# sanweiliti/LEMO

Measured on AMD Instinct MI355X. Metric: fitting-iterations/sec (T=120 frames), higher is better.
Workload: dtype f32

## Files before the change

include/lemo_hip.h:

```cpp
#ifndef LEMO_HIP_H
#define LEMO_HIP_H

#ifdef __cplusplus
extern "C" {
#endif
#if defined(__GNUC__) || defined(__clang__)
#pragma GCC visibility push(default)
#endif

#define LEMO_ERR_SHAPE 10001
#define LEMO_ERR_ARG 10002
#define LEMO_ERR_STATE 10003

int lemo_abi_version(void);
int lemo_build_flags(void);

int lemo_conv3x3_mfma(const float* in, const float* wt, const float* bias, const float* aux, float* out,
                      int H, int W, int cin, int cout, int epi, int variant, void* stream);
int lemo_conv3x3_mfma_splitk(const float* in, const float* wt, const float* bias, const float* aux, float* out,
                             float* partial, int ks, int H, int W, int cin, int cout, int epi, void* stream);
int lemo_conv3x3_mfma_lds(const float* in, const float* wt, const float* wt2, const float* bias, const float* aux,
                          float* out, int H, int W, int cin, int cout, int epi, void* stream);
int lemo_conv3x3_mfma_lds_census(const float* in, const float* wt, const float* wt2, const float* bias, float* out,
                                 int H, int W, int cin, int cout, unsigned long long* dbg, void* stream);
int lemo_conv3x3_split_supported(int H, int W, int cin, int cout);
int lemo_conv3x3_mfma_split(const float* in, const void* w3, const float* wt, const float* bias, const float* aux,
                            float* out, int H, int W, int cin, int cout, int epi, void* stream);
int lemo_conv3x3_mfma_split_census(const float* in, const void* w3, const float* wt, const float* bias, float* out,
                                   int H, int W, int cin, int cout, unsigned long long* dbg, void* stream);
int lemo_conv3x3_mfma_split_f16(const float* in, const void* w2, float winv, const float* wt, const float* bias, const float* aux,
                                float* out, int H, int W, int cin, int cout, int epi, void* stream);
int lemo_conv3x3_mfma_split_census2(const float* in, const void* w, float winv, int pieces, const float* wt, const float* bias, float* out,
                                    int H, int W, int cin, int cout, unsigned long long* dbg, void* stream);
int lemo_conv3x3_pair_supported(int H, int W, int c0, int c1, int c2);
int lemo_conv3x3_pair_f16(const float* in, const void* wA, float winvA, const float* biasA, const float* auxA, float* mid,
                          const void* wB, float winvB, const float* biasB, const float* auxB, float* out, int H, int W, int epi,
                          unsigned long long* dbg, void* stream);
int lemo_conv3x3_wino_supported(int H, int W, int cin, int cout);
int lemo_conv3x3_wino_f16(const float* in, const void* wU, float winv, const float* wt, const float* bias, const float* aux, float* out,
                          int H, int W, int epi, unsigned long long* dbg, void* stream);
int lemo_conv3x3_c1(const float* x0, const float* w, const float* bias, float* out, int H, int W, int cout, void* stream);
int lemo_conv3x3_c1_bwd(const float* dpre, const float* w, float* dx0, int H, int W, int cout, void* stream);
int lemo_smooth_loss_blocks(int H, int W, int C);
int lemo_smooth_loss(const float* z, float* dpre, float* partial, int H, int W, int C, float coef2, void* stream);

typedef struct lemo_vposer_w {
  const float *w1, *w1t, *b1;
  const float *w2, *w2t, *b2;
  const float *w3, *w3t, *b3;
} lemo_vposer_w;
int lemo_vposer_decode_fwd(const lemo_vposer_w* w, const float* z, int z_stride, int B, float* h1, float* h2, float* o,
                           float* matrot, float* aa, void* stream);
int lemo_vposer_decode_bwd(const lemo_vposer_w* w, const float* h1, const float* h2, const float* o, const float* d_aa,
                           const float* d_matrot, int B, float* dz, int dz_stride, float* scratch, void* stream);
int lemo_vposer_mlp_bwd(const lemo_vposer_w* w, const float* h1, const float* h2, int B, float* dz, int dz_stride,
                        float* scratch, void* stream);
int lemo_gemm_nt16(const float* A, int lda, const float* B, int ldb, int M, int N, int K, float* C, int ldc,
                   const float* bias, const float* aux, int ldaux, int epi, void* stream);
int lemo_gemm_nt16_splitk_part_floats(int M, int S);
int lemo_gemm_nt16_splitk(const float* A, int lda, const float* B, int ldb, int M, int N, int K, float* C, int ldc, float* part, int S,
                          const float* A_grouped, void* stream);
int lemo_rot6d_to_aa_fwd(const float* x6, int stride, int N, float* aa, void* stream);
int lemo_rot6d_to_aa_bwd(const float* x6, int stride, const float* d_aa, int N, float* dx6, void* stream);

typedef struct lemo_body_const {
  int nj, nshape, ncomp, nlev;
  const int *parents, *level_start, *level_joints, *child_start, *child_list;
  const float *J_template, *J_dirs, *pose_mean, *lh_comp, *rh_comp;
} lemo_body_const;
typedef struct lemo_pose_in {
  const float *global_orient, *body_pose, *jaw, *leye, *reye, *lh, *rh;
  int hand_stride;
  const float* betas;
  int betas_stride;
  const float* expr;
  const float* rot6d;
  const float* vposer_o;
  float* go_out;
  double* zero_f64;
  int n_zero;
  const int* step_ctr;
  int* step_cur;
  int* nonfinite;
} lemo_pose_in;
typedef struct lemo_pose_ws {
  float *full_pose, *R, *J, *T, *A, *Jtr, *Xg;
  int Bp;
  unsigned short* XgS;
  int xgs_f16;
} lemo_pose_ws;
typedef struct lemo_pose_grad_in {
  const float *dA, *dJtr, *dX;
  const float* d_full_pose;
} lemo_pose_grad_in;
typedef struct lemo_pose_grad_out {
  float *d_global_orient, *d_body_pose, *d_jaw, *d_leye, *d_reye, *d_lh, *d_rh;
  int hand_stride;
  float *d_betas, *d_expr;
  const float* rot6d;
  float* d_rot6d;
  const float* vposer_o;
  float* d_vposer_o;
} lemo_pose_grad_out;
int lemo_smplx_pose_fwd(const lemo_body_const* c, const lemo_pose_in* in, const lemo_pose_ws* ws, int B, void* stream);
int lemo_smplx_pose_bwd(const lemo_body_const* c, const lemo_pose_ws* ws, const lemo_pose_grad_in* gi,
                        const lemo_pose_grad_out* go, int B, void* stream);

typedef struct lemo_skin_const {
  int V, NC, KW;
  int blend_fp32;
  const float* Dg;
  const float* v_template;
  const int* w_idx;
  const float* w_val;
  const unsigned short* DgH;
  float dgh_inv;
} lemo_skin_const;
typedef struct lemo_vertex_set_bwd {
  int n, NCs;
  const int *ids, *vp_row;
  const float* Dk;
  const float* DkT;
  const int *jcsr_start, *jcsr_u;
  const float* jcsr_w;
  const int* jcsr_chunk;
  const int* jc_u;
  const float* jc_w;
  float* part;
  int part_frames;
  int gemm_slabs;
  float* gemm_part;
  const float* DkG;
} lemo_vertex_set_bwd;
int lemo_lbs_verts_fwd(const lemo_skin_const* c, const float* Xg, int Bp, const float* A, int nj, const float* transl,
                       const int* ids, int n, int B, float* verts, float* v_posed, void* stream);
int lemo_lbs_verts_fwd_xs(const lemo_skin_const* c, const float* Xg, const unsigned short* XgS, int Bp, const float* A, int nj,
                          const float* transl, const int* ids, int n, int B, float* verts, float* v_posed, void* stream);
int lemo_lbs_verts_fwd_census(const lemo_skin_const* c, const float* Xg, int Bp, const float* A, int nj, const float* transl,
                              int n, int B, float* verts, float* v_posed, unsigned long long* dbg, void* stream,
                              const unsigned short* XgS );
int lemo_lbs_verts_fwd_active(const lemo_skin_const* c, const lemo_vertex_set_bwd* u, const float* Xg, int Bp, const float* A,
                              int nj, const float* transl, int B, float* blend, float* verts, float* v_posed, void* stream);
int lemo_lbs_verts_bwd(const lemo_skin_const* c, const lemo_vertex_set_bwd* u, const float* A, int nj, const float* v_posed,
                       int vp_rows, const float* dverts, int B, int Bp, float* dvp, float* dA, float* dtransl, float* dX,
                       void* stream);
int lemo_joints_assemble(const float* Jtr, int nj, const float* verts, int vrows, const int* extra_rows, int n_extra,
                         const int* lmk_rows, const float* lmk_bary, int n_lmk, const float* transl, int B, float* joints,
                         void* stream);

int lemo_reconstruct_global_body(const float* in, int T, int J, double rot_0_pivot, float* out, void* stream);
int lemo_reconstruct_global_body_dev(const float* in, int T, int J, const double* rot_0_pivot, float* out, void* stream);
int lemo_decode_clip(const float* rec, const float* traj, const double* stats, const double* rot_0_pivot, const float* post, int T,
                     int J, float* contact_lbl, float* markers, void* stream);
int lemo_local_markers_4chan(const float* body, const float* contact, int T, int M1, float* image, double* rot_0_pivot,
                             void* stream);

int lemo_maxpool3s2_fwd(const float* in, int H, int W, float* out, unsigned char* idx, int C, void* stream);
int lemo_maxpool3s2_bwd(const float* dout, const unsigned char* idx, const float* act, float* din, int H, int W, int C, void* stream);
int lemo_stuff2_fwd(const float* in, int h, int w, float* out, int H, int W, int C, void* stream);
int lemo_stuff2_bwd(const float* dout, int H, int W, const float* act, float* din, int h, int w, int C, void* stream);
int lemo_conv3x3_wgrad_nslab(int H, int W);
int lemo_conv3x3_wgrad(const float* dy, const float* x, int H, int W, int cin, int cout, int cin_real, int cout_real,
                       float* partial, float* dw, float* db, void* stream);
#define LEMO_WGRAD_MAX_JOBS 24
typedef struct lemo_wgrad_job {
  const float* partial;
  const float* dy;
  float* dw;
  float* db;
  int nslab, cin, cout, cin_real, cout_real, H, W;
} lemo_wgrad_job;
int lemo_conv3x3_wgrad_partial(const float* dy, const float* x, int H, int W, int cin, int cout, float* partial, void* stream);
int lemo_conv3x3_wgrad_reduce_multi(const lemo_wgrad_job* jobs, int n, void* stream);
int lemo_adam_flat(float* p, const float* g, float* m, float* v, int n, float lr, int step, void* stream);
int lemo_adam_flat_ctr(float* p, const float* g, float* m, float* v, int n, float lr, int* step_ctr, void* stream);

typedef struct lemo_ae_desc {
  int H, W;
  float lr;
  float* ws;
  long long ws_floats;
  int clips;
} lemo_ae_desc;
long long lemo_ae_ws_floats(int H, int W);
int lemo_ae_n_param(void);
void* lemo_ae_create(const lemo_ae_desc* d);
void lemo_ae_destroy(void* h);
int lemo_ae_load(void* h, const float* flat, const float* x, const float* moc, void* stream);
int lemo_ae_step(void* h, int n, int use_graph, void* stream);
int lemo_ae_forward(void* h, float* rec, float* z, void* stream);
int lemo_ae_params(void* h, float* flat_out, void* stream);
int lemo_ae_load_clip(void* h, int clip, const float* flat, const float* x, const float* moc, void* stream);
int lemo_ae_forward_clip(void* h, int clip, float* rec, float* z, void* stream);
int lemo_ae_params_clip(void* h, int clip, float* flat_out, void* stream);
int lemo_ae_wgrad_probe(void* h, int mode, void* stream);
int lemo_ae_conv(const float* in, const float* wt, const float* bias, const float* aux, float* out, int H, int W, int fineH, int fineW,
                 int in_s, int out_s, int cin, int cout, int epi, int mt, int pt, int ks, void* stream);
int lemo_ae_conv_f16(const float* in, const float* wt, const float* bias, const float* aux, float* out, int H, int W, int fineH, int fineW,
                     int in_s, int out_s, int cin, int cout, int epi, int mt, int pt, int ks, const float* amax_in, float in_fac,
                     const float* wmax, float* amax_out, void* stream);

typedef struct lemo_sptrain_desc {
  int H, W, bs;
  float lr;
  float weight_rec, weight_smooth;
  float* ws;
  long long ws_floats;
  int use_graph;
} lemo_sptrain_desc;
long long lemo_sptrain_ws_floats(int H, int W, int bs);
int lemo_sptrain_n_param(void);
void* lemo_sptrain_create(const lemo_sptrain_desc* d);
void lemo_sptrain_destroy(void* h);
int lemo_sptrain_load(void* h, const float* flat, void* stream);
int lemo_sptrain_step(void* h, const float* x, int n, float* losses, void* stream);
int lemo_sptrain_eval(void* h, const float* x, float* losses, float* rec, void* stream);
int lemo_sptrain_params(void* h, float* flat_out, void* stream);
int lemo_sptrain_grads(void* h, float* flat_out, void* stream);
long long lemo_wgrad3x3_batched_ws_floats(int H, int W, int bs, int ca, int cb);
int lemo_wgrad3x3_batched(const float* A, long long a_stride, const float* B, long long b_stride, int bs, int H, int W, int ca, int cb,
                          int bias_b, float* ws, float* gw, float* gb, void* stream);
int lemo_dec_end_fwd(const float* u, long long u_stride, const float* w8, const float* b8, const float* w9, const float* b9, float* r1,
                     float* rec, int bs, int H, int W, void* stream);

int lemo_capture_begin(void* stream);
int lemo_capture_end(void* stream, void** graph_exec);
int lemo_graph_launch(void* graph_exec, void* stream);
int lemo_graph_destroy(void* graph_exec);

int lemo_sdf_sample(const float* sdf, int D, int H, int W, const float* pts, int N, const float* gmin, const float* gmax,
                    float* val, float* dval, void* stream);

typedef struct lemo_fit_const {
  int n, n67, n81;
  const int *row67, *row81, *foot_start, *foot_row, *u_row, *u_m67, *u_m81, *u_foot_mask;
  const float *Xstd, *Xmean;
  const float* cam2world;
} lemo_fit_const;

int lemo_enc_head(const lemo_fit_const* fc, const float* verts, int nrows, const float* Jtr, int nj, const float* transl, int B, const float* w0,
                  const float* b0, const void* w1pack, float w1inv, const float* b1, float* x0, float* canon, float* act1, float* act2,
                  void* stream);
int lemo_enc_tail(const float* din, const void* w1bpack, float w1binv, const float* act1, const float* w0, float* dx0, int H, int W,
                  void* stream);
int lemo_enc_tail3(const float* din, const void* w2bpack, float w2binv, const float* act2, const void* w1bpack, float w1binv, const float* act1,
                   const float* w0, float* dx0, int H, int W, void* stream);

typedef struct lemo_fit_desc {
  int B, Bp, V, nrows;
  int full_vertices;
  int conv_variant;
  lemo_vposer_w vposer;
  lemo_body_const body;
  lemo_skin_const skin;
  lemo_vertex_set_bwd uset;
  lemo_fit_const fit;
  const int* fwd_ids;
  int enc_ch[11];
  const float* enc_w[10];
  const float* enc_b[10];
  const float* enc_wbwd[10];
  const float* enc_w2[10];
  const float* enc_wbwd2[10];
  const void* enc_w3[10];
  const void* enc_wbwd3[10];
  float enc_w3_inv[10];
  float enc_wbwd3_inv[10];
  const float* target;
  const float* contact;
  const float* weights;
  float weights_host[6];
  float *transl, *rot6d, *other;
  const float* shape;
  float *adam_m[3], *adam_v[3];
  int* step_ctr;
  float lr0, lr1;
  int lr_switch;
  float *go_aa, *body_aa, *h1, *h2, *vo, *vp_scratch;
  lemo_pose_ws pose;
  float *verts, *v_posed, *x0, *canon;
  float* act[11];
  float* dact[2];
  float *dx0, *spartial, *vpartial, *losses, *dverts, *dvp, *dA, *dX;
  double* loss_acc;
  int* step_cur;
  float *g_transl, *g_rot6d, *g_other, *g_go, *g_body;
  float* snap;
  int* nonfinite;
  int per_frame;
  float lr2;
  int lr_switch2;
  float* verts_side;
  float* transl_side;
} lemo_fit_desc;

void* lemo_fit_create(const lemo_fit_desc* d);
void lemo_fit_destroy(void* h);
int lemo_fit_forward(void* h, void* stream);
int lemo_fit_backward(void* h, void* stream);
int lemo_fit_step(void* h, int n, int use_graph, void* stream);
int lemo_fit_prepare(void* h, int n, void* stream);
#define LEMO_FIT_NSTAGE 7
int lemo_fit_census(void* h, int reps, float* ms_out , void* stream);
typedef struct lemo_fit_state {
  float *transl, *rot6d, *other;
  float *adam_m[3], *adam_v[3];
  int* step;
} lemo_fit_state;
int lemo_fit_load_state(void* h, const lemo_fit_state* st, void* stream);
int lemo_fit_save_state(void* h, const lemo_fit_state* st, void* stream);

typedef struct lemo_prox_const {
  int n_op, n_sj;
  const int* joint_map;
  const int *jm_start, *jm_list;
  int n_extra, n_lmk;
  const int* extra_rows;
  const int* lmk_rows;
  const float* lmk_bary;
  int n_s;
  const int *s_vid, *s_m67, *s_m81, *s_foot_mask, *s_fric;
  const int *s_jstart, *s_jidx;
  const float* s_jw;
  int n_fric;
  const int* fric_vid;
  int n67;
  const int* m67_vid;
  const int *foot_start, *foot_vid;
} lemo_prox_const;

#define LEMO_PROX_NW 13
typedef struct lemo_prox_desc {
  int B, Bp, V;
  int conv_variant;
  int first_batch_flag;
  int use_infill;
  int T;
  lemo_vposer_w vposer;
  lemo_body_const body;
  lemo_skin_const skin;
  lemo_vertex_set_bwd uset;
  lemo_fit_const fit;
  lemo_prox_const pc;
  int enc_ch[11];
  const float* enc_w[10]; const float* enc_b[10]; const float* enc_wbwd[10];
  const float* enc_w2[10]; const float* enc_wbwd2[10];
  const void* enc_w3[10]; const void* enc_wbwd3[10];
  float enc_w3_inv[10]; float enc_wbwd3_inv[10];
  const float* sdf; int sdf_dim[3];
  float grid_min[3], grid_max[3];
  float cam2world[12];
  float cam[4];
  const float* gt_joints;
  const float* w2;
  const float* marker_mask;
  const float* body_markers_rec;
  const float* contact_lbl_rec;
  const float* weights;
  float weights_host[LEMO_PROX_NW];
  float *global_orient, *transl, *left_hand_pose, *right_hand_pose, *jaw_pose, *leye_pose, *reye_pose, *expression, *pose_embedding;
  const float* betas;
  float *adam_m, *adam_v;
  int* step_ctr; int* step_cur; int* nonfinite;
  float lr;
  float *h1, *h2, *vo, *vp_scratch;
  lemo_pose_ws pose;
  float *verts, *v_posed, *dverts;
  float *x0, *canon, *dx0;
  float* act[11]; float* dact[2];
  float *dJtr, *dJv, *dtr_j, *gp, *dfp_add;
  float *dvp, *dA, *dtr_v, *dX;
  float *g_go, *g_lh, *g_rh, *g_jaw, *g_leye, *g_reye, *g_expr, *g_pe;
  double* loss_acc;
  float* losses;
} lemo_prox_desc;
void* lemo_prox_create(const lemo_prox_desc* d);
void lemo_prox_destroy(void* h);
int lemo_prox_closure(void* h, void* stream);
int lemo_prox_step(void* h, int n, int use_graph, void* stream);
typedef struct lemo_prox_state {
  float *global_orient, *transl, *left_hand_pose, *right_hand_pose, *jaw_pose, *leye_pose, *reye_pose, *expression, *pose_embedding;
  float *adam_m, *adam_v;
  int* step;
} lemo_prox_state;
int lemo_prox_load_state(void* h, const lemo_prox_state* st, void* stream);
int lemo_prox_save_state(void* h, const lemo_prox_state* st, void* stream);

#if defined(__GNUC__) || defined(__clang__)
#pragma GCC visibility pop
#endif
#ifdef __cplusplus
}
#endif
#endif
```

lemo_amd/_hip.py:

```python
from __future__ import annotations

import ctypes as C
import os
from typing import Optional

import torch

_CSRC = os.path.join(os.path.dirname(os.path.abspath(__file__)), 'csrc')
LIB_PATH = os.environ.get('LEMO_HIP_LIB') or os.path.join(_CSRC, 'liblemo_hip.so')
EMU_LIB_PATH = os.path.join(_CSRC, 'liblemo_emu.so')

fp = C.POINTER(C.c_float)
ip = C.POINTER(C.c_int)
vp = C.c_void_p


class VPoserW(C.Structure):
    _fields_ = [(n, vp) for n in ('w1', 'w1t', 'b1', 'w2', 'w2t', 'b2', 'w3', 'w3t', 'b3')]


class BodyConst(C.Structure):
    _fields_ = [('nj', C.c_int), ('nshape', C.c_int), ('ncomp', C.c_int), ('nlev', C.c_int)] + \
        [(n, vp) for n in ('parents', 'level_start', 'level_joints', 'child_start', 'child_list',
                           'J_template', 'J_dirs', 'pose_mean', 'lh_comp', 'rh_comp')]


class PoseIn(C.Structure):
    _fields_ = [(n, vp) for n in ('global_orient', 'body_pose', 'jaw', 'leye', 'reye', 'lh', 'rh')] + \
        [('hand_stride', C.c_int), ('betas', vp), ('betas_stride', C.c_int), ('expr', vp),
         ('rot6d', vp), ('vposer_o', vp), ('go_out', vp), ('zero_f64', vp), ('n_zero', C.c_int),
         ('step_ctr', vp), ('step_cur', vp), ('nonfinite', vp)]


class PoseWs(C.Structure):
    _fields_ = [(n, vp) for n in ('full_pose', 'R', 'J', 'T', 'A', 'Jtr', 'Xg')] + [('Bp', C.c_int), ('XgS', vp), ('xgs_f16', C.c_int)]


class PoseGradIn(C.Structure):
    _fields_ = [(n, vp) for n in ('dA', 'dJtr', 'dX', 'd_full_pose')]


class PoseGradOut(C.Structure):
    _fields_ = [(n, vp) for n in ('d_global_orient', 'd_body_pose', 'd_jaw', 'd_leye', 'd_reye', 'd_lh', 'd_rh')] + \
        [('hand_stride', C.c_int), ('d_betas', vp), ('d_expr', vp),
         ('rot6d', vp), ('d_rot6d', vp), ('vposer_o', vp), ('d_vposer_o', vp)]


WGRAD_MAX_JOBS = 24


class WgradJob(C.Structure):
    _fields_ = [('partial', vp), ('dy', vp), ('dw', vp), ('db', vp), ('nslab', C.c_int), ('cin', C.c_int), ('cout', C.c_int),
                ('cin_real', C.c_int), ('cout_real', C.c_int), ('H', C.c_int), ('W', C.c_int)]


class AeDesc(C.Structure):
    _fields_ = [('H', C.c_int), ('W', C.c_int), ('lr', C.c_float), ('ws', vp), ('ws_floats', C.c_longlong), ('clips', C.c_int)]


class SptrainDesc(C.Structure):
    _fields_ = [('H', C.c_int), ('W', C.c_int), ('bs', C.c_int), ('lr', C.c_float), ('weight_rec', C.c_float),
                ('weight_smooth', C.c_float), ('ws', vp), ('ws_floats', C.c_longlong), ('use_graph', C.c_int)]


class SkinConst(C.Structure):
    _fields_ = [('V', C.c_int), ('NC', C.c_int), ('KW', C.c_int), ('blend_fp32', C.c_int)] + \
        [(n, vp) for n in ('Dg', 'v_template', 'w_idx', 'w_val', 'DgH')] + [('dgh_inv', C.c_float)]


class VertexSetBwd(C.Structure):
    _fields_ = [('n', C.c_int), ('NCs', C.c_int)] + \
        [(n, vp) for n in ('ids', 'vp_row', 'Dk', 'DkT', 'jcsr_start', 'jcsr_u', 'jcsr_w', 'jcsr_chunk', 'jc_u', 'jc_w', 'part')] + \
        [('part_frames', C.c_int), ('gemm_slabs', C.c_int), ('gemm_part', vp), ('DkG', vp)]


class FitConst(C.Structure):
    _fields_ = [('n', C.c_int), ('n67', C.c_int), ('n81', C.c_int)] + \
        [(n, vp) for n in ('row67', 'row81', 'foot_start', 'foot_row', 'u_row', 'u_m67', 'u_m81',
                           'u_foot_mask', 'Xstd', 'Xmean', 'cam2world')]


CHAIN_MAX = 8


class FitDesc(C.Structure):
    _fields_ = [
        ('B', C.c_int), ('Bp', C.c_int), ('V', C.c_int), ('nrows', C.c_int), ('full_vertices', C.c_int),
        ('conv_variant', C.c_int),
        ('vposer', VPoserW), ('body', BodyConst), ('skin', SkinConst), ('uset', VertexSetBwd), ('fit', FitConst),
        ('fwd_ids', vp),
        ('enc_ch', C.c_int * 11), ('enc_w', vp * 10), ('enc_b', vp * 10), ('enc_wbwd', vp * 10),
        ('enc_w2', vp * 10), ('enc_wbwd2', vp * 10), ('enc_w3', vp * 10), ('enc_wbwd3', vp * 10), ('enc_w3_inv', C.c_float * 10), ('enc_wbwd3_inv', C.c_float * 10),
        ('target', vp), ('contact', vp), ('weights', vp), ('weights_host', C.c_float * 6),
        ('transl', vp), ('rot6d', vp), ('other', vp), ('shape', vp),
        ('adam_m', vp * 3), ('adam_v', vp * 3), ('step_ctr', vp),
        ('lr0', C.c_float), ('lr1', C.c_float), ('lr_switch', C.c_int),
        ('go_aa', vp), ('body_aa', vp), ('h1', vp), ('h2', vp), ('vo', vp), ('vp_scratch', vp),
        ('pose', PoseWs),
        ('verts', vp), ('v_posed', vp), ('x0', vp), ('canon', vp),
        ('act', vp * 11), ('dact', vp * 2),
        ('dx0', vp), ('spartial', vp), ('vpartial', vp), ('losses', vp), ('dverts', vp), ('dvp', vp),
        ('dA', vp), ('dX', vp), ('loss_acc', vp), ('step_cur', vp),
        ('g_transl', vp), ('g_rot6d', vp), ('g_other', vp), ('g_go', vp), ('g_body', vp),
        ('snap', vp), ('nonfinite', vp), ('per_frame', C.c_int), ('lr2', C.c_float), ('lr_switch2', C.c_int),
        ('verts_side', vp), ('transl_side', vp),
    ]


class ProxConst(C.Structure):
    _fields_ = [('n_op', C.c_int), ('n_sj', C.c_int), ('joint_map', vp), ('jm_start', vp), ('jm_list', vp),
                ('n_extra', C.c_int), ('n_lmk', C.c_int), ('extra_rows', vp), ('lmk_rows', vp), ('lmk_bary', vp),
                ('n_s', C.c_int), ('s_vid', vp), ('s_m67', vp), ('s_m81', vp), ('s_foot_mask', vp), ('s_fric', vp),
                ('s_jstart', vp), ('s_jidx', vp), ('s_jw', vp), ('n_fric', C.c_int), ('fric_vid', vp), ('n67', C.c_int),
                ('m67_vid', vp), ('foot_start', vp), ('foot_vid', vp)]


PROX_NW = 13


class ProxDesc(C.Structure):
    _fields_ = [
        ('B', C.c_int), ('Bp', C.c_int), ('V', C.c_int), ('conv_variant', C.c_int), ('first_batch_flag', C.c_int),
        ('use_infill', C.c_int), ('T', C.c_int),
        ('vposer', VPoserW), ('body', BodyConst), ('skin', SkinConst), ('uset', VertexSetBwd), ('fit', FitConst), ('pc', ProxConst),
        ('enc_ch', C.c_int * 11), ('enc_w', vp * 10), ('enc_b', vp * 10), ('enc_wbwd', vp * 10), ('enc_w2', vp * 10),
        ('enc_wbwd2', vp * 10), ('enc_w3', vp * 10), ('enc_wbwd3', vp * 10), ('enc_w3_inv', C.c_float * 10), ('enc_wbwd3_inv', C.c_float * 10),
        ('sdf', vp), ('sdf_dim', C.c_int * 3), ('grid_min', C.c_float * 3), ('grid_max', C.c_float * 3),
        ('cam2world', C.c_float * 12), ('cam', C.c_float * 4),
        ('gt_joints', vp), ('w2', vp), ('marker_mask', vp), ('body_markers_rec', vp), ('contact_lbl_rec', vp),
        ('weights', vp), ('weights_host', C.c_float * PROX_NW),
        ('global_orient', vp), ('transl', vp), ('left_hand_pose', vp), ('right_hand_pose', vp), ('jaw_pose', vp),
        ('leye_pose', vp), ('reye_pose', vp), ('expression', vp), ('pose_embedding', vp), ('betas', vp),
        ('adam_m', vp), ('adam_v', vp), ('step_ctr', vp), ('step_cur', vp), ('nonfinite', vp), ('lr', C.c_float),
        ('h1', vp), ('h2', vp), ('vo', vp), ('vp_scratch', vp), ('pose', PoseWs),
        ('verts', vp), ('v_posed', vp), ('dverts', vp), ('x0', vp), ('canon', vp), ('dx0', vp),
        ('act', vp * 11), ('dact', vp * 2),
        ('dJtr', vp), ('dJv', vp), ('dtr_j', vp), ('gp', vp), ('dfp_add', vp),
        ('dvp', vp), ('dA', vp), ('dtr_v', vp), ('dX', vp),
        ('g_go', vp), ('g_lh', vp), ('g_rh', vp), ('g_jaw', vp), ('g_leye', vp), ('g_reye', vp), ('g_expr', vp), ('g_pe', vp),
        ('loss_acc', vp), ('losses', vp),
    ]


class FitState(C.Structure):
    _fields_ = [('transl', vp), ('rot6d', vp), ('other', vp), ('adam_m', vp * 3), ('adam_v', vp * 3), ('step', vp)]


class ProxState(C.Structure):
    _fields_ = [(n, vp) for n in ('global_orient', 'transl', 'left_hand_pose', 'right_hand_pose', 'jaw_pose', 'leye_pose', 'reye_pose',
                                  'expression', 'pose_embedding', 'adam_m', 'adam_v', 'step')]


def ptr(t: Optional[torch.Tensor]):
    if t is None:
        return None
    assert t.is_contiguous(), 'C ABI takes contiguous buffers'
    return t.data_ptr()


class LemoHipError(RuntimeError):
    pass


_SIGS = {
    'lemo_abi_version': (C.c_int, []),
    'lemo_build_flags': (C.c_int, []),
    'lemo_conv3x3_mfma': (C.c_int, [vp, vp, vp, vp, vp, C.c_int, C.c_int, C.c_int, C.c_int, C.c_int, C.c_int, vp]),
    'lemo_conv3x3_mfma_splitk': (C.c_int, [vp, vp, vp, vp, vp, vp, C.c_int, C.c_int, C.c_int, C.c_int, C.c_int, C.c_int, vp]),
    'lemo_conv3x3_mfma_lds': (C.c_int, [vp, vp, vp, vp, vp, vp, C.c_int, C.c_int, C.c_int, C.c_int, C.c_int, vp]),
    'lemo_lbs_verts_fwd_active': (C.c_int, [C.POINTER(SkinConst), C.POINTER(VertexSetBwd), vp, C.c_int, vp, C.c_int, vp, C.c_int, vp, vp, vp, vp]),
    'lemo_capture_begin': (C.c_int, [vp]),
    'lemo_capture_end': (C.c_int, [vp, C.POINTER(C.c_void_p)]),
    'lemo_graph_launch': (C.c_int, [vp, vp]),
    'lemo_graph_destroy': (C.c_int, [vp]),
    'lemo_reconstruct_global_body': (C.c_int, [vp, C.c_int, C.c_int, C.c_double, vp, vp]),
    'lemo_reconstruct_global_body_dev': (C.c_int, [vp, C.c_int, C.c_int, vp, vp, vp]),
    'lemo_local_markers_4chan': (C.c_int, [vp, vp, C.c_int, C.c_int, vp, vp, vp]),
    'lemo_decode_clip': (C.c_int, [vp, vp, vp, vp, vp, C.c_int, C.c_int, vp, vp, vp]),
    'lemo_conv3x3_split_supported': (C.c_int, [C.c_int, C.c_int, C.c_int, C.c_int]),
    'lemo_conv3x3_mfma_split': (C.c_int, [vp, vp, vp, vp, vp, vp, C.c_int, C.c_int, C.c_int, C.c_int, C.c_int, vp]),
    'lemo_conv3x3_mfma_split_census': (C.c_int, [vp, vp, vp, vp, vp, C.c_int, C.c_int, C.c_int, C.c_int, vp, vp]),
    'lemo_conv3x3_mfma_split_f16': (C.c_int, [vp, vp, C.c_float, vp, vp, vp, vp, C.c_int, C.c_int, C.c_int, C.c_int, C.c_int, vp]),
    'lemo_conv3x3_pair_supported': (C.c_int, [C.c_int] * 5),
    'lemo_conv3x3_wino_supported': (C.c_int, [C.c_int] * 4),
    'lemo_conv3x3_wino_f16': (C.c_int, [vp, vp, C.c_float, vp, vp, vp, vp, C.c_int, C.c_int, C.c_int, vp, vp]),
    'lemo_conv3x3_pair_f16': (C.c_int, [vp, vp, C.c_float, vp, vp, vp, vp, C.c_float, vp, vp, vp, C.c_int, C.c_int, C.c_int, vp, vp]),
    'lemo_enc_head': (C.c_int, [vp, vp, C.c_int, vp, C.c_int, vp, C.c_int, vp, vp, vp, C.c_float, vp, vp, vp, vp, vp, vp]),
    'lemo_enc_tail': (C.c_int, [vp, vp, C.c_float, vp, vp, vp, C.c_int, C.c_int, vp]),
    'lemo_enc_tail3': (C.c_int, [vp, vp, C.c_float, vp, vp, C.c_float, vp, vp, vp, C.c_int, C.c_int, vp]),
    'lemo_conv3x3_mfma_split_census2': (C.c_int, [vp, vp, C.c_float, C.c_int, vp, vp, vp, C.c_int, C.c_int, C.c_int, C.c_int, vp, vp]),
    'lemo_conv3x3_mfma_lds_census': (C.c_int, [vp, vp, vp, vp, vp, C.c_int, C.c_int, C.c_int, C.c_int, vp, vp]),
    'lemo_conv3x3_c1': (C.c_int, [vp, vp, vp, vp, C.c_int, C.c_int, C.c_int, vp]),
    'lemo_conv3x3_c1_bwd': (C.c_int, [vp, vp, vp, C.c_int, C.c_int, C.c_int, vp]),
    'lemo_smooth_loss_blocks': (C.c_int, [C.c_int, C.c_int, C.c_int]),
    'lemo_smooth_loss': (C.c_int, [vp, vp, vp, C.c_int, C.c_int, C.c_int, C.c_float, vp]),
    'lemo_vposer_decode_fwd': (C.c_int, [C.POINTER(VPoserW), vp, C.c_int, C.c_int, vp, vp, vp, vp, vp, vp]),
    'lemo_vposer_decode_bwd': (C.c_int, [C.POINTER(VPoserW), vp, vp, vp, vp, vp, C.c_int, vp, C.c_int, vp, vp]),
    'lemo_vposer_mlp_bwd': (C.c_int, [C.POINTER(VPoserW), vp, vp, C.c_int, vp, C.c_int, vp, vp]),
    'lemo_gemm_nt16': (C.c_int, [vp, C.c_int, vp, C.c_int, C.c_int, C.c_int, C.c_int, vp, C.c_int, vp, vp, C.c_int, C.c_int, vp]),
    'lemo_gemm_nt16_splitk_part_floats': (C.c_int, [C.c_int, C.c_int]),
    'lemo_gemm_nt16_splitk': (C.c_int, [vp, C.c_int, vp, C.c_int, C.c_int, C.c_int, C.c_int, vp, C.c_int, vp, C.c_int, vp, vp]),
    'lemo_rot6d_to_aa_fwd': (C.c_int, [vp, C.c_int, C.c_int, vp, vp]),
    'lemo_rot6d_to_aa_bwd': (C.c_int, [vp, C.c_int, vp, C.c_int, vp, vp]),
    'lemo_smplx_pose_fwd': (C.c_int, [C.POINTER(BodyConst), C.POINTER(PoseIn), C.POINTER(PoseWs), C.c_int, vp]),
    'lemo_smplx_pose_bwd': (C.c_int, [C.POINTER(BodyConst), C.POINTER(PoseWs), C.POINTER(PoseGradIn),
                                      C.POINTER(PoseGradOut), C.c_int, vp]),
    'lemo_lbs_verts_fwd': (C.c_int, [C.POINTER(SkinConst), vp, C.c_int, vp, C.c_int, vp, vp, C.c_int, C.c_int, vp, vp, vp]),
    'lemo_lbs_verts_fwd_xs': (C.c_int, [C.POINTER(SkinConst), vp, vp, C.c_int, vp, C.c_int, vp, vp, C.c_int, C.c_int, vp, vp, vp]),
    'lemo_lbs_verts_fwd_census': (C.c_int, [C.POINTER(SkinConst), vp, C.c_int, vp, C.c_int, vp, C.c_int, C.c_int, vp, vp, vp, vp, vp]),
    'lemo_lbs_verts_bwd': (C.c_int, [C.POINTER(SkinConst), C.POINTER(VertexSetBwd), vp, C.c_int, vp, C.c_int, vp,
                                     C.c_int, C.c_int, vp, vp, vp, vp, vp]),
    'lemo_joints_assemble': (C.c_int, [vp, C.c_int, vp, C.c_int, vp, C.c_int, vp, vp, C.c_int, vp, C.c_int, vp, vp]),
    'lemo_maxpool3s2_fwd': (C.c_int, [vp, C.c_int, C.c_int, vp, vp, C.c_int, vp]),
    'lemo_maxpool3s2_bwd': (C.c_int, [vp, vp, vp, vp, C.c_int, C.c_int, C.c_int, vp]),
    'lemo_stuff2_fwd': (C.c_int, [vp, C.c_int, C.c_int, vp, C.c_int, C.c_int, C.c_int, vp]),
    'lemo_stuff2_bwd': (C.c_int, [vp, C.c_int, C.c_int, vp, vp, C.c_int, C.c_int, C.c_int, vp]),
    'lemo_conv3x3_wgrad_nslab': (C.c_int, [C.c_int, C.c_int]),
    'lemo_conv3x3_wgrad': (C.c_int, [vp, vp, C.c_int, C.c_int, C.c_int, C.c_int, C.c_int, C.c_int, vp, vp, vp, vp]),
    'lemo_conv3x3_wgrad_partial': (C.c_int, [vp, vp, C.c_int, C.c_int, C.c_int, C.c_int, vp, vp]),
    'lemo_conv3x3_wgrad_reduce_multi': (C.c_int, [C.POINTER(WgradJob), C.c_int, vp]),
    'lemo_adam_flat': (C.c_int, [vp, vp, vp, vp, C.c_int, C.c_float, C.c_int, vp]),
    'lemo_adam_flat_ctr': (C.c_int, [vp, vp, vp, vp, C.c_int, C.c_float, vp, vp]),
    'lemo_ae_ws_floats': (C.c_longlong, [C.c_int, C.c_int]),
    'lemo_ae_n_param': (C.c_int, []),
    'lemo_ae_create': (vp, [C.POINTER(AeDesc)]),
    'lemo_ae_destroy': (None, [vp]),
    'lemo_ae_load': (C.c_int, [vp, vp, vp, vp, vp]),
    'lemo_ae_step': (C.c_int, [vp, C.c_int, C.c_int, vp]),
    'lemo_ae_forward': (C.c_int, [vp, vp, vp, vp]),
    'lemo_ae_params': (C.c_int, [vp, vp, vp]),
    'lemo_ae_load_clip': (C.c_int, [vp, C.c_int, vp, vp, vp, vp]),
    'lemo_ae_forward_clip': (C.c_int, [vp, C.c_int, vp, vp, vp]),
    'lemo_ae_params_clip': (C.c_int, [vp, C.c_int, vp, vp]),
    'lemo_ae_wgrad_probe': (C.c_int, [vp, C.c_int, vp]),
    'lemo_ae_conv': (C.c_int, [vp, vp, vp, vp, vp] + [C.c_int] * 12 + [vp]),
    'lemo_ae_conv_f16': (C.c_int, [vp, vp, vp, vp, vp] + [C.c_int] * 12 + [vp, C.c_float, vp, vp, vp]),
    'lemo_sptrain_ws_floats': (C.c_longlong, [C.c_int, C.c_int, C.c_int]),
    'lemo_sptrain_n_param': (C.c_int, []),
    'lemo_sptrain_create': (vp, [C.POINTER(SptrainDesc)]),
    'lemo_sptrain_destroy': (None, [vp]),
    'lemo_sptrain_load': (C.c_int, [vp, vp, vp]),
    'lemo_sptrain_step': (C.c_int, [vp, vp, C.c_int, vp, vp]),
    'lemo_sptrain_eval': (C.c_int, [vp, vp, vp, vp, vp]),
    'lemo_sptrain_params': (C.c_int, [vp, vp, vp]),
    'lemo_sptrain_grads': (C.c_int, [vp, vp, vp]),
    'lemo_wgrad3x3_batched_ws_floats': (C.c_longlong, [C.c_int] * 5),
    'lemo_wgrad3x3_batched': (C.c_int, [vp, C.c_longlong, vp, C.c_longlong] + [C.c_int] * 6 + [vp, vp, vp, vp]),
    'lemo_dec_end_fwd': (C.c_int, [vp, C.c_longlong, vp, vp, vp, vp, vp, vp, C.c_int, C.c_int, C.c_int, vp]),
    'lemo_sdf_sample': (C.c_int, [vp, C.c_int, C.c_int, C.c_int, vp, C.c_int, C.POINTER(C.c_float), C.POINTER(C.c_float), vp, vp, vp]),
    'lemo_fit_create': (vp, [C.POINTER(FitDesc)]),
    'lemo_fit_destroy': (None, [vp]),
    'lemo_fit_forward': (C.c_int, [vp, vp]),
    'lemo_fit_backward': (C.c_int, [vp, vp]),
    'lemo_fit_step': (C.c_int, [vp, C.c_int, C.c_int, vp]),
    'lemo_fit_prepare': (C.c_int, [vp, C.c_int, vp]),
    'lemo_fit_census': (C.c_int, [vp, C.c_int, C.POINTER(C.c_float), vp]),
    'lemo_fit_load_state': (C.c_int, [vp, C.POINTER(FitState), vp]),
    'lemo_fit_save_state': (C.c_int, [vp, C.POINTER(FitState), vp]),
    'lemo_prox_load_state': (C.c_int, [vp, C.POINTER(ProxState), vp]),
    'lemo_prox_save_state': (C.c_int, [vp, C.POINTER(ProxState), vp]),
    'lemo_prox_create': (vp, [C.POINTER(ProxDesc)]),
    'lemo_prox_destroy': (None, [vp]),
    'lemo_prox_closure': (C.c_int, [vp, vp]),
    'lemo_prox_step': (C.c_int, [vp, C.c_int, C.c_int, vp]),
}
EXPORTED_SYMBOLS = tuple(_SIGS)


class HipLib:

    def __init__(self, path: str, is_emu: bool = False):
        if not os.path.exists(path):
            raise LemoHipError(
                f'{path} not found: the HIP extension is not built. Build it with '
                f'`make -C {_CSRC}` (hipcc --offload-arch=gfx950); there is no CPU fallback.')
        self.path, self.is_emu = path, is_emu
        self._dll = C.CDLL(path)
        for name, (res, args) in _SIGS.items():
            fn = getattr(self._dll, name)
            fn.restype, fn.argtypes = res, args
            setattr(self, name[len('lemo_'):], fn)
        if not self.build_flags() & 1:
            raise LemoHipError(f'{path} was built without -fno-slp-vectorize -fno-vectorize (-DLEMO_NO_PACKED_FP32): rebuild it with '
                               f'`make -C {_CSRC}`')

    def check(self, rc: int, what: str = ''):
        if rc != 0:
            raise LemoHipError(f'liblemo_hip: {what} failed with code {rc}')

    def stream(self, device) -> Optional[int]:
        if self.is_emu:
            return None
        return torch.cuda.current_stream(device).cuda_stream


_DEFERRED: list = []


def quiesce(device, lib=None) -> bool:
    try:
        dev = torch.device(device)
        if dev.type == 'cuda' and not (lib is not None and lib.is_emu) and torch.cuda.is_available():
            if torch.cuda.is_current_stream_capturing():
                return False
            torch.cuda.synchronize(dev)
    except Exception:
        pass
    return True


def flush_deferred() -> None:
    if not _DEFERRED:
        return
    try:
        if torch.cuda.is_available() and torch.cuda.is_current_stream_capturing():
            return
    except Exception:
        return
    pending, _DEFERRED[:] = list(_DEFERRED), []
    for fn in pending:
        try:
            fn()
        except Exception:
            pass


def release(device, lib, destroy, event=None) -> None:
    def wait():
        if event is None:
            return quiesce(device, lib)
        try:
            if torch.cuda.is_current_stream_capturing():
                return False
            event.synchronize()
        except Exception:
            pass
        return True

    def run():
        if event is not None:
            try:
                event.synchronize()
            except Exception:
                pass
        destroy()

    if wait():
        flush_deferred()
        try:
            destroy()
        except Exception:
            pass
    else:
        _DEFERRED.append(run)


_LIB: Optional[HipLib] = None


def get_lib() -> HipLib:
    global _LIB
    if _LIB is None:
        _LIB = HipLib(LIB_PATH, is_emu=False)
    return _LIB


def check_device(lib: HipLib, t: torch.Tensor):
    if lib.is_emu:
        if t.is_cuda:
            raise LemoHipError('the host-emulated test library only takes CPU tensors')
    elif not t.is_cuda:
        raise LemoHipError('lemo_amd compute entry points need tensors on a HIP device (no CPU fallback)')


class StreamOrdered:
    _gpu = False
    _setup_ev = _run_ev = None

    def _init_order(self, device, lib):
        self._gpu = torch.device(device).type == 'cuda' and not lib.is_emu and os.environ.get('LEMO_UNORDERED', '0') != '1'
        self._odev = torch.device(device)
        self._setup_ev = self._run_ev = None

    def _cur(self):
        return torch.cuda.current_stream(self._odev)

    def _before_write(self):
        if self._gpu and self._run_ev is not None:
            self._cur().wait_event(self._run_ev)

    def _after_write(self):
        if self._gpu:
            if self._setup_ev is None:
                self._setup_ev = torch.cuda.Event()
            self._setup_ev.record(self._cur())

    def _before_run(self):
        if self._gpu:
            flush_deferred()
            for ev in (self._setup_ev, self._run_ev):
                if ev is not None:
                    self._cur().wait_event(ev)

    def _after_run(self):
        if self._gpu:
            if self._run_ev is None:
                self._run_ev = torch.cuda.Event()
            self._run_ev.record(self._cur())

    _before_read = _before_write
```

lemo_amd/csrc/conv_head_kernels.hip:

```cpp
#include <type_traits>
#include "conv_f16.hpp"
#include "loss_device.hpp"

namespace lemo {

constexpr int HD_TH = 10, HD_TW = 14;
constexpr int HD_XW = HD_TW + 4, HD_XH = HD_TH + 4, HD_NX = HD_XW * HD_XH;
constexpr int HD_MIDW = HD_TW + 2, HD_MIDH = HD_TH + 2;
constexpr int HD_MIDP = HD_MIDW + 2, HD_NMIDP = HD_MIDP * HD_MIDH;
constexpr int HD_PL_MID = HD_NMIDP * 16, HD_GRP_MID = 2 * HD_PL_MID;
constexpr int HD_PL_IN = HD_NX * 16, HD_GRP_IN = 2 * HD_PL_IN;
static_assert(HD_MIDW == 16 && HD_XW == HD_MIDP, "N-tiles = 2 rows x 16 columns on grids of row pitch 18");

__device__ __forceinline__ int hd_lane_col(int j) { return j < 16 ? j : ((j - 18) & 15); }

template <int U, int END> struct HdSteps {
  template <class F> static __device__ __forceinline__ void run(F&& f) { f(std::integral_constant<int, U>{}); HdSteps<U + 1, END>::run(f); }
};
template <int END> struct HdSteps<END, END> { template <class F> static __device__ __forceinline__ void run(F&&) {} };

#define HD_RA 4
template <int GRP, int PL, int MT = 1, int NST = 18, int PITCH = HD_MIDP>
__device__ __forceinline__ void hd_kloop(f32x16 (&acc)[3], const uint4* __restrict__ w, const unsigned char* bbase, int li, int lane, int mt = 0) {
  const int h = lane >> 5;
  uint4 ra[HD_RA][2], rb[2][2];
#define HD_LOAD_A(SET, U) _Pragma("unroll") for (int s_ = 0; s_ < 2; ++s_) ra[SET][s_] = w[(unsigned)(((U) * MT + mt) * 2 + s_) * 64u + lane];
#define HD_LOAD_B(SET, U) _Pragma("unroll") for (int s_ = 0; s_ < 2; ++s_)                                                          \
    rb[SET][s_] = *reinterpret_cast<const uint4*>(bbase + (2 * ((U) / 9) + h) * GRP + s_ * PL + (li + (((U) % 9) / 3 - 1) * PITCH + (((U) % 9) % 3 - 1)) * 16);
#pragma unroll
  for (int u0 = 0; u0 < HD_RA - 1; ++u0) { HD_LOAD_A(u0, u0) }
  HD_LOAD_B(0, 0)
  HdSteps<0, NST>::run([&](auto uc) {
    constexpr int u = decltype(uc)::value;
    if (u + HD_RA - 1 < NST) { HD_LOAD_A((u + HD_RA - 1) % HD_RA, (u + HD_RA - 1 < NST ? u + HD_RA - 1 : NST - 1)) }
    if (u + 1 < NST) { HD_LOAD_B((u + 1) & 1, (u + 1 < NST ? u + 1 : NST - 1)) }
    __builtin_amdgcn_sched_barrier(0);
    acc[0] = __builtin_amdgcn_mfma_f32_32x32x16_f16(__builtin_bit_cast(f16x8, ra[u % HD_RA][0]), __builtin_bit_cast(f16x8, rb[u & 1][1]), acc[0], 0, 0, 0);
    acc[1] = __builtin_amdgcn_mfma_f32_32x32x16_f16(__builtin_bit_cast(f16x8, ra[u % HD_RA][1]), __builtin_bit_cast(f16x8, rb[u & 1][0]), acc[1], 0, 0, 0);
    acc[2] = __builtin_amdgcn_mfma_f32_32x32x16_f16(__builtin_bit_cast(f16x8, ra[u % HD_RA][0]), __builtin_bit_cast(f16x8, rb[u & 1][0]), acc[2], 0, 0, 0);
    __builtin_amdgcn_sched_barrier(0);
  });
#undef HD_LOAD_A
#undef HD_LOAD_B
}

template <int GRP, int PL, int MT>
__device__ __forceinline__ void hd_kloop2(f32x16 (&acc)[2][3], const uint4* __restrict__ w, const unsigned char* bbase, const int (&li)[2], int lane, int mt) {
  const int h = lane >> 5;
  uint4 ra[HD_RA][2], rb[2][2][2];
#define HD_LOAD_A(SET, U) _Pragma("unroll") for (int s_ = 0; s_ < 2; ++s_) ra[SET][s_] = w[(unsigned)(((U) * MT + mt) * 2 + s_) * 64u + lane];
#define HD_LOAD_B(SET, U) _Pragma("unroll") for (int t_ = 0; t_ < 2; ++t_) _Pragma("unroll") for (int s_ = 0; s_ < 2; ++s_)            \
    rb[SET][t_][s_] = *reinterpret_cast<const uint4*>(bbase + (2 * ((U) / 9) + h) * GRP + s_ * PL + (li[t_] + (((U) % 9) / 3 - 1) * HD_MIDP + (((U) % 9) % 3 - 1)) * 16);
#pragma unroll
  for (int u0 = 0; u0 < HD_RA - 1; ++u0) { HD_LOAD_A(u0, u0) }
  HD_LOAD_B(0, 0)
  HdSteps<0, 18>::run([&](auto uc) {
    constexpr int u = decltype(uc)::value;
    if (u + HD_RA - 1 < 18) { HD_LOAD_A((u + HD_RA - 1) % HD_RA, (u + HD_RA - 1 < 18 ? u + HD_RA - 1 : 17)) }
    if (u + 1 < 18) { HD_LOAD_B((u + 1) & 1, (u + 1 < 18 ? u + 1 : 17)) }
    __builtin_amdgcn_sched_barrier(0);
#pragma unroll
    for (int t_ = 0; t_ < 2; ++t_) {
      acc[t_][0] = __builtin_amdgcn_mfma_f32_32x32x16_f16(__builtin_bit_cast(f16x8, ra[u % HD_RA][0]), __builtin_bit_cast(f16x8, rb[u & 1][t_][1]), acc[t_][0], 0, 0, 0);
      acc[t_][1] = __builtin_amdgcn_mfma_f32_32x32x16_f16(__builtin_bit_cast(f16x8, ra[u % HD_RA][1]), __builtin_bit_cast(f16x8, rb[u & 1][t_][0]), acc[t_][1], 0, 0, 0);
      acc[t_][2] = __builtin_amdgcn_mfma_f32_32x32x16_f16(__builtin_bit_cast(f16x8, ra[u % HD_RA][0]), __builtin_bit_cast(f16x8, rb[u & 1][t_][0]), acc[t_][2], 0, 0, 0);
    }
    __builtin_amdgcn_sched_barrier(0);
  });
#undef HD_LOAD_A
#undef HD_LOAD_B
}

struct HeadArgs {
  FitConst fc;
  const float* verts; int nrows;
  const float* Jtr; int nj;
  const float* transl; int B;
  const float *w0, *b0;
  const uint4* w1; float w1inv;
  const float* b1;
  float *x0, *canon_out, *act1, *act2;
  int ntx, ntiles;
};

__global__ void __launch_bounds__(512)
enc_head_kernel(HeadArgs a) {
  __shared__ __attribute__((aligned(16))) unsigned char mid[4 * HD_GRP_MID];
  __shared__ float xs[HD_NX];
  __shared__ float cn[12];
  __shared__ float wmax[8];
  const FitConst& fc = a.fc;
  const int tid = (int)threadIdx.x, lane = tid & 63, wave = tid >> 6;
  const int D = 3 * fc.n81, H = D + 2, W = a.B - 1 + 16, Wp = W + 2, HWp = (H + 2) * Wp;
  int tile = (int)blockIdx.x;
  {
    const int q = a.ntiles >> 3, r = a.ntiles & 7, xcd = tile & 7, k = tile >> 3;
    tile = (xcd < r ? xcd * (q + 1) : r * (q + 1) + (xcd - r) * q) + k;
  }
  const int ty = tile / a.ntx, tx = tile - ty * a.ntx;
  const int y0 = ty * HD_TH, x0c = tx * HD_TW;
  float va[3] = {0.f, 0.f, 0.f}, vb[3] = {0.f, 0.f, 0.f}, xm = 0.f, xsd = 1.f;
  int cc = 0;
  bool inside = false;
  const int ip = tid < HD_NX ? tid : HD_NX - 1;
  const int ily = ip / HD_XW, ilx = ip - ily * HD_XW;
  {
    const int yy = y0 - 2 + ily, xx = x0c - 2 + ilx;
    inside = yy >= 0 && yy < H && xx >= 0 && xx < W;
    const int yc = min(max(yy, 0), H - 1), xc = min(max(xx, 0), W - 1);
    const int d = reflect_idx(yc - 1, D), tp = reflect_idx(xc - 8, a.B - 1);
    const int m = d / 3;
    cc = d - 3 * m;
    const float* v0 = a.verts + ((size_t)tp * a.nrows + fc.row81[m]) * 3;
    const float* v1 = v0 + (size_t)a.nrows * 3;
#pragma unroll
    for (int e = 0; e < 3; ++e) { va[e] = v0[e]; vb[e] = v1[e]; }
    xm = fc.Xmean[d]; xsd = fc.Xstd[d];
  }
  if (tid >= 512 - HD_MIDH * 2 * 8) {
    const int i = tid - (512 - HD_MIDH * 2 * 8), pl = i / (HD_MIDH * 2), rc = i - pl * (HD_MIDH * 2);
    *reinterpret_cast<uint4*>(mid + pl * HD_PL_MID + ((rc >> 1) * HD_MIDP + (rc & 1) * (HD_MIDP - 1)) * 16) = make_uint4(0u, 0u, 0u, 0u);
  }
  if (tid == 0) {
    canonical_frame(a.verts, a.nrows, fc.row81, a.Jtr, a.nj, a.transl, cn, fc.cam2world);
    if (blockIdx.x == 0) for (int i = 0; i < 12; ++i) a.canon_out[i] = cn[i];
  }
  __syncthreads();
  if (tid < HD_NX) {
    const float g0 = (va[0] - cn[9]) * cn[cc] + (va[1] - cn[10]) * cn[3 + cc] + (va[2] - cn[11]) * cn[6 + cc];
    const float g1 = (vb[0] - cn[9]) * cn[cc] + (vb[1] - cn[10]) * cn[3 + cc] + (vb[2] - cn[11]) * cn[6 + cc];
    const float n0 = (g0 - xm) / xsd, n1 = (g1 - xm) / xsd;
    const float v = inside ? n1 - n0 : 0.f;
    xs[tid] = v;
    if (inside && ily >= 2 && ily < 2 + HD_TH && ilx >= 2 && ilx < 2 + HD_TW)
      a.x0[(size_t)(y0 + ily - 2 + 1) * Wp + (x0c + ilx - 2 + 1)] = v;
  }
  __syncthreads();
  const int halfu = __builtin_amdgcn_readfirstlane(wave / 3);
  const bool worker = wave < 6;
  const int px = worker ? tid - 192 * halfu : 0;
  const int my = px >> 4, mx = px & 15;
  const int y = y0 - 1 + my, x = x0c - 1 + mx;
  const bool inimg = worker && (unsigned)y < (unsigned)H && (unsigned)x < (unsigned)W;
  const bool inner = inimg && my >= 1 && my <= HD_TH && mx >= 1 && mx <= HD_TW;
  float r[16];
  float mloc = 0.f;
  if (worker) {
    float xin[9];
#pragma unroll
    for (int tp = 0; tp < 9; ++tp) xin[tp] = xs[(my + tp / 3) * HD_XW + mx + tp % 3];
#pragma unroll
    for (int c = 0; c < 16; ++c) {
      const float* wc = a.w0 + (size_t)(halfu * 16 + c) * 9;
      float acc = 0.f;
#pragma unroll
      for (int tp = 0; tp < 9; ++tp) acc = fmaf(wc[tp], xin[tp], acc);
      const float v = lrelu(acc + a.b0[halfu * 16 + c]);
      r[c] = inimg ? v : 0.f;
      mloc = fmaxf(mloc, fabsf(r[c]));
    }
  } else {
#pragma unroll
    for (int c = 0; c < 16; ++c) r[c] = 0.f;
  }
  mloc = wave_max(mloc);
  if (lane == 0) wmax[wave] = mloc;
  __syncthreads();
  float sm, smi;
  {
    float mm = 0.f;
#pragma unroll
    for (int i = 0; i < 8; ++i) mm = fmaxf(mm, wmax[i]);
    f16_scale_for(mm, sm, smi);
  }
  if (worker) {
    const int yc = y < 0 ? 0 : (y >= H ? H - 1 : y), xc = x < 0 ? 0 : (x >= W ? W - 1 : x);
    const int poff = (yc + 1) * Wp + (xc + 1);
#pragma unroll
    for (int g = 0; g < 2; ++g) {
      const float4 lo4 = make_float4(r[8 * g], r[8 * g + 1], r[8 * g + 2], r[8 * g + 3]);
      const float4 hi4 = make_float4(r[8 * g + 4], r[8 * g + 5], r[8 * g + 6], r[8 * g + 7]);
      if (inner) {
        float* o = a.act1 + ((size_t)(2 * halfu + g) * HWp + poff) * 8;
        st4(o, lo4); st4(o + 4, hi4);
      }
      uint2 a0, a1, b0, b1;
      split2x4(lo4, sm, a0, a1);
      split2x4(hi4, sm, b0, b1);
      unsigned char* d = mid + (2 * halfu + g) * HD_GRP_MID + (my * HD_MIDP + mx + 1) * 16;
      *reinterpret_cast<uint4*>(d) = make_uint4(a0.x, a0.y, b0.x, b0.y);
      *reinterpret_cast<uint4*>(d + HD_PL_MID) = make_uint4(a1.x, a1.y, b1.x, b1.y);
    }
  }
  __syncthreads();
  if (wave >= 5) return;
  const int j = lane & 31, h = lane >> 5;
  const int oy = 2 * wave + (j >> 4), c = hd_lane_col(j), ox = c - 1;
  const int lo = (oy + 1) * HD_MIDP + c + 1;
  f32x16 acc[3];
#pragma unroll
  for (int p = 0; p < 3; ++p)
#pragma unroll
    for (int e = 0; e < 16; ++e) acc[p][e] = 0.f;
  hd_kloop<HD_GRP_MID, HD_PL_MID>(acc, a.w1, mid, lo, lane);
  const int yo = y0 + oy, xo = x0c + ox;
  const bool ok = ox >= 0 && ox < HD_TW && yo < H && xo < W;
  const int yoc = yo < H ? yo : H - 1, xoc = xo < 0 ? 0 : (xo < W ? xo : W - 1);
  const int po = (yoc + 1) * Wp + (xoc + 1);
  const float f = smi * a.w1inv;
#pragma unroll
  for (int q = 0; q < 4; ++q) {
    const int c0 = q * 8 + 4 * h;
    const float4 bb = ld4(a.b1 + c0);
    float4 v;
    v.x = lrelu(((acc[0][4 * q] + acc[1][4 * q]) + acc[2][4 * q]) * f + bb.x);
    v.y = lrelu(((acc[0][4 * q + 1] + acc[1][4 * q + 1]) + acc[2][4 * q + 1]) * f + bb.y);
    v.z = lrelu(((acc[0][4 * q + 2] + acc[1][4 * q + 2]) + acc[2][4 * q + 2]) * f + bb.z);
    v.w = lrelu(((acc[0][4 * q + 3] + acc[1][4 * q + 3]) + acc[2][4 * q + 3]) * f + bb.w);
    if (ok) st4(a.act2 + ((size_t)(c0 >> 3) * HWp + po) * 8 + (c0 & 7), v);
  }
}

int enc_head(const FitConst& fc, const float* verts, int nrows, const float* Jtr, int nj, const float* transl, int B, const float* w0,
             const float* b0, const void* w1pack, float w1inv, const float* b1, float* x0, float* canon, float* act1, float* act2,
             hipStream_t s) {
  if (B < 10 || !w1pack || !(w1inv > 0.f) || !verts || !x0 || !canon || !act1 || !act2) return LEMO_ERR_ARG;
  const int H = 3 * fc.n81 + 2, W = B - 1 + 16;
  HeadArgs a{};
  a.fc = fc; a.verts = verts; a.nrows = nrows; a.Jtr = Jtr; a.nj = nj; a.transl = transl; a.B = B;
  a.w0 = w0; a.b0 = b0; a.w1 = reinterpret_cast<const uint4*>(w1pack); a.w1inv = w1inv; a.b1 = b1;
  a.x0 = x0; a.canon_out = canon; a.act1 = act1; a.act2 = act2;
  a.ntx = (W + HD_TW - 1) / HD_TW;
  a.ntiles = a.ntx * ((H + HD_TH - 1) / HD_TH);
  hipLaunchKernelGGL(enc_head_kernel, dim3(a.ntiles), dim3(512), 0, s, a);
  return (int)hipGetLastError();
}

constexpr int H3_IW = HD_TW + 6, H3_IH = HD_TH + 6, H3_NI = H3_IW * H3_IH;
constexpr int H3_PL1 = HD_NX * 16, H3_GRP1 = 2 * H3_PL1;

struct Head3Args {
  HeadArgs h;
  const uint4* w2; float w2inv; const float* b2;
  float* act3;
};

__global__ void __launch_bounds__(512)
enc_head3_kernel(Head3Args A3) {
  __shared__ __attribute__((aligned(16))) unsigned char p1[4 * H3_GRP1];
  __shared__ __attribute__((aligned(16))) unsigned char p2[4 * HD_GRP_MID];
  __shared__ float xs[H3_NI];
  __shared__ float cn[12];
  __shared__ float wmax[24];
  const HeadArgs& a = A3.h;
  const FitConst& fc = a.fc;
  const int tid = (int)threadIdx.x, lane = tid & 63, wave = tid >> 6;
  const int j = lane & 31, h = lane >> 5;
  const int D = 3 * fc.n81, H = D + 2, W = a.B - 1 + 16, Wp = W + 2, HWp = (H + 2) * Wp;
  int tile = (int)blockIdx.x;
  {
    const int q = a.ntiles >> 3, r = a.ntiles & 7, xcd = tile & 7, k = tile >> 3;
    tile = (xcd < r ? xcd * (q + 1) : r * (q + 1) + (xcd - r) * q) + k;
  }
  const int ty = tile / a.ntx, tx = tile - ty * a.ntx;
  const int y0 = ty * HD_TH, x0c = tx * HD_TW;
  float va[3] = {0.f, 0.f, 0.f}, vb[3] = {0.f, 0.f, 0.f}, xm = 0.f, xsd = 1.f;
  int cc = 0;
  bool inside = false;
  const int ip = tid < H3_NI ? tid : H3_NI - 1;
  const int ily = ip / H3_IW, ilx = ip - ily * H3_IW;
  {
    const int yy = y0 - 3 + ily, xx = x0c - 3 + ilx;
    inside = yy >= 0 && yy < H && xx >= 0 && xx < W;
    const int yc = min(max(yy, 0), H - 1), xc = min(max(xx, 0), W - 1);
    const int d = reflect_idx(yc - 1, D), tp = reflect_idx(xc - 8, a.B - 1);
    const int m = d / 3;
    cc = d - 3 * m;
    const float* v0 = a.verts + ((size_t)tp * a.nrows + fc.row81[m]) * 3;
    const float* v1 = v0 + (size_t)a.nrows * 3;
#pragma unroll
    for (int e = 0; e < 3; ++e) { va[e] = v0[e]; vb[e] = v1[e]; }
    xm = fc.Xmean[d]; xsd = fc.Xstd[d];
  }
  if (tid >= 512 - HD_MIDH * 2 * 8) {
    const int i = tid - (512 - HD_MIDH * 2 * 8), pl = i / (HD_MIDH * 2), rc = i - pl * (HD_MIDH * 2);
    *reinterpret_cast<uint4*>(p2 + pl * HD_PL_MID + ((rc >> 1) * HD_MIDP + (rc & 1) * (HD_MIDP - 1)) * 16) = make_uint4(0u, 0u, 0u, 0u);
  }
  if (tid == 0) {
    canonical_frame(a.verts, a.nrows, fc.row81, a.Jtr, a.nj, a.transl, cn, fc.cam2world);
    if (blockIdx.x == 0) for (int i = 0; i < 12; ++i) a.canon_out[i] = cn[i];
  }
  __syncthreads();
  if (tid < H3_NI) {
    const float g0 = (va[0] - cn[9]) * cn[cc] + (va[1] - cn[10]) * cn[3 + cc] + (va[2] - cn[11]) * cn[6 + cc];
    const float g1 = (vb[0] - cn[9]) * cn[cc] + (vb[1] - cn[10]) * cn[3 + cc] + (vb[2] - cn[11]) * cn[6 + cc];
    const float n0 = (g0 - xm) / xsd, n1 = (g1 - xm) / xsd;
    const float v = inside ? n1 - n0 : 0.f;
    xs[tid] = v;
    if (inside && ily >= 3 && ily < 3 + HD_TH && ilx >= 3 && ilx < 3 + HD_TW)
      a.x0[(size_t)(y0 + ily - 3 + 1) * Wp + (x0c + ilx - 3 + 1)] = v;
  }
  __syncthreads();
  {
    const int halfu = __builtin_amdgcn_readfirstlane(wave >> 2);
    const int px = tid & 255;
    const bool worker = px < HD_NX;
    const int pc = worker ? px : 0;
    const int r1 = pc / HD_XW, c1 = pc - r1 * HD_XW;
    const int y = y0 - 2 + r1, x = x0c - 2 + c1;
    const bool inimg = worker && (unsigned)y < (unsigned)H && (unsigned)x < (unsigned)W;
    const bool inner = inimg && r1 >= 2 && r1 < 2 + HD_TH && c1 >= 2 && c1 < 2 + HD_TW;
    float r[16];
    float mloc = 0.f;
    float xin[9];
#pragma unroll
    for (int tp = 0; tp < 9; ++tp) xin[tp] = xs[(r1 + tp / 3) * H3_IW + c1 + tp % 3];
#pragma unroll
    for (int c = 0; c < 16; ++c) {
      const float* wc = a.w0 + (size_t)(halfu * 16 + c) * 9;
      float acc = 0.f;
#pragma unroll
      for (int tp = 0; tp < 9; ++tp) acc = fmaf(wc[tp], xin[tp], acc);
      const float v = lrelu(acc + a.b0[halfu * 16 + c]);
      r[c] = inimg ? v : 0.f;
      mloc = fmaxf(mloc, fabsf(r[c]));
    }
    mloc = wave_max(mloc);
    if (lane == 0) wmax[wave] = mloc;
    __syncthreads();
    float sm, smi;
    {
      float mm = 0.f;
#pragma unroll
      for (int i = 0; i < 8; ++i) mm = fmaxf(mm, wmax[i]);
      f16_scale_for(mm, sm, smi);
    }
    if (lane == 0 && wave == 0) wmax[20] = smi;
    if (worker) {
      const int yc = y < 0 ? 0 : (y >= H ? H - 1 : y), xc = x < 0 ? 0 : (x >= W ? W - 1 : x);
      const int poff = (yc + 1) * Wp + (xc + 1);
#pragma unroll
      for (int g = 0; g < 2; ++g) {
        const float4 lo4 = make_float4(r[8 * g], r[8 * g + 1], r[8 * g + 2], r[8 * g + 3]);
        const float4 hi4 = make_float4(r[8 * g + 4], r[8 * g + 5], r[8 * g + 6], r[8 * g + 7]);
        if (inner) {
          float* o = a.act1 + ((size_t)(2 * halfu + g) * HWp + poff) * 8;
          st4(o, lo4); st4(o + 4, hi4);
        }
        uint2 a0, a1, b0, b1;
        split2x4(lo4, sm, a0, a1);
        split2x4(hi4, sm, b0, b1);
        unsigned char* d = p1 + (2 * halfu + g) * H3_GRP1 + pc * 16;
        *reinterpret_cast<uint4*>(d) = make_uint4(a0.x, a0.y, b0.x, b0.y);
        *reinterpret_cast<uint4*>(d + H3_PL1) = make_uint4(a1.x, a1.y, b1.x, b1.y);
      }
    }
  }
  __syncthreads();
  float4 v1[4];
  float m1 = 0.f;
  int mp2 = 0, mpoff = 0;
  bool inner2 = false;
  if (wave < 6) {
    const int my = 2 * wave + (j >> 4), mx = hd_lane_col(j);
    const int li = (my + 1) * HD_XW + mx + 1;
    f32x16 acc[3];
#pragma unroll
    for (int p = 0; p < 3; ++p)
#pragma unroll
      for (int e = 0; e < 16; ++e) acc[p][e] = 0.f;
    hd_kloop<H3_GRP1, H3_PL1>(acc, a.w1, p1, li, lane);
    const int y = y0 - 1 + my, x = x0c - 1 + mx;
    const bool inimg = (unsigned)y < (unsigned)H && (unsigned)x < (unsigned)W;
    inner2 = inimg && my >= 1 && my <= HD_TH && mx >= 1 && mx <= HD_TW;
    const int yc = y < 0 ? 0 : (y >= H ? H - 1 : y), xc = x < 0 ? 0 : (x >= W ? W - 1 : x);
    mpoff = (yc + 1) * Wp + (xc + 1);
    mp2 = my * HD_MIDP + mx + 1;
    const float f = wmax[20] * a.w1inv;
#pragma unroll
    for (int q = 0; q < 4; ++q) {
      const float4 bb = ld4(a.b1 + q * 8 + 4 * h);
      float4 v;
      v.x = lrelu(((acc[0][4 * q] + acc[1][4 * q]) + acc[2][4 * q]) * f + bb.x);
      v.y = lrelu(((acc[0][4 * q + 1] + acc[1][4 * q + 1]) + acc[2][4 * q + 1]) * f + bb.y);
      v.z = lrelu(((acc[0][4 * q + 2] + acc[1][4 * q + 2]) + acc[2][4 * q + 2]) * f + bb.z);
      v.w = lrelu(((acc[0][4 * q + 3] + acc[1][4 * q + 3]) + acc[2][4 * q + 3]) * f + bb.w);
      if (!inimg) v = make_float4(0.f, 0.f, 0.f, 0.f);
      v1[q] = v;
      m1 = absmax4(v, m1);
    }
  } else {
#pragma unroll
    for (int q = 0; q < 4; ++q) v1[q] = make_float4(0.f, 0.f, 0.f, 0.f);
  }
  m1 = wave_max(m1);
  if (lane == 0 && wave < 6) wmax[8 + wave] = m1;
  if (lane == 0 && wave >= 6) wmax[8 + wave] = 0.f;
  __syncthreads();
  float sm2, smi2;
  {
    float mm = 0.f;
#pragma unroll
    for (int i = 0; i < 8; ++i) mm = fmaxf(mm, wmax[8 + i]);
    f16_scale_for(mm, sm2, smi2);
  }
  if (wave < 6) {
#pragma unroll
    for (int q = 0; q < 4; ++q) {
      const int c0 = q * 8 + 4 * h;
      if (inner2) st4(a.act2 + ((size_t)(c0 >> 3) * HWp + mpoff) * 8 + (c0 & 7), v1[q]);
      uint2 s0, s1;
      split2x4(v1[q], sm2, s0, s1);
      unsigned char* d = p2 + q * HD_GRP_MID + mp2 * 16 + 8 * h;
      *reinterpret_cast<uint2*>(d) = s0;
      *reinterpret_cast<uint2*>(d + HD_PL_MID) = s1;
    }
  }
  __syncthreads();
  {
    const int mt = wave & 1, ts = wave >> 1;
    const float f = smi2 * A3.w2inv;
    auto store_tile = [&](const f32x16 (&acc)[3], int T) {
      const int oy = 2 * T + (j >> 4), c = hd_lane_col(j), ox = c - 1;
      const int yo = y0 + oy, xo = x0c + ox;
      const bool ok = ox >= 0 && ox < HD_TW && yo < H && xo < W;
      const int yoc = yo < H ? yo : H - 1, xoc = xo < 0 ? 0 : (xo < W ? xo : W - 1);
      const int po = (yoc + 1) * Wp + (xoc + 1);
#pragma unroll
      for (int q = 0; q < 4; ++q) {
        const int c0 = mt * 32 + q * 8 + 4 * h;
        const float4 bb = ld4(A3.b2 + c0);
        float4 v;
        v.x = lrelu(((acc[0][4 * q] + acc[1][4 * q]) + acc[2][4 * q]) * f + bb.x);
        v.y = lrelu(((acc[0][4 * q + 1] + acc[1][4 * q + 1]) + acc[2][4 * q + 1]) * f + bb.y);
        v.z = lrelu(((acc[0][4 * q + 2] + acc[1][4 * q + 2]) + acc[2][4 * q + 2]) * f + bb.z);
        v.w = lrelu(((acc[0][4 * q + 3] + acc[1][4 * q + 3]) + acc[2][4 * q + 3]) * f + bb.w);
        if (ok) st4(A3.act3 + ((size_t)(c0 >> 3) * HWp + po) * 8 + (c0 & 7), v);
      }
    };
    auto lo_of = [&](int T) { const int oy = 2 * T + (j >> 4), c = hd_lane_col(j); return (oy + 1) * HD_MIDP + c + 1; };
    if (ts < 3) {
      f32x16 acc[3];
#pragma unroll
      for (int p = 0; p < 3; ++p)
#pragma unroll
        for (int e = 0; e < 16; ++e) acc[p][e] = 0.f;
      hd_kloop<HD_GRP_MID, HD_PL_MID, 2>(acc, A3.w2, p2, lo_of(ts), lane, mt);
      store_tile(acc, ts);
    } else {
      f32x16 acc[2][3];
#pragma unroll
      for (int t = 0; t < 2; ++t)
#pragma unroll
        for (int p = 0; p < 3; ++p)
#pragma unroll
          for (int e = 0; e < 16; ++e) acc[t][p][e] = 0.f;
      const int li2[2] = {lo_of(3), lo_of(4)};
      hd_kloop2<HD_GRP_MID, HD_PL_MID, 2>(acc, A3.w2, p2, li2, lane, mt);
      store_tile(acc[0], 3);
      store_tile(acc[1], 4);
    }
  }
}

int enc_head3(const FitConst& fc, const float* verts, int nrows, const float* Jtr, int nj, const float* transl, int B, const float* w0,
              const float* b0, const void* w1pack, float w1inv, const float* b1, const void* w2pack, float w2inv, const float* b2,
              float* x0, float* canon, float* act1, float* act2, float* act3, hipStream_t s) {
  if (B < 10 || !w1pack || !w2pack || !(w1inv > 0.f) || !(w2inv > 0.f) || !verts || !x0 || !canon || !act1 || !act2 || !act3) return LEMO_ERR_ARG;
  const int H = 3 * fc.n81 + 2, W = B - 1 + 16;
  Head3Args A{};
  HeadArgs& a = A.h;
  a.fc = fc; a.verts = verts; a.nrows = nrows; a.Jtr = Jtr; a.nj = nj; a.transl = transl; a.B = B;
  a.w0 = w0; a.b0 = b0; a.w1 = reinterpret_cast<const uint4*>(w1pack); a.w1inv = w1inv; a.b1 = b1;
  a.x0 = x0; a.canon_out = canon; a.act1 = act1; a.act2 = act2;
  a.ntx = (W + HD_TW - 1) / HD_TW;
  a.ntiles = a.ntx * ((H + HD_TH - 1) / HD_TH);
  A.w2 = reinterpret_cast<const uint4*>(w2pack); A.w2inv = w2inv; A.b2 = b2; A.act3 = act3;
  hipLaunchKernelGGL(enc_head3_kernel, dim3(a.ntiles), dim3(512), 0, s, A);
  return (int)hipGetLastError();
}

struct TailArgs {
  const float* din;
  const uint4* w1b; float w1binv;
  const float* act1;
  const float* w0;
  float* dx0;
  int H, W, ntx, ntiles;
};

__global__ void __launch_bounds__(512)
enc_tail_kernel(TailArgs a) {
  __shared__ __attribute__((aligned(16))) unsigned char inp[4 * HD_GRP_IN];
  __shared__ __attribute__((aligned(16))) float d1[32 * HD_NMIDP];
  __shared__ float wmax[8];
  const int tid = (int)threadIdx.x, lane = tid & 63, wave = tid >> 6;
  const int H = a.H, W = a.W, Wp = W + 2, HWp = (H + 2) * Wp;
  int tile = (int)blockIdx.x;
  {
    const int q = a.ntiles >> 3, r = a.ntiles & 7, xcd = tile & 7, k = tile >> 3;
    tile = (xcd < r ? xcd * (q + 1) : r * (q + 1) + (xcd - r) * q) + k;
  }
  const int ty = tile / a.ntx, tx = tile - ty * a.ntx;
  const int y0 = ty * HD_TH, x0c = tx * HD_TW;
  float4 st[4];
  int dst[4];
#pragma unroll
  for (int k = 0; k < 4; ++k) {
    int c0 = tid + k * 512;
    c0 = c0 < 4 * 2 * HD_NX ? c0 : 4 * 2 * HD_NX - 1;
    const int gg = c0 / (2 * HD_NX), c = c0 - gg * (2 * HD_NX);
    const int px = c >> 1, half = c & 1;
    const int r = px / HD_XW, col = px - r * HD_XW;
    int gy = y0 - 2 + r, gx = x0c - 2 + col;
    gy = (gy < -1 ? -1 : (gy > H ? H : gy)) + 1;
    gx = (gx < -1 ? -1 : (gx > W ? W : gx)) + 1;
    st[k] = ld4(a.din + ((size_t)gg * HWp + gy * Wp + gx) * 8 + 4 * half);
    dst[k] = gg * HD_GRP_IN + px * 16 + 8 * half;
  }
  float sc, sci;
  {
    float m = 0.f;
#pragma unroll
    for (int k = 0; k < 4; ++k) m = absmax4(st[k], m);
    m = wave_max(m);
    if (lane == 0) wmax[wave] = m;
    __syncthreads();
    float mm = 0.f;
#pragma unroll
    for (int i = 0; i < 8; ++i) mm = fmaxf(mm, wmax[i]);
    f16_scale_for(mm, sc, sci);
  }
#pragma unroll
  for (int k = 0; k < 4; ++k) {
    uint2 s0, s1;
    split2x4(st[k], sc, s0, s1);
    *reinterpret_cast<uint2*>(inp + dst[k]) = s0;
    *reinterpret_cast<uint2*>(inp + dst[k] + HD_PL_IN) = s1;
  }
  __syncthreads();
  if (wave < 6) {
    const int j = lane & 31, h = lane >> 5;
    const int my = 2 * wave + (j >> 4), mx = hd_lane_col(j);
    const int li = (my + 1) * HD_XW + mx + 1;
    f32x16 acc[3];
#pragma unroll
    for (int p = 0; p < 3; ++p)
#pragma unroll
      for (int e = 0; e < 16; ++e) acc[p][e] = 0.f;
    const int y = y0 - 1 + my, x = x0c - 1 + mx;
    const bool inimg = (unsigned)y < (unsigned)H && (unsigned)x < (unsigned)W;
    const int yc = y < 0 ? 0 : (y >= H ? H - 1 : y), xc = x < 0 ? 0 : (x >= W ? W - 1 : x);
    const int poff = (yc + 1) * Wp + (xc + 1);
    float4 aux[4];
#pragma unroll
    for (int q = 0; q < 4; ++q) { const int c0 = q * 8 + 4 * h; aux[q] = ld4(a.act1 + ((size_t)(c0 >> 3) * HWp + poff) * 8 + (c0 & 7)); }
    hd_kloop<HD_GRP_IN, HD_PL_IN>(acc, a.w1b, inp, li, lane);
    const float f = sci * a.w1binv;
#pragma unroll
    for (int q = 0; q < 4; ++q) {
      const int c0 = q * 8 + 4 * h;
      float v[4];
      const float ax[4] = {aux[q].x, aux[q].y, aux[q].z, aux[q].w};
#pragma unroll
      for (int e = 0; e < 4; ++e) {
        const float s = ((acc[0][4 * q + e] + acc[1][4 * q + e]) + acc[2][4 * q + e]) * f * lrelu_grad_from_out(ax[e]);
        v[e] = inimg ? s : 0.f;
      }
#pragma unroll
      for (int e = 0; e < 4; ++e) d1[(c0 + e) * HD_NMIDP + my * HD_MIDP + mx + 1] = v[e];
    }
  }
  __syncthreads();
  if (tid < HD_TH * HD_TW) {
    const int oy = tid / HD_TW, ox = tid - oy * HD_TW;
    const int y = y0 + oy, x = x0c + ox;
    if (y < H && x < W) {
      float acc = 0.f;
      for (int g = 0; g < 4; ++g) {
#pragma unroll
        for (int t = 0; t < 9; ++t) {
          const int dy = t / 3 - 1, dx = t % 3 - 1;
          const float* q = d1 + (size_t)(g * 8) * HD_NMIDP + (oy + 1 - dy) * HD_MIDP + (ox + 1 - dx) + 1;
          const float* wc = a.w0 + (size_t)(g * 8) * 9 + t;
#pragma unroll
          for (int c = 0; c < 8; ++c) acc = fmaf(q[c * HD_NMIDP], wc[9 * c], acc);
        }
      }
      a.dx0[(size_t)y * W + x] = acc;
    }
  }
}

int enc_tail(const float* din, const void* w1bpack, float w1binv, const float* act1, const float* w0, float* dx0, int H, int W, hipStream_t s) {
  if (!din || !w1bpack || !(w1binv > 0.f) || !act1 || !w0 || !dx0 || H < 1 || W < 1) return LEMO_ERR_ARG;
  TailArgs a{};
  a.din = din; a.w1b = reinterpret_cast<const uint4*>(w1bpack); a.w1binv = w1binv; a.act1 = act1; a.w0 = w0; a.dx0 = dx0;
  a.H = H; a.W = W;
  a.ntx = (W + HD_TW - 1) / HD_TW;
  a.ntiles = a.ntx * ((H + HD_TH - 1) / HD_TH);
  hipLaunchKernelGGL(enc_tail_kernel, dim3(a.ntiles), dim3(512), 0, s, a);
  return (int)hipGetLastError();
}

constexpr int T3_IW = HD_TW + 6, T3_IH = HD_TH + 6, T3_NI = T3_IW * T3_IH;
constexpr int T3_PL = T3_NI * 16, T3_GRP = 2 * T3_PL;
constexpr int T3_MID_OFF = 8 * T3_GRP;
constexpr int T3_WMAX_OFF = T3_MID_OFF + 4 * HD_GRP_IN;
constexpr int T3_SMEM = T3_WMAX_OFF + 16 * 4;
static_assert(32 * HD_NMIDP * 4 <= T3_MID_OFF, "d(pre-act 1) fits in the dead input planes");

struct Tail3Args {
  TailArgs t;
  const uint4* w2b; float w2binv;
  const float* act2;
};

__global__ void __launch_bounds__(512)
enc_tail3_kernel(Tail3Args A3) {
  LEMO_DYN_SMEM(smem_f);
  unsigned char* smem = reinterpret_cast<unsigned char*>(smem_f);
  unsigned char* inp = smem + T3_MID_OFF;
  float* d1 = smem_f;
  float* wmax = reinterpret_cast<float*>(smem + T3_WMAX_OFF);
  const TailArgs& a = A3.t;
  const int tid = (int)threadIdx.x, lane = tid & 63, wave = tid >> 6;
  const int j = lane & 31, h = lane >> 5;
  const int H = a.H, W = a.W, Wp = W + 2, HWp = (H + 2) * Wp;
  int tile = (int)blockIdx.x;
  {
    const int q = a.ntiles >> 3, r = a.ntiles & 7, xcd = tile & 7, k = tile >> 3;
    tile = (xcd < r ? xcd * (q + 1) : r * (q + 1) + (xcd - r) * q) + k;
  }
  const int ty = tile / a.ntx, tx = tile - ty * a.ntx;
  const int y0 = ty * HD_TH, x0c = tx * HD_TW;
  float sc, sci;
  {
    float4 st[10];
    int dst[10];
#pragma unroll
    for (int k = 0; k < 10; ++k) {
      const int c0 = tid + k * 512;
      const int gg = c0 / (2 * T3_NI), c = c0 - gg * (2 * T3_NI);
      const int px = c >> 1, half = c & 1;
      const int r = px / T3_IW, col = px - r * T3_IW;
      int gy = y0 - 3 + r, gx = x0c - 3 + col;
      gy = (gy < -1 ? -1 : (gy > H ? H : gy)) + 1;
      gx = (gx < -1 ? -1 : (gx > W ? W : gx)) + 1;
      st[k] = ld4(a.din + ((size_t)gg * HWp + gy * Wp + gx) * 8 + 4 * half);
      dst[k] = gg * T3_GRP + px * 16 + 8 * half;
    }
    float m = 0.f;
#pragma unroll
    for (int k = 0; k < 10; ++k) m = absmax4(st[k], m);
    m = wave_max(m);
    if (lane == 0) wmax[wave] = m;
    __syncthreads();
    float mm = 0.f;
#pragma unroll
    for (int i = 0; i < 8; ++i) mm = fmaxf(mm, wmax[i]);
    f16_scale_for(mm, sc, sci);
#pragma unroll
    for (int k = 0; k < 10; ++k) {
      uint2 s0, s1;
      split2x4(st[k], sc, s0, s1);
      *reinterpret_cast<uint2*>(smem + dst[k]) = s0;
      *reinterpret_cast<uint2*>(smem + dst[k] + T3_PL) = s1;
    }
  }
  __syncthreads();
  {
    const int o = 32 * wave + j, oc = o < HD_NX ? o : HD_NX - 1;
    const int r = oc / HD_XW, c = oc - r * HD_XW;
    const int li = (r + 1) * T3_IW + c + 1;
    const int y = y0 - 2 + r, x = x0c - 2 + c;
    const bool inimg = (unsigned)y < (unsigned)H && (unsigned)x < (unsigned)W;
    const int yc = y < 0 ? 0 : (y >= H ? H - 1 : y), xc = x < 0 ? 0 : (x >= W ? W - 1 : x);
    const int poff = (yc + 1) * Wp + (xc + 1);
    float4 aux[4];
#pragma unroll
    for (int q = 0; q < 4; ++q) { const int c0 = q * 8 + 4 * h; aux[q] = ld4(A3.act2 + ((size_t)(c0 >> 3) * HWp + poff) * 8 + (c0 & 7)); }
    f32x16 acc[3];
#pragma unroll
    for (int p = 0; p < 3; ++p)
#pragma unroll
      for (int e = 0; e < 16; ++e) acc[p][e] = 0.f;
    hd_kloop<T3_GRP, T3_PL, 1, 36, T3_IW>(acc, A3.w2b, smem, li, lane);
    const float f = sci * A3.w2binv;
    float4 v2[4];
    float m2 = 0.f;
#pragma unroll
    for (int q = 0; q < 4; ++q) {
      const float ax[4] = {aux[q].x, aux[q].y, aux[q].z, aux[q].w};
      float v[4];
#pragma unroll
      for (int e = 0; e < 4; ++e) {
        const float s = ((acc[0][4 * q + e] + acc[1][4 * q + e]) + acc[2][4 * q + e]) * f * lrelu_grad_from_out(ax[e]);
        v[e] = inimg ? s : 0.f;
      }
      v2[q] = make_float4(v[0], v[1], v[2], v[3]);
      m2 = absmax4(v2[q], m2);
    }
    m2 = wave_max(m2);
    if (lane == 0) wmax[8 + wave] = m2;
    __syncthreads();
    float mm = 0.f;
#pragma unroll
    for (int i = 0; i < 8; ++i) mm = fmaxf(mm, wmax[8 + i]);
    f16_scale_for(mm, sc, sci);
    if (o < HD_NX) {
#pragma unroll
      for (int q = 0; q < 4; ++q) {
        uint2 s0, s1;
        split2x4(v2[q], sc, s0, s1);
        unsigned char* d = inp + q * HD_GRP_IN + o * 16 + 8 * h;
        *reinterpret_cast<uint2*>(d) = s0;
        *reinterpret_cast<uint2*>(d + HD_PL_IN) = s1;
      }
    }
  }
  __syncthreads();
  if (wave < 6) {
    const int my = 2 * wave + (j >> 4), mx = hd_lane_col(j);
    const int li = (my + 1) * HD_XW + mx + 1;
    f32x16 acc[3];
#pragma unroll
    for (int p = 0; p < 3; ++p)
#pragma unroll
      for (int e = 0; e < 16; ++e) acc[p][e] = 0.f;
    const int y = y0 - 1 + my, x = x0c - 1 + mx;
    const bool inimg = (unsigned)y < (unsigned)H && (unsigned)x < (unsigned)W;
    const int yc = y < 0 ? 0 : (y >= H ? H - 1 : y), xc = x < 0 ? 0 : (x >= W ? W - 1 : x);
    const int poff = (yc + 1) * Wp + (xc + 1);
    float4 aux[4];
#pragma unroll
    for (int q = 0; q < 4; ++q) { const int c0 = q * 8 + 4 * h; aux[q] = ld4(a.act1 + ((size_t)(c0 >> 3) * HWp + poff) * 8 + (c0 & 7)); }
    hd_kloop<HD_GRP_IN, HD_PL_IN>(acc, a.w1b, inp, li, lane);
    const float f = sci * a.w1binv;
#pragma unroll
    for (int q = 0; q < 4; ++q) {
      const int c0 = q * 8 + 4 * h;
      float v[4];
      const float ax[4] = {aux[q].x, aux[q].y, aux[q].z, aux[q].w};
#pragma unroll
      for (int e = 0; e < 4; ++e) {
        const float s = ((acc[0][4 * q + e] + acc[1][4 * q + e]) + acc[2][4 * q + e]) * f * lrelu_grad_from_out(ax[e]);
        v[e] = inimg ? s : 0.f;
      }
#pragma unroll
      for (int e = 0; e < 4; ++e) d1[(c0 + e) * HD_NMIDP + my * HD_MIDP + mx + 1] = v[e];
    }
  }
  __syncthreads();
  if (tid < HD_TH * HD_TW) {
    const int oy = tid / HD_TW, ox = tid - oy * HD_TW;
    const int y = y0 + oy, x = x0c + ox;
    if (y < H && x < W) {
      float acc = 0.f;
      for (int g = 0; g < 4; ++g) {
#pragma unroll
        for (int t = 0; t < 9; ++t) {
          const int dy = t / 3 - 1, dx = t % 3 - 1;
          const float* q = d1 + (size_t)(g * 8) * HD_NMIDP + (oy + 1 - dy) * HD_MIDP + (ox + 1 - dx) + 1;
          const float* wc = a.w0 + (size_t)(g * 8) * 9 + t;
#pragma unroll
          for (int c = 0; c < 8; ++c) acc = fmaf(q[c * HD_NMIDP], wc[9 * c], acc);
        }
      }
      a.dx0[(size_t)y * W + x] = acc;
    }
  }
}

int enc_tail3_init() {
  static LdsOptinOnce once;
  return lds_optin(once, {{&enc_tail3_kernel, T3_SMEM}});
}

int enc_tail3(const float* din, const void* w2bpack, float w2binv, const float* act2, const void* w1bpack, float w1binv, const float* act1,
              const float* w0, float* dx0, int H, int W, hipStream_t s) {
  if (!din || !w2bpack || !(w2binv > 0.f) || !act2 || !w1bpack || !(w1binv > 0.f) || !act1 || !w0 || !dx0 || H < 1 || W < 1) return LEMO_ERR_ARG;
  if (int rc = enc_tail3_init()) return rc;
  Tail3Args A{};
  TailArgs& a = A.t;
  a.din = din; a.w1b = reinterpret_cast<const uint4*>(w1bpack); a.w1binv = w1binv; a.act1 = act1; a.w0 = w0; a.dx0 = dx0;
  a.H = H; a.W = W;
  a.ntx = (W + HD_TW - 1) / HD_TW;
  a.ntiles = a.ntx * ((H + HD_TH - 1) / HD_TH);
  A.w2b = reinterpret_cast<const uint4*>(w2bpack); A.w2binv = w2binv; A.act2 = act2;
  hipLaunchKernelGGL(enc_tail3_kernel, dim3(a.ntiles), dim3(512), T3_SMEM, s, A);
  return (int)hipGetLastError();
}

}
```

lemo_amd/csrc/conv_pair_kernels.hip:

```cpp
#include "conv_common.hpp"
#include "conv_f16.hpp"

namespace lemo {

constexpr int CP_TH = 10, CP_TW = 14;
constexpr int CP_INW = CP_TW + 4, CP_INH = CP_TH + 4, CP_NIN = CP_INW * CP_INH;
constexpr int CP_MIDW = CP_TW + 2, CP_MIDH = CP_TH + 2, CP_NMID = CP_MIDW * CP_MIDH;
constexpr int CP_MIDP = CP_MIDW + 2, CP_NMIDP = CP_MIDP * CP_MIDH;
constexpr int CP_NOUT = CP_TH * CP_TW;
constexpr int CP_PL_IN = CP_NIN * 16, CP_GRP_IN = 2 * CP_PL_IN;
constexpr int CP_PL_MID = CP_NMIDP * 16, CP_GRP_MID = 2 * CP_PL_MID;
constexpr int CP_MID_OFF = 8 * CP_GRP_IN;
constexpr int CP_WMAX_OFF = CP_MID_OFF + 8 * CP_GRP_MID;
constexpr int CP_SMEM = CP_WMAX_OFF + 3 * 8 * 4;
constexpr int CP_NSLOT = 4;
static_assert(CP_MIDW == 16 && CP_NMID == 6 * 32 && CP_INW == CP_MIDP, "N-tiles = 2 rows x 16 columns on grids of row pitch 18");
static_assert(4 * 2 * CP_NIN <= CP_NSLOT * 512 && CP_NOUT == 140, "staging slots");
static_assert(8 * 6 * 256 * 4 <= CP_MID_OFF, "the K-half exchange (6 quads per wave) fits the dead input planes");

struct PairArgs {
  const float* in;
  const uint4* wA;
  const uint4* wB;
  const float *biasA, *biasB;
  const float *auxA, *auxB;
  float* mid;
  float* out;
  float winvA, winvB;
  int H, W, ntx, ntiles;
  unsigned long long* dbg;
};

template <int NT> struct PairSplit {
  static constexpr int NQ = NT == 3 ? 6 : 4;
  static constexpr int keep_tile(int KH, int i) { return i < 4 ? KH : 2; }
  static constexpr int keep_quad(int KH, int i) { return i < 4 ? i : (i - 4) + 2 * KH; }
  static constexpr int give_tile(int KH, int i) { return i < 4 ? 1 - KH : 2; }
  static constexpr int give_quad(int KH, int i) { return i < 4 ? i : (i - 4) + 2 * (1 - KH); }
};

template <int NT, int KH>
__device__ __forceinline__ void pair_exchange(const f32x16 (&acc)[3], float4 (&v)[6], float* red_mine, const float* red_theirs) {
  typedef PairSplit<NT> S;
#pragma unroll
  for (int i = 0; i < S::NQ; ++i) {
    const int t = S::give_tile(KH, i), q = S::give_quad(KH, i);
    st4(red_mine + i * 256, make_float4(acc[t][4 * q], acc[t][4 * q + 1], acc[t][4 * q + 2], acc[t][4 * q + 3]));
  }
  __syncthreads();
#pragma unroll
  for (int i = 0; i < S::NQ; ++i) {
    const int t = S::keep_tile(KH, i), q = S::keep_quad(KH, i);
    const float4 o = ld4(red_theirs + i * 256);
    const float4 m = make_float4(acc[t][4 * q], acc[t][4 * q + 1], acc[t][4 * q + 2], acc[t][4 * q + 3]);
    v[i] = KH ? make_float4(o.x + m.x, o.y + m.y, o.z + m.z, o.w + m.w) : make_float4(m.x + o.x, m.y + o.y, m.z + o.z, m.w + o.w);
  }
}

__device__ __forceinline__ int cp_lane_col(int j) { return j < 16 ? j : ((j - 18) & 15); }

#define CP_RA 3

__device__ __forceinline__ void pair_preload_a(uint4 (&ra)[CP_RA][2], const uint4* __restrict__ w, int kh, int ch, int lane) {
#pragma unroll
  for (int u0 = 0; u0 < CP_RA - 1; ++u0)
#pragma unroll
    for (int s_ = 0; s_ < 2; ++s_) ra[u0][s_] = w[(unsigned)((((2 * kh) * 9 + u0) * 2 + ch) * 2 + s_) * 64u + lane];
}

template <int NT, int GRP, int PL, int PITCH, typename MidFn, typename EndFn>
__device__ __forceinline__ void pair_kloop(f32x16 (&acc)[3], uint4 (&ra)[CP_RA][2], const uint4* __restrict__ w, const unsigned char* bbase,
                                           const int (&li)[3], int kh, int ch, int lane, MidFn&& mid_fn, EndFn&& end_fn) {
  const int h = lane >> 5;
  uint4 rb[2][3][2];
#define CP_LOAD_A(SET, U)                                                                              \
  _Pragma("unroll") for (int s_ = 0; s_ < 2; ++s_)                                                     \
    ra[SET][s_] = w[(unsigned)((((2 * kh + (U) / 9) * 9 + (U) % 9) * 2 + ch) * 2 + s_) * 64u + lane];
#define CP_LOAD_B(SET, U)                                                                              \
  _Pragma("unroll") for (int nt_ = 0; nt_ < NT; ++nt_)                                                 \
    _Pragma("unroll") for (int s_ = 0; s_ < 2; ++s_)                                                   \
      rb[SET][nt_][s_] = *reinterpret_cast<const uint4*>(                                              \
          bbase + (2 * (2 * kh + (U) / 9) + h) * GRP + s_ * PL + (li[nt_] + (((U) % 9) / 3 - 1) * PITCH + (((U) % 9) % 3 - 1)) * 16);
#define CP_MFMA1(SA, SETA, SB, SETB)                                                                   \
  _Pragma("unroll") for (int nt_ = 0; nt_ < NT; ++nt_)                                                 \
    acc[nt_] = __builtin_amdgcn_mfma_f32_32x32x16_f16(__builtin_bit_cast(f16x8, ra[SETA][SA]),         \
                                                      __builtin_bit_cast(f16x8, rb[SETB][nt_][SB]), acc[nt_], 0, 0, 0);
#pragma unroll
  for (int cc = 0; cc < 2; ++cc) {
    CP_LOAD_B((cc * 9) & 1, cc * 9)
#pragma unroll
    for (int tap = 0; tap < 9; ++tap) {
      const int u = cc * 9 + tap;
      if (u + CP_RA - 1 < 18) { CP_LOAD_A((u + CP_RA - 1) % CP_RA, u + CP_RA - 1) }
      if (tap + 1 < 9) { CP_LOAD_B((u + 1) & 1, u + 1) }
      __builtin_amdgcn_sched_barrier(0);
      CP_MFMA1(0, u % CP_RA, 1, u & 1) CP_MFMA1(1, u % CP_RA, 0, u & 1) CP_MFMA1(0, u % CP_RA, 0, u & 1)
      mid_fn(cc, tap);
      __builtin_amdgcn_sched_barrier(0);
    }
    end_fn(cc);
  }
#undef CP_LOAD_A
#undef CP_LOAD_B
#undef CP_MFMA1
}

template <int EPI, int NT>
__device__ __forceinline__ void pair_layer2(const PairArgs& a, unsigned char* smem, float* smem_f, int y0, int x0, int T0, int ng2, int ch,
                                            int kh, int lane, float smi, uint4 (&ra)[CP_RA][2]) {
  const int j = lane & 31, h = lane >> 5;
  const int Wp = a.W + 2, HWp = (a.H + 2) * Wp;
  int lo[3] = {0, 0, 0}, poff[3] = {0, 0, 0};
  bool ok[3] = {false, false, false};
#pragma unroll
  for (int nt = 0; nt < NT; ++nt) {
    const int oy = 2 * (T0 + nt) + (j >> 4), c = cp_lane_col(j), ox = c - 1;
    lo[nt] = (oy + 1) * CP_MIDP + c + 1;
    const int y = y0 + oy, x = x0 + ox;
    ok[nt] = ox >= 0 && ox < CP_TW && y < a.H && x < a.W;
    const int yc = y < a.H ? y : a.H - 1, xc = x < 0 ? 0 : (x < a.W ? x : a.W - 1);
    poff[nt] = (yc + 1) * Wp + (xc + 1);
  }
  f32x16 acc[3];
#pragma unroll
  for (int nt = 0; nt < 3; ++nt)
#pragma unroll
    for (int r = 0; r < 16; ++r) acc[nt][r] = 0.f;
  pair_kloop<NT, CP_GRP_MID, CP_PL_MID, CP_MIDP>(acc, ra, a.wB, smem + CP_MID_OFF, lo, kh, ch, lane, [](int, int) {}, [](int) {});
  {
    const float f = smi * a.winvB;
#pragma unroll
    for (int nt = 0; nt < NT; ++nt)
#pragma unroll
      for (int r = 0; r < 16; ++r) acc[nt][r] *= f;
  }
  typedef PairSplit<NT> S;
  const int KHu = __builtin_amdgcn_readfirstlane(kh);
  const int poA = KHu ? poff[1] : poff[0], poB = poff[2];
  const bool okA = KHu ? ok[1] : ok[0], okB = ok[2];
  float4 eo[6];
#pragma unroll
  for (int i = 0; i < S::NQ; ++i) {
    const int q = KHu ? S::keep_quad(1, i) : S::keep_quad(0, i);
    const int c0 = ch * 32 + q * 8 + 4 * h;
    const int po = i < 4 ? poA : poB;
    eo[i] = EPI == 1 ? ld4(a.auxB + ((size_t)(c0 >> 3) * HWp + po) * 8 + (c0 & 7)) : ld4(a.biasB + c0);
  }
  float* red = smem_f + ((ng2 * 2 + ch) * 2) * 1536 + lane * 4;
  float4 v[6];
  if (KHu) pair_exchange<NT, 1>(acc, v, red + 1536, red);
  else pair_exchange<NT, 0>(acc, v, red, red + 1536);
#pragma unroll
  for (int i = 0; i < S::NQ; ++i) {
    const int q = KHu ? S::keep_quad(1, i) : S::keep_quad(0, i);
    const int c0 = ch * 32 + q * 8 + 4 * h;
    const int po = i < 4 ? poA : poB;
    const bool st = i < 4 ? okA : okB;
    float4 r = v[i];
    if (EPI == 1) {
      r.x *= lrelu_grad_from_out(eo[i].x); r.y *= lrelu_grad_from_out(eo[i].y);
      r.z *= lrelu_grad_from_out(eo[i].z); r.w *= lrelu_grad_from_out(eo[i].w);
    } else {
      r.x = lrelu(r.x + eo[i].x); r.y = lrelu(r.y + eo[i].y); r.z = lrelu(r.z + eo[i].z); r.w = lrelu(r.w + eo[i].w);
    }
    if (st) st4(a.out + ((size_t)(c0 >> 3) * HWp + po) * 8 + (c0 & 7), r);
  }
}

template <int EPI, bool DBG>
__global__ void __launch_bounds__(512)
conv3x3_pair_kernel(PairArgs a) {
  unsigned long long t_start = 0, t_pro = 0, t_l1 = 0, t_mid = 0, t_ex = 0, t_mx = 0;
  if (DBG) t_start = __builtin_amdgcn_s_memtime();
  LEMO_DYN_SMEM(smem_f);
  unsigned char* smem = reinterpret_cast<unsigned char*>(smem_f);
  float* wmax = reinterpret_cast<float*>(smem + CP_WMAX_OFF);
  const int tid = (int)threadIdx.x, lane = tid & 63, wave = tid >> 6;
  const int j = lane & 31, h = lane >> 5;
  const int ng = wave & 1, ch = (wave >> 1) & 1, kh = wave >> 2;
  const int H = a.H, W = a.W, Wp = W + 2, HWp = (H + 2) * Wp;
  const unsigned in_gstride = (unsigned)HWp * 8u;
  int tile = (int)blockIdx.x;
  {
    const int q = a.ntiles >> 3, r = a.ntiles & 7, xcd = tile & 7, k = tile >> 3;
    tile = (xcd < r ? xcd * (q + 1) : r * (q + 1) + (xcd - r) * q) + k;
  }
  const int ty = tile / a.ntx, tx = tile - ty * a.ntx;
  const int y0 = ty * CP_TH, x0 = tx * CP_TW;

  uint4 ra[CP_RA][2];
  pair_preload_a(ra, a.wA, kh, ch, lane);

  unsigned offB[CP_NSLOT];
  int dstB[CP_NSLOT];
#pragma unroll
  for (int k = 0; k < CP_NSLOT; ++k) {
    int c0 = tid + k * 512;
    c0 = c0 < 4 * 2 * CP_NIN ? c0 : 4 * 2 * CP_NIN - 1;
    const int gg = c0 / (2 * CP_NIN), c = c0 - gg * (2 * CP_NIN);
    const int px = c >> 1, half = c & 1;
    const int r = px / CP_INW, col = px - r * CP_INW;
    int gy = y0 - 2 + r, gx = x0 - 2 + col;
    gy = (gy < -1 ? -1 : (gy > H ? H : gy)) + 1;
    gx = (gx < -1 ? -1 : (gx > W ? W : gx)) + 1;
    const int g0 = (gg >> 1) * 4 + (gg & 1);
    offB[k] = (unsigned)g0 * in_gstride + (unsigned)(gy * Wp + gx) * 8u + 4u * half;
    dstB[k] = g0 * CP_GRP_IN + px * 16 + 8 * half;
  }
  float4 stB[CP_NSLOT];
#pragma unroll
  for (int k = 0; k < CP_NSLOT; ++k) stB[k] = ld4(a.in + offB[k]);
  if (tid < CP_MIDH * 2 * 16) {
    const int pl = tid / (CP_MIDH * 2), rc = tid - pl * (CP_MIDH * 2);
    *reinterpret_cast<uint4*>(smem + CP_MID_OFF + pl * CP_PL_MID + ((rc >> 1) * CP_MIDP + (rc & 1) * (CP_MIDP - 1)) * 16) = make_uint4(0u, 0u, 0u, 0u);
  }
  float sc[2] = {1.f, 1.f}, sci[2] = {1.f, 1.f};
  {
    float m = 0.f;
#pragma unroll
    for (int k = 0; k < CP_NSLOT; ++k) m = absmax4(stB[k], m);
    m = wave_max(m);
    if (lane == 0) wmax[wave] = m;
    __syncthreads();
    float mm = 0.f;
#pragma unroll
    for (int i = 0; i < 8; ++i) mm = fmaxf(mm, wmax[i]);
    f16_scale_for(mm, sc[0], sci[0]);
  }
#pragma unroll
  for (int k = 0; k < CP_NSLOT; ++k) {
    uint2 s0, s1;
    split2x4(stB[k], sc[0], s0, s1);
    *reinterpret_cast<uint2*>(smem + dstB[k]) = s0;
    *reinterpret_cast<uint2*>(smem + dstB[k] + CP_PL_IN) = s1;
  }
#pragma unroll
  for (int k = 0; k < CP_NSLOT; ++k) stB[k] = ld4(a.in + 2u * in_gstride + offB[k]);
  __syncthreads();
  if (DBG) t_pro = __builtin_amdgcn_s_memtime();

  int li[3];
#pragma unroll
  for (int nt = 0; nt < 3; ++nt) {
    const int my = 2 * (3 * ng + nt) + (j >> 4), mx = cp_lane_col(j);
    li[nt] = (my + 1) * CP_INW + mx + 1;
  }
  f32x16 acc[3];
#pragma unroll
  for (int nt = 0; nt < 3; ++nt)
#pragma unroll
    for (int r = 0; r < 16; ++r) acc[nt][r] = 0.f;
  pair_kloop<3, CP_GRP_IN, CP_PL_IN, CP_INW>(
      acc, ra, a.wA, smem, li, kh, ch, lane,
      [&](int cc, int tap) {
        if (cc != 0) return;
        if (tap == 0) {
          float m = 0.f;
#pragma unroll
          for (int k = 0; k < CP_NSLOT; ++k) m = absmax4(stB[k], m);
          m = wave_max(m);
          if (lane == 0) wmax[8 + wave] = m;
        }
        if (tap == 1) {
          __syncthreads();
          float mm = 0.f;
#pragma unroll
          for (int i = 0; i < 8; ++i) mm = fmaxf(mm, wmax[8 + i]);
          f16_scale_after(mm, sc[0], sc[1], sci[1]);
        }
#pragma unroll
        for (int k = 0; k < CP_NSLOT; ++k) {
          if (2 + (7 * k) / CP_NSLOT != tap) continue;
          uint2 s0, s1;
          split2x4(stB[k], sc[1], s0, s1);
          *reinterpret_cast<uint2*>(smem + 2 * CP_GRP_IN + dstB[k]) = s0;
          *reinterpret_cast<uint2*>(smem + 2 * CP_GRP_IN + dstB[k] + CP_PL_IN) = s1;
        }
      },
      [&](int cc) {
        __syncthreads();
        if (cc == 0) {
          const float f = sc[1] * sci[0];
#pragma unroll
          for (int nt = 0; nt < 3; ++nt)
#pragma unroll
            for (int r = 0; r < 16; ++r) acc[nt][r] *= f;
        }
      });
  if (DBG) t_l1 = __builtin_amdgcn_s_memtime();
  pair_preload_a(ra, a.wB, kh, ch, lane);
  {
    const float f = sci[1] * a.winvA;
#pragma unroll
    for (int nt = 0; nt < 3; ++nt)
#pragma unroll
      for (int r = 0; r < 16; ++r) acc[nt][r] *= f;
  }

  const int KHu = __builtin_amdgcn_readfirstlane(kh);
  typedef PairSplit<3> S3;
  int mp0, mp1, mpoff0, mpoff1;
  bool inimg0, inimg1, inner0, inner1;
  {
    auto geom = [&](int t, int& p_, int& poff_, bool& inimg_, bool& inner_) {
      const int my = 2 * (3 * ng + t) + (j >> 4), mx = cp_lane_col(j);
      const int y = y0 - 1 + my, x = x0 - 1 + mx;
      p_ = my * CP_MIDP + mx + 1;
      inimg_ = (unsigned)y < (unsigned)H && (unsigned)x < (unsigned)W;
      inner_ = inimg_ && my >= 1 && my <= CP_TH && mx >= 1 && mx <= CP_TW;
      const int yc = y < 0 ? 0 : (y >= H ? H - 1 : y), xc = x < 0 ? 0 : (x >= W ? W - 1 : x);
      poff_ = (yc + 1) * Wp + (xc + 1);
    };
    geom(KHu, mp0, mpoff0, inimg0, inner0);
    geom(2, mp1, mpoff1, inimg1, inner1);
  }
  float4 eo[6];
#pragma unroll
  for (int i = 0; i < 6; ++i) {
    const int q = KHu ? S3::keep_quad(1, i) : S3::keep_quad(0, i);
    const int c0 = ch * 32 + q * 8 + 4 * h;
    const int po = i < 4 ? mpoff0 : mpoff1;
    eo[i] = EPI == 1 ? ld4(a.auxA + ((size_t)(c0 >> 3) * HWp + po) * 8 + (c0 & 7)) : ld4(a.biasA + c0);
  }
  float4 v[6];
  {
    float* red = smem_f + ((ng * 2 + ch) * 2) * 1536 + lane * 4;
    if (KHu) pair_exchange<3, 1>(acc, v, red + 1536, red);
    else pair_exchange<3, 0>(acc, v, red, red + 1536);
  }
  if (DBG) t_ex = __builtin_amdgcn_s_memtime();
  float mloc = 0.f;
#pragma unroll
  for (int i = 0; i < 6; ++i) {
    const bool in_i = i < 4 ? inimg0 : inimg1;
    float4 r = v[i];
    if (EPI == 1) {
      r.x *= lrelu_grad_from_out(eo[i].x); r.y *= lrelu_grad_from_out(eo[i].y);
      r.z *= lrelu_grad_from_out(eo[i].z); r.w *= lrelu_grad_from_out(eo[i].w);
    } else {
      r.x = lrelu(r.x + eo[i].x); r.y = lrelu(r.y + eo[i].y); r.z = lrelu(r.z + eo[i].z); r.w = lrelu(r.w + eo[i].w);
    }
    if (!in_i) r = make_float4(0.f, 0.f, 0.f, 0.f);
    v[i] = r;
    mloc = absmax4(r, mloc);
  }
  mloc = wave_max(mloc);
  if (lane == 0) wmax[16 + wave] = mloc;
  __syncthreads();
  float sm, smi;
  {
    float mm = 0.f;
#pragma unroll
    for (int i = 0; i < 8; ++i) mm = fmaxf(mm, wmax[16 + i]);
    f16_scale_for(mm, sm, smi);
  }
  if (DBG) t_mx = __builtin_amdgcn_s_memtime();
#pragma unroll
  for (int i = 0; i < 6; ++i) {
    const int q = KHu ? S3::keep_quad(1, i) : S3::keep_quad(0, i);
    uint2 s0, s1;
    split2x4(v[i], sm, s0, s1);
    unsigned char* d = smem + CP_MID_OFF + (ch * 4 + q) * CP_GRP_MID + (i < 4 ? mp0 : mp1) * 16 + 8 * h;
    *reinterpret_cast<uint2*>(d) = s0;
    *reinterpret_cast<uint2*>(d + CP_PL_MID) = s1;
  }
  __syncthreads();
  if (DBG) t_mid = __builtin_amdgcn_s_memtime();

  const int ng2 = __builtin_amdgcn_readfirstlane(ng ^ kh);
  if (ng2) pair_layer2<EPI, 2>(a, smem, smem_f, y0, x0, 3, 1, ch, kh, lane, smi, ra);
  else pair_layer2<EPI, 3>(a, smem, smem_f, y0, x0, 0, 0, ch, kh, lane, smi, ra);
  if (EPI != 1) {
#pragma unroll
    for (int i = 0; i < 6; ++i) {
      const int q = KHu ? S3::keep_quad(1, i) : S3::keep_quad(0, i);
      const int c0 = ch * 32 + q * 8 + 4 * h;
      if (i < 4 ? inner0 : inner1) st4(a.mid + ((size_t)(c0 >> 3) * HWp + (i < 4 ? mpoff0 : mpoff1)) * 8 + (c0 & 7), v[i]);
    }
  }
  if (DBG && lane == 0) {
    unsigned long long* r = a.dbg + ((size_t)blockIdx.x * 8 + wave) * 8;
    r[0] = __builtin_amdgcn_s_getreg(63492);
    r[1] = t_ex;
    r[2] = t_start; r[3] = __builtin_amdgcn_s_memtime(); r[4] = t_pro; r[5] = t_l1; r[6] = t_mid; r[7] = t_mx;
  }
}

int conv_pair_init() {
  static LdsOptinOnce once;
  return lds_optin(once, {{&conv3x3_pair_kernel<0, false>, CP_SMEM}, {&conv3x3_pair_kernel<1, false>, CP_SMEM}, {&conv3x3_pair_kernel<0, true>, CP_SMEM}});
}

bool conv3x3_pair_supported(int H, int W, int c0, int c1, int c2) {
  return c0 == 64 && c1 == 64 && c2 == 64 && H >= 1 && W >= 1 && (long)H * W <= (1l << 24);
}

int conv3x3_pair_f16(const float* in, const void* wA, float winvA, const float* biasA, const float* auxA, float* mid, const void* wB,
                     float winvB, const float* biasB, const float* auxB, float* out, int H, int W, int epi, hipStream_t s,
                     unsigned long long* dbg) {
  if (!conv3x3_pair_supported(H, W, 64, 64, 64) || (epi != 0 && epi != 1)) return LEMO_ERR_SHAPE;
  if (!in || !wA || !wB || !out || !(winvA > 0.f) || !(winvB > 0.f)) return LEMO_ERR_ARG;
  if (epi == 0 ? (!biasA || !biasB || !mid) : (!auxA || !auxB)) return LEMO_ERR_ARG;
  if (dbg && epi != 0) return LEMO_ERR_ARG;
  if (int rc = conv_pair_init()) return rc;
  PairArgs a{};
  a.in = in; a.wA = reinterpret_cast<const uint4*>(wA); a.wB = reinterpret_cast<const uint4*>(wB);
  a.biasA = biasA; a.biasB = biasB; a.auxA = auxA; a.auxB = auxB; a.mid = mid; a.out = out;
  a.winvA = winvA; a.winvB = winvB; a.H = H; a.W = W;
  a.ntx = (W + CP_TW - 1) / CP_TW;
  a.ntiles = a.ntx * ((H + CP_TH - 1) / CP_TH);
  a.dbg = dbg;
  if (dbg) hipLaunchKernelGGL((conv3x3_pair_kernel<0, true>), dim3(a.ntiles), dim3(512), CP_SMEM, s, a);
  else if (epi == 0) hipLaunchKernelGGL((conv3x3_pair_kernel<0, false>), dim3(a.ntiles), dim3(512), CP_SMEM, s, a);
  else hipLaunchKernelGGL((conv3x3_pair_kernel<1, false>), dim3(a.ntiles), dim3(512), CP_SMEM, s, a);
  return (int)hipGetLastError();
}

}
```

lemo_amd/csrc/enc_chain.hpp:

```cpp
#pragma once
#include "kernels.hpp"

namespace lemo {

#define ENC_CHK(e) do { int _e = (e); if (_e) return _e; } while (0)

template <class D> static inline bool enc_fused_head(const D& d) {
  return d.conv_variant >= 7 && d.conv_variant <= 10 && d.enc_ch[1] == 32 && d.enc_ch[2] == 32 && d.enc_w3[1] && d.enc_wbwd3[1];
}
template <class D> static inline bool enc_fused_head3(const D& d) {
  return d.conv_variant >= 8 && enc_fused_head(d) && d.enc_ch[3] == 64 && d.enc_w3[2];
}
template <class D> static inline bool enc_fused_tail3(const D& d) {
  return d.conv_variant >= 9 && enc_fused_head(d) && d.enc_ch[3] == 64 && d.enc_wbwd3[2];
}
template <class D> static inline int enc_bwd_l_last(const D& d) { return enc_fused_tail3(d) ? 3 : (enc_fused_head(d) ? 2 : 1); }
template <class D> static inline int enc_bwd_tail(const D& d, int cur, int H, int W, hipStream_t s) {
  if (enc_fused_tail3(d))
    return enc_tail3(d.dact[cur], d.enc_wbwd3[2], d.enc_wbwd3_inv[2], d.act[2], d.enc_wbwd3[1], d.enc_wbwd3_inv[1], d.act[1], d.enc_w[0], d.dx0, H, W, s);
  if (enc_fused_head(d)) return enc_tail(d.dact[cur], d.enc_wbwd3[1], d.enc_wbwd3_inv[1], d.act[1], d.enc_w[0], d.dx0, H, W, s);
  return conv3x3_c1_bwd(d.dact[cur], d.enc_w[0], d.dx0, H, W, d.enc_ch[1], s);
}

template <class D>
static inline int enc_layer(const D& d, int l, bool bwd, const float* src, float* dst, int H, int W, hipStream_t s) {
  const int cin = bwd ? d.enc_ch[l + 1] : d.enc_ch[l], cout = bwd ? d.enc_ch[l] : d.enc_ch[l + 1];
  const float* wt = bwd ? d.enc_wbwd[l] : d.enc_w[l];
  const float* wt2 = bwd ? d.enc_wbwd2[l] : d.enc_w2[l];
  const void* w3 = bwd ? d.enc_wbwd3[l] : d.enc_w3[l];
  const float* bias = bwd ? nullptr : d.enc_b[l];
  const float* aux = bwd ? d.act[l] : nullptr;
  const int epi = bwd ? 1 : 0;
  if (d.conv_variant == 10 && w3 && conv3x3_wino_supported(H, W, cin, cout))
    return conv3x3_wino_f16(src, w3, bwd ? d.enc_wbwd3_inv[l] : d.enc_w3_inv[l], wt, bias, aux, dst, H, W, epi, s);
  if (d.conv_variant >= 3 && w3 && conv3x3_split_supported(H, W, cin, cout))
    return conv3x3_mfma_split(src, w3, wt, bias, aux, dst, H, W, cin, cout, epi, s, nullptr, d.conv_variant >= 4 ? 2 : 3,
                              bwd ? d.enc_wbwd3_inv[l] : d.enc_w3_inv[l]);
  if (d.conv_variant >= 2 && 127 + 2 * (127 / W + 1) + 2 * (W + 2) + 3 <= 416)
    return conv3x3_mfma_lds(src, wt, wt2, bias, aux, dst, H, W, cin, cout, epi, s);
  return conv3x3_mfma(src, wt, bias, aux, dst, H, W, cin, cout, epi, d.conv_variant >= 2 ? 1 : d.conv_variant, s);
}

template <class D>
static inline int enc_chain_fwd(const D& d, int H, int W, hipStream_t s, int l_first = 1) {
  int l = l_first;
  while (l < 10) {
    if (d.conv_variant >= 5 && d.conv_variant != 10 && l + 1 < 10 && d.enc_w3[l] && d.enc_w3[l + 1] &&
        conv3x3_pair_supported(H, W, d.enc_ch[l], d.enc_ch[l + 1], d.enc_ch[l + 2])) {
      ENC_CHK(conv3x3_pair_f16(d.act[l], d.enc_w3[l], d.enc_w3_inv[l], d.enc_b[l], nullptr, d.act[l + 1],
                                                                           d.enc_w3[l + 1], d.enc_w3_inv[l + 1], d.enc_b[l + 1], nullptr, d.act[l + 2],
                                                                           H, W, 0, s, nullptr));
      l += 2;
    } else {
      ENC_CHK(enc_layer(d, l, false, d.act[l], d.act[l + 1], H, W, s));
      ++l;
    }
  }
  return 0;
}

template <class D>
static inline int enc_chain_bwd(const D& d, int H, int W, hipStream_t s, int* cur_out, int l_last = 1) {
  int cur = 0, l = 9;
  while (l >= l_last) {
    if (d.conv_variant >= 5 && d.conv_variant != 10 && l - 1 >= l_last && d.enc_wbwd3[l] && d.enc_wbwd3[l - 1] &&
        conv3x3_pair_supported(H, W, d.enc_ch[l + 1], d.enc_ch[l], d.enc_ch[l - 1])) {
      ENC_CHK(conv3x3_pair_f16(d.dact[cur], d.enc_wbwd3[l], d.enc_wbwd3_inv[l], nullptr, d.act[l], nullptr,
                                                                           d.enc_wbwd3[l - 1], d.enc_wbwd3_inv[l - 1], nullptr, d.act[l - 1],
                                                                           d.dact[1 - cur], H, W, 1, s, nullptr));
      l -= 2;
    } else {
      ENC_CHK(enc_layer(d, l, true, d.dact[cur], d.dact[1 - cur], H, W, s));
      --l;
    }
    cur = 1 - cur;
  }
  *cur_out = cur;
  return 0;
}

}
```

lemo_amd/csrc/kernels.hpp:

```cpp
#pragma once
#include "common.hpp"
#include "lemo_hip.h"

#include <cmath>
#include <initializer_list>
#include <mutex>

namespace lemo {

struct LdsOptin {
  const void* fn;
  int bytes;
  template <typename F> LdsOptin(F* kernel, int b) : fn(reinterpret_cast<const void*>(kernel)), bytes(b) {}
};
struct LdsOptinOnce { std::once_flag flag[64]; int rc[64]; };
int lds_optin(LdsOptinOnce& once, std::initializer_list<LdsOptin> tab);
int lds_init_all();
int conv_lds_init();
int conv_split_init();
int conv_pair_init();
int conv_wino_init();
int enc_tail3_init();
int lbs_init();
int ae_conv_init();

static inline double lr_decimal(float lr) {
  if (!(lr > 0.f) || !std::isfinite(lr)) return (double)lr;
  const double k = std::pow(10.0, 5.0 - std::floor(std::log10((double)lr)));
  const double d = std::nearbyint((double)lr * k) / k;
  return (float)d == lr ? d : (double)lr;
}

int conv3x3_mfma(const float* in, const float* wt, const float* bias, const float* aux, float* out,
                 int H, int W, int cin, int cout, int epi, int variant, hipStream_t s);
int conv3x3_mfma_splitk(const float* in, const float* wt, const float* bias, const float* aux, float* out, float* partial, int ks,
                        int H, int W, int cin, int cout, int epi, hipStream_t s);
int conv3x3_mfma_lds(const float* in, const float* wt, const float* wt2, const float* bias, const float* aux, float* out,
                     int H, int W, int cin, int cout, int epi, hipStream_t s, unsigned long long* dbg = nullptr);
bool conv3x3_split_supported(int H, int W, int cin, int cout);
int conv3x3_mfma_split(const float* in, const void* w3, const float* wt, const float* bias, const float* aux, float* out,
                       int H, int W, int cin, int cout, int epi, hipStream_t s, unsigned long long* dbg = nullptr, int pieces = 3,
                       float winv = 1.f);
bool conv3x3_pair_supported(int H, int W, int c0, int c1, int c2);
int conv3x3_pair_f16(const float* in, const void* wA, float winvA, const float* biasA, const float* auxA, float* mid, const void* wB,
                     float winvB, const float* biasB, const float* auxB, float* out, int H, int W, int epi, hipStream_t s,
                     unsigned long long* dbg = nullptr);
bool conv3x3_wino_supported(int H, int W, int cin, int cout);
int conv3x3_wino_f16(const float* in, const void* wU, float winv, const float* wt, const float* bias, const float* aux, float* out,
                     int H, int W, int epi, hipStream_t s, unsigned long long* dbg = nullptr);
int conv3x3_c1(const float* x0, const float* w, const float* bias, float* out, int H, int W, int cout, hipStream_t s);
int conv3x3_c1_bwd(const float* dpre, const float* w, float* dx0, int H, int W, int cout, hipStream_t s);

int sp_wgrad_init();
int wgrad3x3_batched_ws_floats(int H, int W, int bs, int ca, int cb);
int wgrad3x3_batched(const float* A, size_t a_stride, const float* B, size_t b_stride, int bs, int H, int W, int ca, int cb,
                     int bias_b, float* ws, float* gw, float* gb, hipStream_t s);
int dec_end_lpart_floats(int H, int W, int bs);
int dec_end_fwd(const float* u, size_t u_stride, const float* w8, const float* b8, const float* w9, const float* b9, float* r1,
                float* rec, const float* x0, float* drec, float gscale, float* lpart, float* ctr, double lr, int bs, int H, int W,
                hipStream_t s);
int dec_end_bwd(const float* drec, const float* w9, const float* r1, float* dpre8, const float* w8, const float* u, size_t u_stride,
                float* du, int bs, int H, int W, hipStream_t s);
struct SpPackJob { float* wt; float* wt2; int src, cin, cout, trans, first; };
#define SP_MAX_PACK 40
struct SpPackJobs { SpPackJob j[SP_MAX_PACK]; int n, total; };
int sp_repack(const SpPackJobs& J, const float* theta, hipStream_t s);
int sp_pad(const float* x, float* x0, int bs, int H, int W, hipStream_t s);
int sp_add(float* dst, const float* src, size_t n, hipStream_t s);
int sp_losses(const float* lpart, int nl, const float* spart, int ns, double n_rec, double n_smooth, float w_rec, float w_smooth,
              float* losses, hipStream_t s);
int sp_adam(float* theta, float* m, float* v, const float* g, const float* ctr, int n, hipStream_t s);
int smooth_loss_blocks(int H, int W, int C);
int smooth_loss(const float* z, float* dpre, float* partial, int H, int W, int C, float coef2, hipStream_t s,
                double* acc = nullptr);

int gemm_nt16(const float* A, int lda, const float* B, int ldb, int M, int N, int K, float* C, int ldc,
              const float* bias, const float* aux, int ldaux, int epi, hipStream_t s);

int gemm_nt16_splitk_part_floats(int M, int S);
int gemm_nt16_splitk_partials(const float* A, int lda, const float* B, int ldb, int M, int N, int K, float* part, int S, hipStream_t s,
                              const float* A_grouped = nullptr);
int gemm_nt16_splitk(const float* A, int lda, const float* B, int ldb, int M, int N, int K, float* C, int ldc, float* part, int S,
                     hipStream_t s, const float* A_grouped = nullptr);
int gemm_nt16_kg8(const float* A, int lda, const float* Xg, int rows, int M, int N, int K, float* C, int ldc, hipStream_t s);

typedef lemo_vposer_w VPoserW;
typedef lemo_body_const BodyConst;
typedef lemo_pose_in PoseIn;
typedef lemo_pose_ws PoseWs;
typedef lemo_pose_grad_in PoseGradIn;
typedef lemo_pose_grad_out PoseGradOut;
typedef lemo_skin_const SkinConst;
typedef lemo_vertex_set_bwd VertexSetBwd;
typedef lemo_fit_const FitConst;
struct DvertsIn {
  const float* verts; int nrows; const float* target; const float* contact; const float* dx0; const float* canon;
  const float* weights; int B;
  int Bn;
};
struct FitFuse { FitConst fc; DvertsIn in; const double* acc; double smooth_count; float* losses_out; };

int vposer_decode_fwd(const VPoserW& w, const float* z, int z_stride, int B, float* h1, float* h2, float* o,
                      float* matrot , float* aa , hipStream_t s);
int vposer_decode_bwd(const VPoserW& w, const float* h1, const float* h2, const float* o, const float* matrot,
                      const float* d_aa, const float* d_matrot, int B, float* dz, int dz_stride, float* scratch ,
                      hipStream_t s);
constexpr int VP_HIDDEN = 512, VP_OUT_PAD = 128;
static inline float* vposer_scratch_dout(float* scratch, int) { return scratch; }
static inline float* vposer_scratch_dh2(float* scratch, int B) { return scratch + (size_t)B * VP_OUT_PAD; }
static inline float* vposer_scratch_dh1(float* scratch, int B) { return scratch + (size_t)B * (VP_OUT_PAD + VP_HIDDEN); }
int vposer_mlp_bwd(const VPoserW& w, const float* h1, const float* h2, int B, float* dz, int dz_stride, float* scratch,
                   hipStream_t s);
int rot6d_to_aa_fwd(const float* x6, int stride, int N, float* aa, hipStream_t s);
int rot6d_to_aa_bwd(const float* x6, int stride, const float* d_aa, int N, float* dx6, hipStream_t s);
int smplx_pose_fwd(const BodyConst& c, const PoseIn& in, const PoseWs& ws, int B, hipStream_t s);
int smplx_pose_bwd(const BodyConst& c, const PoseWs& ws, const PoseGradIn& gi, const PoseGradOut& go, int B, hipStream_t s);

int lbs_verts_fwd_active(const SkinConst& c, const VertexSetBwd& u, const float* Xg, int Bp, const float* A, int nj,
                         const float* transl, int B, float* blend, float* verts, float* v_posed, hipStream_t s, float* transl_copy = nullptr);
int lbs_verts_fwd(const SkinConst& c, const float* Xg, int Bp, const float* A, int nj, const float* transl,
                  const int* ids, int n, int B, float* verts, float* v_posed, hipStream_t s, unsigned long long* dbg = nullptr,
                  const unsigned short* XgS = nullptr, int max_blocks_x = 0 );
bool lbs_verts_bwd_fusable(const SkinConst& c, const VertexSetBwd& u, int nj);
int lbs_verts_bwd(const SkinConst& c, const VertexSetBwd& u, const float* A, int nj, const float* v_posed, int vp_rows,
                  const float* dverts , int B, int Bp, float* dvp ,
                  float* dA , float* dtransl , float* dX , hipStream_t s, const FitFuse* fuse = nullptr);
int joints_assemble(const float* Jtr, int nj, const float* verts, int vrows, const int* extra_rows, int n_extra,
                    const int* lmk_rows , const float* lmk_bary, int n_lmk, const float* transl,
                    int B, float* joints , hipStream_t s);

int sdf_sample(const float* sdf, int D, int H, int W, const float* pts, int N, const float* gmin ,
               const float* gmax , float* val, float* dval, hipStream_t s);

int maxpool3s2_fwd(const float* in, int H, int W, float* out, unsigned char* idx, int C, hipStream_t s, int nclip = 1, size_t cs = 0);
int maxpool3s2_bwd(const float* dout, const unsigned char* idx, const float* act, float* din, int H, int W, int C, hipStream_t s,
                   int nclip = 1, size_t cs = 0);
int stuff2_fwd(const float* in, int h, int w, float* out, int H, int W, int C, hipStream_t s, int nclip = 1, size_t cs = 0);
int stuff2_bwd(const float* dout, int H, int W, const float* act, float* din, int h, int w, int C, hipStream_t s);
int conv3x3_wgrad_nslab(int H, int W);
int conv3x3_wgrad_partial(const float* dy, const float* x, int H, int W, int cin, int cout, float* partial, hipStream_t s);
int conv3x3_wgrad_reduce_multi(const lemo_wgrad_job* jobs, int n, hipStream_t s);
int conv3x3_wgrad(const float* dy, const float* x, int H, int W, int cin, int cout, int cin_real, int cout_real,
                  float* partial, float* dw, float* db, hipStream_t s);
int adam_flat(float* p, const float* g, float* m, float* v, int n, float lr, int step, int* step_dev, hipStream_t s);

int marker_c1(const FitConst& fc, const float* verts, int nrows, const float* Jtr, int nj, const float* transl, int B,
              const float* w, const float* bias, float* x0, float* canon, float* out, int cout, hipStream_t s);
int enc_head(const FitConst& fc, const float* verts, int nrows, const float* Jtr, int nj, const float* transl, int B, const float* w0,
             const float* b0, const void* w1pack, float w1inv, const float* b1, float* x0, float* canon, float* act1, float* act2,
             hipStream_t s);
int enc_head3(const FitConst& fc, const float* verts, int nrows, const float* Jtr, int nj, const float* transl, int B, const float* w0,
              const float* b0, const void* w1pack, float w1inv, const float* b1, const void* w2pack, float w2inv, const float* b2,
              float* x0, float* canon, float* act1, float* act2, float* act3, hipStream_t s);
int enc_tail(const float* din, const void* w1bpack, float w1binv, const float* act1, const float* w0, float* dx0, int H, int W, hipStream_t s);
int enc_tail3(const float* din, const void* w2bpack, float w2binv, const float* act2, const void* w1bpack, float w1binv, const float* act1,
              const float* w0, float* dx0, int H, int W, hipStream_t s);
int marker_feature(const FitConst& fc, const float* verts, int nrows, const float* Jtr, int nj, const float* transl, int B,
                   float* x0, float* canon, hipStream_t s);
int fit_losses(const float* z, float* dpre, int H, int W, int C, float coef2, double* sm_acc, const FitConst& fc, const float* verts,
               int nrows, const float* target, const float* contact, const float* shape, const float* other, int B, double* acc,
               hipStream_t s);
int vertex_loss_accumulate(const FitConst& fc, const float* verts, int nrows, const float* target, const float* contact,
                           const float* shape, const float* other, int B, double* acc, hipStream_t s);
int loss_finalize(const double* acc, int B, int n67, double smooth_count, const float* weights, float* losses, hipStream_t s);
int dverts_assemble(const FitConst& fc, const float* verts, int nrows, const float* target, const float* contact,
                    const float* dx0, const float* canon, const float* weights, const double* acc, double smooth_count,
                    float* losses, int B, float* dverts, hipStream_t s, int Bn = 0);
struct FitTail {
  const float *w1, *w1t, *b1;
  const float* dh1;
  float* g_other;
  float* h1;
  float *transl, *rot6d, *other;
  const float *g_transl, *g_rot6d;
  float *m0, *v0, *m1, *v1, *m2, *v2;
  const float* weights;
  int* step_ctr;
  const int* step_cur;
  double lr0, lr1;
  int lr_switch;
  double lr2;
  int lr_switch2;
  float* snap;
  int* nonfinite;
  const float* losses;
  int B, do_dz, do_adam;
  int Bn;
};
int fit_tail(const FitTail& a, hipStream_t s);
int adam_step(float* transl, const float* g_transl, float* m0, float* v0, float* rot6d, const float* g_rot, float* m1,
              float* v1, float* other, const float* g_other, float* m2, float* v2, int B, const float* weights,
              int* step_ctr, const int* step_cur, float lr0, float lr1, int lr_switch, hipStream_t s, float lr2 = 0.f,
              int lr_switch2 = 0, float* snap = nullptr, int* nonfinite = nullptr, const float* losses = nullptr);

static const int STATE_MAX_JOBS = 12;
struct StateCopy {
  const float* src[STATE_MAX_JOBS];
  float* dst[STATE_MAX_JOBS];
  int n[STATE_MAX_JOBS];
  int njobs;
  const int* step_src;
  int* step_dst;
  int* nonfinite;
};
int state_copy(const StateCopy& a, hipStream_t s);

int reconstruct_global_body(const float* in, int T, int J, double rot0, float* out, hipStream_t s, const double* rot0_dev = nullptr);
int local_markers_4chan(const float* body, const float* contact, int T, int M1, float* image, double* rot0, hipStream_t s);
int decode_clip(const float* rec, const float* traj, const double* stats, const double* rot0, const float* post, int T, int J,
                float* lbl, float* markers, hipStream_t s);

}
```

lemo_amd/csrc/lemo_hip.hip:

```cpp
#include "kernels.hpp"
#include "enc_chain.hpp"

#include <new>

using namespace lemo;

#define S(x) ((hipStream_t)(x))
#define CHK(e) do { int _e = (e); if (_e) return _e; } while (0)

namespace lemo {

int lds_optin(LdsOptinOnce& once, std::initializer_list<LdsOptin> tab) {
  int dev = 0;
  if (hipGetDevice(&dev) != hipSuccess || dev < 0 || dev >= 64) return LEMO_ERR_ARG;
  std::call_once(once.flag[dev], [&] {
    int lds = 0;
    hipError_t e = hipDeviceGetAttribute(&lds, hipDeviceAttributeMaxSharedMemoryPerBlock, dev);
    for (const LdsOptin& t : tab)
      if (e == hipSuccess && t.bytes > lds) e = hipErrorInvalidValue;
    for (const LdsOptin& t : tab)
      if (e == hipSuccess) e = hipFuncSetAttribute(t.fn, hipFuncAttributeMaxDynamicSharedMemorySize, t.bytes);
    once.rc[dev] = (int)e;
  });
  return once.rc[dev];
}

int lds_init_all() {
  for (int (*init)() : {conv_lds_init, conv_split_init, conv_pair_init, conv_wino_init, enc_tail3_init, lbs_init, ae_conv_init, sp_wgrad_init})
    if (int rc = init()) return rc;
  return 0;
}

}

extern "C" {

int lemo_abi_version(void) { return 5; }
int lemo_build_flags(void) {
#ifdef LEMO_NO_PACKED_FP32
  return 1;
#else
  return 0;
#endif
}

int lemo_conv3x3_mfma(const float* in, const float* wt, const float* bias, const float* aux, float* out, int H, int W,
                      int cin, int cout, int epi, int variant, void* stream) {
  if (!in || !wt || !out || (epi != 1 && !bias) || (epi == 1 && !aux)) return LEMO_ERR_ARG;
  return conv3x3_mfma(in, wt, bias, aux, out, H, W, cin, cout, epi, variant, S(stream));
}
int lemo_conv3x3_mfma_splitk(const float* in, const float* wt, const float* bias, const float* aux, float* out,
                             float* partial, int ks, int H, int W, int cin, int cout, int epi, void* stream) {
  if (!in || !wt || !out || !partial || (epi != 1 && !bias) || (epi == 1 && !aux)) return LEMO_ERR_ARG;
  return conv3x3_mfma_splitk(in, wt, bias, aux, out, partial, ks, H, W, cin, cout, epi, S(stream));
}
int lemo_conv3x3_mfma_lds(const float* in, const float* wt, const float* wt2, const float* bias, const float* aux,
                          float* out, int H, int W, int cin, int cout, int epi, void* stream) {
  if (!in || !wt || !wt2 || !out || (epi != 1 && !bias) || (epi == 1 && !aux)) return LEMO_ERR_ARG;
  return conv3x3_mfma_lds(in, wt, wt2, bias, aux, out, H, W, cin, cout, epi, S(stream));
}
int lemo_conv3x3_split_supported(int H, int W, int cin, int cout) { return conv3x3_split_supported(H, W, cin, cout) ? 1 : 0; }
int lemo_conv3x3_mfma_split(const float* in, const void* w3, const float* wt, const float* bias, const float* aux,
                            float* out, int H, int W, int cin, int cout, int epi, void* stream) {
  if (!in || !w3 || !wt || !out || (epi != 1 && !bias) || (epi == 1 && !aux)) return LEMO_ERR_ARG;
  return conv3x3_mfma_split(in, w3, wt, bias, aux, out, H, W, cin, cout, epi, S(stream));
}
int lemo_conv3x3_mfma_split_census(const float* in, const void* w3, const float* wt, const float* bias, float* out,
                                   int H, int W, int cin, int cout, unsigned long long* dbg, void* stream) {
  if (!in || !w3 || !wt || !bias || !out || !dbg) return LEMO_ERR_ARG;
  return conv3x3_mfma_split(in, w3, wt, bias, nullptr, out, H, W, cin, cout, 0, S(stream), dbg);
}
int lemo_conv3x3_mfma_split_f16(const float* in, const void* w2, float winv, const float* wt, const float* bias, const float* aux,
                                float* out, int H, int W, int cin, int cout, int epi, void* stream) {
  if (!in || !w2 || !wt || !out || (epi != 1 && !bias) || (epi == 1 && !aux)) return LEMO_ERR_ARG;
  return conv3x3_mfma_split(in, w2, wt, bias, aux, out, H, W, cin, cout, epi, S(stream), nullptr, 2, winv);
}
int lemo_conv3x3_wino_supported(int H, int W, int cin, int cout) { return conv3x3_wino_supported(H, W, cin, cout) ? 1 : 0; }
int lemo_conv3x3_wino_f16(const float* in, const void* wU, float winv, const float* wt, const float* bias, const float* aux, float* out,
                          int H, int W, int epi, unsigned long long* dbg, void* stream) {
  return conv3x3_wino_f16(in, wU, winv, wt, bias, aux, out, H, W, epi, S(stream), dbg);
}
int lemo_conv3x3_pair_supported(int H, int W, int c0, int c1, int c2) { return conv3x3_pair_supported(H, W, c0, c1, c2) ? 1 : 0; }
int lemo_conv3x3_pair_f16(const float* in, const void* wA, float winvA, const float* biasA, const float* auxA, float* mid,
                          const void* wB, float winvB, const float* biasB, const float* auxB, float* out, int H, int W, int epi,
                          unsigned long long* dbg, void* stream) {
  return conv3x3_pair_f16(in, wA, winvA, biasA, auxA, mid, wB, winvB, biasB, auxB, out, H, W, epi, S(stream), dbg);
}
int lemo_enc_head(const lemo_fit_const* fc, const float* verts, int nrows, const float* Jtr, int nj, const float* transl, int B, const float* w0,
                  const float* b0, const void* w1pack, float w1inv, const float* b1, float* x0, float* canon, float* act1, float* act2,
                  void* stream) {
  if (!fc) return LEMO_ERR_ARG;
  return enc_head(*fc, verts, nrows, Jtr, nj, transl, B, w0, b0, w1pack, w1inv, b1, x0, canon, act1, act2, S(stream));
}
int lemo_enc_tail(const float* din, const void* w1bpack, float w1binv, const float* act1, const float* w0, float* dx0, int H, int W,
                  void* stream) {
  return enc_tail(din, w1bpack, w1binv, act1, w0, dx0, H, W, S(stream));
}
int lemo_enc_tail3(const float* din, const void* w2bpack, float w2binv, const float* act2, const void* w1bpack, float w1binv, const float* act1,
                   const float* w0, float* dx0, int H, int W, void* stream) {
  return enc_tail3(din, w2bpack, w2binv, act2, w1bpack, w1binv, act1, w0, dx0, H, W, S(stream));
}
int lemo_conv3x3_mfma_split_census2(const float* in, const void* w, float winv, int pieces, const float* wt, const float* bias, float* out,
                                    int H, int W, int cin, int cout, unsigned long long* dbg, void* stream) {
  if (!in || !w || !wt || !bias || !out || !dbg) return LEMO_ERR_ARG;
  return conv3x3_mfma_split(in, w, wt, bias, nullptr, out, H, W, cin, cout, 0, S(stream), dbg, pieces, winv);
}
int lemo_conv3x3_mfma_lds_census(const float* in, const float* wt, const float* wt2, const float* bias, float* out,
                                 int H, int W, int cin, int cout, unsigned long long* dbg, void* stream) {
  if (!in || !wt || !wt2 || !out || !bias || !dbg) return LEMO_ERR_ARG;
  return conv3x3_mfma_lds(in, wt, wt2, bias, nullptr, out, H, W, cin, cout, 0, S(stream), dbg);
}
int lemo_conv3x3_c1(const float* x0, const float* w, const float* bias, float* out, int H, int W, int cout, void* stream) {
  return conv3x3_c1(x0, w, bias, out, H, W, cout, S(stream));
}
int lemo_conv3x3_c1_bwd(const float* dpre, const float* w, float* dx0, int H, int W, int cout, void* stream) {
  return conv3x3_c1_bwd(dpre, w, dx0, H, W, cout, S(stream));
}
int lemo_smooth_loss_blocks(int H, int W, int C) { return smooth_loss_blocks(H, W, C); }
int lemo_smooth_loss(const float* z, float* dpre, float* partial, int H, int W, int C, float coef2, void* stream) {
  return smooth_loss(z, dpre, partial, H, W, C, coef2, S(stream));
}

int lemo_vposer_decode_fwd(const lemo_vposer_w* w, const float* z, int z_stride, int B, float* h1, float* h2, float* o,
                           float* matrot, float* aa, void* stream) {
  if (!w || !z || !h1 || !h2 || !o) return LEMO_ERR_ARG;
  return vposer_decode_fwd(*w, z, z_stride, B, h1, h2, o, matrot, aa, S(stream));
}
int lemo_vposer_decode_bwd(const lemo_vposer_w* w, const float* h1, const float* h2, const float* o, const float* d_aa,
                           const float* d_matrot, int B, float* dz, int dz_stride, float* scratch, void* stream) {
  if (!w || !dz || !scratch || (!d_aa && !d_matrot)) return LEMO_ERR_ARG;
  return vposer_decode_bwd(*w, h1, h2, o, nullptr, d_aa, d_matrot, B, dz, dz_stride, scratch, S(stream));
}
int lemo_vposer_mlp_bwd(const lemo_vposer_w* w, const float* h1, const float* h2, int B, float* dz, int dz_stride,
                        float* scratch, void* stream) {
  if (!w || !h1 || !h2 || !dz || !scratch) return LEMO_ERR_ARG;
  return vposer_mlp_bwd(*w, h1, h2, B, dz, dz_stride, scratch, S(stream));
}
int lemo_gemm_nt16(const float* A, int lda, const float* B, int ldb, int M, int N, int K, float* C, int ldc,
                   const float* bias, const float* aux, int ldaux, int epi, void* stream) {
  if (!A || !B || !C) return LEMO_ERR_ARG;
  return gemm_nt16(A, lda, B, ldb, M, N, K, C, ldc, bias, aux, ldaux, epi, S(stream));
}
int lemo_gemm_nt16_splitk_part_floats(int M, int S) { return gemm_nt16_splitk_part_floats(M, S); }
int lemo_gemm_nt16_splitk(const float* A, int lda, const float* B, int ldb, int M, int N, int K, float* C, int ldc, float* part, int S,
                          const float* A_grouped, void* stream) {
  if (!A || !B || !C || !part) return LEMO_ERR_ARG;
  return gemm_nt16_splitk(A, lda, B, ldb, M, N, K, C, ldc, part, S, S(stream), A_grouped);
}
int lemo_rot6d_to_aa_fwd(const float* x6, int stride, int N, float* aa, void* stream) {
  return rot6d_to_aa_fwd(x6, stride, N, aa, S(stream));
}
int lemo_rot6d_to_aa_bwd(const float* x6, int stride, const float* d_aa, int N, float* dx6, void* stream) {
  return rot6d_to_aa_bwd(x6, stride, d_aa, N, dx6, S(stream));
}
int lemo_smplx_pose_fwd(const lemo_body_const* c, const lemo_pose_in* in, const lemo_pose_ws* ws, int B, void* stream) {
  if (!c || !in || !ws) return LEMO_ERR_ARG;
  return smplx_pose_fwd(*c, *in, *ws, B, S(stream));
}
int lemo_smplx_pose_bwd(const lemo_body_const* c, const lemo_pose_ws* ws, const lemo_pose_grad_in* gi,
                        const lemo_pose_grad_out* go, int B, void* stream) {
  if (!c || !ws || !gi || !go || !gi->dA) return LEMO_ERR_ARG;
  return smplx_pose_bwd(*c, *ws, *gi, *go, B, S(stream));
}
int lemo_lbs_verts_fwd_active(const lemo_skin_const* c, const lemo_vertex_set_bwd* u, const float* Xg, int Bp, const float* A,
                              int nj, const float* transl, int B, float* blend, float* verts, float* v_posed, void* stream) {
  if (!c || !u || !Xg || !A || !blend || !verts) return LEMO_ERR_ARG;
  return lbs_verts_fwd_active(*c, *u, Xg, Bp, A, nj, transl, B, blend, verts, v_posed, S(stream));
}
int lemo_lbs_verts_fwd(const lemo_skin_const* c, const float* Xg, int Bp, const float* A, int nj, const float* transl,
                       const int* ids, int n, int B, float* verts, float* v_posed, void* stream) {
  if (!c || !Xg || !A || !verts) return LEMO_ERR_ARG;
  return lbs_verts_fwd(*c, Xg, Bp, A, nj, transl, ids, n, B, verts, v_posed, S(stream));
}
int lemo_lbs_verts_fwd_xs(const lemo_skin_const* c, const float* Xg, const unsigned short* XgS, int Bp, const float* A, int nj,
                          const float* transl, const int* ids, int n, int B, float* verts, float* v_posed, void* stream) {
  if (!c || !Xg || !A || !verts) return LEMO_ERR_ARG;
  return lbs_verts_fwd(*c, Xg, Bp, A, nj, transl, ids, n, B, verts, v_posed, S(stream), nullptr, XgS);
}
int lemo_lbs_verts_fwd_census(const lemo_skin_const* c, const float* Xg, int Bp, const float* A, int nj, const float* transl,
                              int n, int B, float* verts, float* v_posed, unsigned long long* dbg, void* stream,
                              const unsigned short* XgS) {
  if (!c || !Xg || !A || !verts || !dbg) return LEMO_ERR_ARG;
  return lbs_verts_fwd(*c, Xg, Bp, A, nj, transl, nullptr, n, B, verts, v_posed, S(stream), dbg, XgS);
}
int lemo_lbs_verts_bwd(const lemo_skin_const* c, const lemo_vertex_set_bwd* u, const float* A, int nj, const float* v_posed,
                       int vp_rows, const float* dverts, int B, int Bp, float* dvp, float* dA, float* dtransl, float* dX,
                       void* stream) {
  if (!c || !u || !A || !v_posed || !dverts || !dvp || !dA || !dX) return LEMO_ERR_ARG;
  return lbs_verts_bwd(*c, *u, A, nj, v_posed, vp_rows, dverts, B, Bp, dvp, dA, dtransl, dX, S(stream));
}
int lemo_joints_assemble(const float* Jtr, int nj, const float* verts, int vrows, const int* extra_rows, int n_extra,
                         const int* lmk_rows, const float* lmk_bary, int n_lmk, const float* transl, int B, float* joints,
                         void* stream) {
  return joints_assemble(Jtr, nj, verts, vrows, extra_rows, n_extra, lmk_rows, lmk_bary, n_lmk, transl, B, joints, S(stream));
}

int lemo_maxpool3s2_fwd(const float* in, int H, int W, float* out, unsigned char* idx, int C, void* stream) {
  if (!in || !out || !idx) return LEMO_ERR_ARG;
  return maxpool3s2_fwd(in, H, W, out, idx, C, S(stream));
}
int lemo_maxpool3s2_bwd(const float* dout, const unsigned char* idx, const float* act, float* din, int H, int W, int C, void* stream) {
  if (!dout || !idx || !din) return LEMO_ERR_ARG;
  return maxpool3s2_bwd(dout, idx, act, din, H, W, C, S(stream));
}
int lemo_stuff2_fwd(const float* in, int h, int w, float* out, int H, int W, int C, void* stream) {
  if (!in || !out) return LEMO_ERR_ARG;
  return stuff2_fwd(in, h, w, out, H, W, C, S(stream));
}
int lemo_stuff2_bwd(const float* dout, int H, int W, const float* act, float* din, int h, int w, int C, void* stream) {
  if (!dout || !din) return LEMO_ERR_ARG;
  return stuff2_bwd(dout, H, W, act, din, h, w, C, S(stream));
}
int lemo_conv3x3_wgrad_nslab(int H, int W) { return conv3x3_wgrad_nslab(H, W); }
int lemo_conv3x3_wgrad(const float* dy, const float* x, int H, int W, int cin, int cout, int cin_real, int cout_real,
                       float* partial, float* dw, float* db, void* stream) {
  if (!dy || !x || !partial || !dw) return LEMO_ERR_ARG;
  return conv3x3_wgrad(dy, x, H, W, cin, cout, cin_real, cout_real, partial, dw, db, S(stream));
}
int lemo_conv3x3_wgrad_partial(const float* dy, const float* x, int H, int W, int cin, int cout, float* partial, void* stream) {
  if (!dy || !x || !partial) return LEMO_ERR_ARG;
  return conv3x3_wgrad_partial(dy, x, H, W, cin, cout, partial, S(stream));
}
int lemo_conv3x3_wgrad_reduce_multi(const lemo_wgrad_job* jobs, int n, void* stream) {
  return conv3x3_wgrad_reduce_multi(jobs, n, S(stream));
}
int lemo_adam_flat(float* p, const float* g, float* m, float* v, int n, float lr, int step, void* stream) {
  if (!p || !g || !m || !v) return LEMO_ERR_ARG;
  return adam_flat(p, g, m, v, n, lr, step, nullptr, S(stream));
}
int lemo_adam_flat_ctr(float* p, const float* g, float* m, float* v, int n, float lr, int* step_ctr, void* stream) {
  if (!p || !g || !m || !v || !step_ctr) return LEMO_ERR_ARG;
  return adam_flat(p, g, m, v, n, lr, 0, step_ctr, S(stream));
}
int lemo_capture_begin(void* stream) {
  if (!stream) return LEMO_ERR_ARG;
  return (int)hipStreamBeginCapture(S(stream), hipStreamCaptureModeRelaxed);
}
int lemo_capture_end(void* stream, void** graph_exec) {
  if (!stream || !graph_exec) return LEMO_ERR_ARG;
  hipGraph_t g = nullptr;
  hipError_t e = hipStreamEndCapture(S(stream), &g);
  if (e != hipSuccess || !g) return e != hipSuccess ? (int)e : LEMO_ERR_STATE;
  hipGraphExec_t x = nullptr;
  e = hipGraphInstantiate(&x, g, nullptr, nullptr, 0);
  (void)hipGraphDestroy(g);
  if (e != hipSuccess) return (int)e;
  *graph_exec = (void*)x;
  return 0;
}
int lemo_graph_launch(void* graph_exec, void* stream) {
  if (!graph_exec) return LEMO_ERR_ARG;
  return (int)hipGraphLaunch((hipGraphExec_t)graph_exec, S(stream));
}
int lemo_graph_destroy(void* graph_exec) {
  if (!graph_exec) return 0;
  return (int)hipGraphExecDestroy((hipGraphExec_t)graph_exec);
}
#ifdef LEMO_CENSUS
extern "C" int lemo_census_set_pose(unsigned long long*);
extern "C" int lemo_census_set_lbs(unsigned long long*);
extern "C" int lemo_census_set(unsigned long long* buf) { return lemo_census_set_pose(buf) | lemo_census_set_lbs(buf); }
#endif
int lemo_sdf_sample(const float* sdf, int D, int H, int W, const float* pts, int N, const float* gmin, const float* gmax,
                    float* val, float* dval, void* stream) {
  if (!sdf || !pts || !gmin || !gmax || !val) return LEMO_ERR_ARG;
  return sdf_sample(sdf, D, H, W, pts, N, gmin, gmax, val, dval, S(stream));
}

int lemo_reconstruct_global_body(const float* in, int T, int J, double rot_0_pivot, float* out, void* stream) {
  if (!in || !out) return LEMO_ERR_ARG;
  return reconstruct_global_body(in, T, J, rot_0_pivot, out, S(stream));
}
int lemo_reconstruct_global_body_dev(const float* in, int T, int J, const double* rot_0_pivot, float* out, void* stream) {
  if (!in || !out || !rot_0_pivot) return LEMO_ERR_ARG;
  return reconstruct_global_body(in, T, J, 0.0, out, S(stream), rot_0_pivot);
}
int lemo_decode_clip(const float* rec, const float* traj, const double* stats, const double* rot_0_pivot, const float* post, int T,
                     int J, float* contact_lbl, float* markers, void* stream) {
  if (!rec || !traj || !stats || !rot_0_pivot || !contact_lbl || !markers) return LEMO_ERR_ARG;
  return decode_clip(rec, traj, stats, rot_0_pivot, post, T, J, contact_lbl, markers, S(stream));
}
int lemo_local_markers_4chan(const float* body, const float* contact, int T, int M1, float* image, double* rot_0_pivot,
                             void* stream) {
  if (!body || !contact || !image || !rot_0_pivot) return LEMO_ERR_ARG;
  return local_markers_4chan(body, contact, T, M1, image, rot_0_pivot, S(stream));
}

static const int FIT_MAXG = 20;

struct FitSide { hipStream_t side = nullptr; hipEvent_t fork = nullptr, join = nullptr; bool pending = false; };
struct FitEngine {
  lemo_fit_desc d;
  hipGraphExec_t exec[FIT_MAXG + 1] = {};
  int head = 5;
  FitSide fs;
};

static int fit_iteration(const lemo_fit_desc& d, hipStream_t s, bool first, bool last, FitSide* fs);

static int capture_iterations(FitEngine* e, hipStream_t s, int iters, hipGraphExec_t* out) {
  hipGraph_t g = nullptr;
  CHK((int)hipStreamBeginCapture(s, hipStreamCaptureModeThreadLocal));
  int rc = 0;
  for (int i = 0; i < iters && !rc; ++i) rc = fit_iteration(e->d, s, i == 0, i == iters - 1, &e->fs);
  const int ec = (int)hipStreamEndCapture(s, &g);
  if (rc) { if (g) (void)hipGraphDestroy(g); return rc; }
  CHK(ec);
  const int ic = (int)hipGraphInstantiate(out, g, nullptr, nullptr, 0);
  (void)hipGraphDestroy(g);
  if (!ic) (void)hipGraphUpload(*out, s);
  return ic;
}

static int fit_graphs(FitEngine* e, hipStream_t s, int n, bool launch) {
  int open[2] = {0, 0}, left = n;
  if (e->head > 0) {
    if (left > 0) { open[0] = 1; left -= 1; }
    if (left > 0) { open[1] = left < e->head ? left : (e->head < FIT_MAXG ? e->head : FIT_MAXG); left -= open[1]; }
  }
  const int nfull = left / FIT_MAXG, rem = left - nfull * FIT_MAXG;
  const int need[4] = {open[0], open[1], nfull ? FIT_MAXG : 0, rem};
  for (int i = 0; i < 4; ++i)
    if (need[i] && !e->exec[need[i]]) CHK(capture_iterations(e, s, need[i], &e->exec[need[i]]));
  if (!launch) return 0;
  for (int i = 0; i < 2; ++i) if (open[i]) CHK((int)hipGraphLaunch(e->exec[open[i]], s));
  for (int i = 0; i < nfull; ++i) CHK((int)hipGraphLaunch(e->exec[FIT_MAXG], s));
  if (rem) CHK((int)hipGraphLaunch(e->exec[rem], s));
  return 0;
}

static FitTail fit_tail_args(const lemo_fit_desc& d, bool dz, bool adam, bool h1) {
  FitTail a{};
  a.w1 = d.vposer.w1; a.w1t = d.vposer.w1t; a.b1 = d.vposer.b1;
  a.dh1 = vposer_scratch_dh1(d.vp_scratch, d.B);
  a.g_other = d.g_other; a.h1 = h1 ? d.h1 : nullptr;
  a.transl = d.transl; a.rot6d = d.rot6d; a.other = d.other; a.g_transl = d.g_transl; a.g_rot6d = d.g_rot6d;
  a.m0 = d.adam_m[0]; a.v0 = d.adam_v[0]; a.m1 = d.adam_m[1]; a.v1 = d.adam_v[1]; a.m2 = d.adam_m[2]; a.v2 = d.adam_v[2];
  a.weights = d.weights; a.step_ctr = d.step_ctr; a.step_cur = d.step_cur;
  a.lr0 = lr_decimal(d.lr0); a.lr1 = lr_decimal(d.lr1); a.lr_switch = d.lr_switch; a.lr2 = lr_decimal(d.lr2); a.lr_switch2 = d.lr_switch2;
  a.snap = d.snap; a.nonfinite = d.nonfinite; a.losses = d.losses;
  a.B = d.B; a.do_dz = dz; a.do_adam = adam;
  a.Bn = d.per_frame ? 1 : d.B;
  return a;
}

#define FIT_SIDE_BLOCKS 125
static int fit_side_launch(const lemo_fit_desc& d, hipStream_t s) {
  static const int blocks = getenv("LEMO_FIT_SIDE_BLOCKS") ? atoi(getenv("LEMO_FIT_SIDE_BLOCKS")) : FIT_SIDE_BLOCKS;
  return lbs_verts_fwd(d.skin, d.pose.Xg, d.Bp, d.pose.A, d.body.nj, d.transl_side, nullptr, d.V, d.B, d.verts_side, nullptr, s, nullptr, d.pose.XgS,
                       blocks);
}
static int fit_side_join(FitSide* fs, hipStream_t s) {
  if (!fs || !fs->pending) return 0;
  fs->pending = false;
  return fs->side ? (int)hipStreamWaitEvent(s, fs->join, 0) : 0;
}

static int fit_forward(const lemo_fit_desc& d, hipStream_t s, bool finalize, bool compute_h1 = true, unsigned stages = ~0u, FitSide* fs = nullptr) {
  const int B = d.B, nj = d.body.nj;
  const int H = 3 * d.fit.n81 + 2, W = B - 1 + 16;
  if (stages & 1u) {
  if (compute_h1) CHK(fit_tail(fit_tail_args(d, false, false, true), s));
  CHK(gemm_nt16(d.vposer.w2, 512, d.h1, 512, 512, B, 512, d.h2, 512, d.vposer.b2, nullptr, 0, 1, s));
  CHK(gemm_nt16(d.vposer.w3, 512, d.h2, 512, 128, B, 512, d.vo, 128, d.vposer.b3, nullptr, 0, 2, s));
  lemo_pose_in in{};
  in.rot6d = d.rot6d; in.vposer_o = d.vo; in.go_out = d.go_aa;
  in.lh = d.other + 32; in.rh = d.other + 44; in.hand_stride = 56;
  in.betas = d.shape; in.betas_stride = 10;
  in.zero_f64 = d.loss_acc; in.n_zero = 512; in.step_ctr = d.step_ctr; in.step_cur = d.step_cur;
  in.nonfinite = d.nonfinite;
  CHK(fit_side_join(fs, s));
  CHK(smplx_pose_fwd(d.body, in, d.pose, B, s));
  }
  if (stages & 2u) {
  if (d.full_vertices) CHK(lbs_verts_fwd(d.skin, d.pose.Xg, d.Bp, d.pose.A, nj, d.transl, nullptr, d.V, B, d.verts, d.v_posed, s, nullptr, d.pose.XgS));
  else if (d.uset.DkT && d.uset.n == d.fit.n)
    CHK(lbs_verts_fwd_active(d.skin, d.uset, d.pose.Xg, d.Bp, d.pose.A, nj, d.transl, B, d.dvp, d.verts, d.v_posed, s, d.verts_side ? d.transl_side : nullptr));
  else {
    CHK(lbs_verts_fwd(d.skin, d.pose.Xg, d.Bp, d.pose.A, nj, d.transl, d.fwd_ids, d.fit.n, B, d.verts, d.v_posed, s, nullptr, d.pose.XgS));
    if (d.verts_side && !d.full_vertices) CHK((int)hipMemcpyAsync(d.transl_side, d.transl, sizeof(float) * 3 * B, hipMemcpyDeviceToDevice, s));
  }
  if (d.verts_side && !d.full_vertices && !fs) CHK(fit_side_launch(d, s));
  }
  if (d.per_frame) {
    CHK(vertex_loss_accumulate(d.fit, d.verts, d.nrows, d.target, d.contact, d.shape, d.other, B, d.loss_acc, s));
    if (finalize) CHK(loss_finalize(d.loss_acc, B, d.fit.n67, 1.0, d.weights, d.losses, s));
    return 0;
  }
  if (stages & 4u) {
  if (enc_fused_head3(d))
    CHK(enc_head3(d.fit, d.verts, d.nrows, d.pose.Jtr, nj, d.transl, B, d.enc_w[0], d.enc_b[0], d.enc_w3[1], d.enc_w3_inv[1], d.enc_b[1], d.enc_w3[2],
                  d.enc_w3_inv[2], d.enc_b[2], d.x0, d.canon, d.act[1], d.act[2], d.act[3], s));
  else if (enc_fused_head(d))
    CHK(enc_head(d.fit, d.verts, d.nrows, d.pose.Jtr, nj, d.transl, B, d.enc_w[0], d.enc_b[0], d.enc_w3[1], d.enc_w3_inv[1], d.enc_b[1], d.x0, d.canon,
                 d.act[1], d.act[2], s));
  else
    CHK(marker_c1(d.fit, d.verts, d.nrows, d.pose.Jtr, nj, d.transl, B, d.enc_w[0], d.enc_b[0], d.x0, d.canon, d.act[1], d.enc_ch[1], s));
  CHK(enc_chain_fwd(d, H, W, s, enc_fused_head3(d) ? 3 : (enc_fused_head(d) ? 2 : 1)));
  }
  const double cnt = (double)d.enc_ch[10] * H * (W - 1);
  const float coef2 = (float)((double)d.weights_host[5] * 2.0 / cnt);
  if (stages & 8u)
  CHK(fit_losses(d.act[10], d.dact[0], H, W, d.enc_ch[10], coef2, d.loss_acc + 9, d.fit, d.verts, d.nrows, d.target, d.contact,
                 d.shape, d.other, B, d.loss_acc, s));
  if (finalize) CHK(loss_finalize(d.loss_acc, B, d.fit.n67, cnt, d.weights, d.losses, s));
  return 0;
}

static int fit_backward(const lemo_fit_desc& d, hipStream_t s, bool update = false, bool next_h1 = false, unsigned stages = ~0u, FitSide* fs = nullptr) {
  const int B = d.B, nj = d.body.nj;
  const int H = 3 * d.fit.n81 + 2, W = B - 1 + 16;
  const double cnt = d.per_frame ? 1.0 : (double)d.enc_ch[10] * H * (W - 1);
  int cur = 0;
  if (d.per_frame || !(stages & 16u)) goto vertex_stage;
  CHK(enc_chain_bwd(d, H, W, s, &cur, enc_bwd_l_last(d)));
  CHK(enc_bwd_tail(d, cur, H, W, s));
  if (fs && d.verts_side && !d.full_vertices) {
    if (fs->side) {
      CHK((int)hipEventRecord(fs->fork, s));
      CHK((int)hipStreamWaitEvent(fs->side, fs->fork, 0));
      CHK(fit_side_launch(d, fs->side));
      CHK((int)hipEventRecord(fs->join, fs->side));
    } else CHK(fit_side_launch(d, s));
    fs->pending = true;
  }
vertex_stage:
  if (!(stages & 32u)) goto pose_stage;
  if (lbs_verts_bwd_fusable(d.skin, d.uset, nj) && d.fit.n == d.uset.n) {
    const FitFuse ff{d.fit, DvertsIn{d.verts, d.nrows, d.target, d.contact, d.dx0, d.canon, d.weights, B, d.per_frame ? 1 : B}, d.loss_acc, cnt, d.losses};
    CHK(lbs_verts_bwd(d.skin, d.uset, d.pose.A, nj, d.v_posed, d.nrows, nullptr, B, d.Bp, d.dvp, d.dA, d.g_transl, d.dX, s, &ff));
  } else {
    CHK(dverts_assemble(d.fit, d.verts, d.nrows, d.target, d.contact, d.dx0, d.canon, d.weights, d.loss_acc, cnt, d.losses, B, d.dverts, s, d.per_frame ? 1 : B));
    CHK(lbs_verts_bwd(d.skin, d.uset, d.pose.A, nj, d.v_posed, d.nrows, d.dverts, B, d.Bp, d.dvp, d.dA, d.g_transl, d.dX, s));
  }
pose_stage:
  if (!(stages & 64u)) return 0;
  lemo_pose_grad_in gi{d.dA, nullptr, d.dX};
  lemo_pose_grad_out go{};
  go.d_lh = d.g_other + 32; go.d_rh = d.g_other + 44; go.hand_stride = 56;
  go.rot6d = d.rot6d; go.d_rot6d = d.g_rot6d;
  go.vposer_o = d.vo; go.d_vposer_o = d.vp_scratch;
  CHK(smplx_pose_bwd(d.body, d.pose, gi, go, B, s));
  CHK(vposer_mlp_bwd(d.vposer, d.h1, d.h2, B, nullptr, 56, d.vp_scratch, s));
  CHK(fit_tail(fit_tail_args(d, true, update, update && next_h1), s));
  return 0;
}

static int fit_iteration(const lemo_fit_desc& d, hipStream_t s, bool first, bool last, FitSide* fs) {
  const bool side = d.verts_side && !d.full_vertices && !d.per_frame;
  CHK(fit_forward(d, s, false, first, ~0u, side ? fs : nullptr));
  if (side && !fs) return LEMO_ERR_STATE;
  CHK(fit_backward(d, s, true, !last, ~0u, side ? fs : nullptr));
  if (last) CHK(fit_side_join(fs, s));
  return 0;
}

void* lemo_fit_create(const lemo_fit_desc* d) {
  if (!d || d->B < (d->per_frame ? 1 : 10) || d->B > d->Bp || !d->verts || !d->transl) return nullptr;
  if (lds_init_all()) return nullptr;
  if (d->pose.XgS && (d->skin.DgH != nullptr) != (d->pose.xgs_f16 != 0)) return nullptr;
  FitEngine* e = new (std::nothrow) FitEngine();
  if (e) {
    e->d = *d;
    if (d->per_frame) e->head = 0;
    if (const char* h = getenv("LEMO_FIT_HEAD")) e->head = atoi(h);
    if (d->verts_side && !d->full_vertices) {
      if (!d->transl_side || d->per_frame) { delete e; return nullptr; }
      if (hipStreamCreateWithPriority(&e->fs.side, hipStreamNonBlocking, getenv("LEMO_FIT_SIDE_PRIO") ? atoi(getenv("LEMO_FIT_SIDE_PRIO")) : 0) != hipSuccess ||
          hipEventCreateWithFlags(&e->fs.fork, hipEventDisableTiming) != hipSuccess ||
          hipEventCreateWithFlags(&e->fs.join, hipEventDisableTiming) != hipSuccess) { lemo_fit_destroy(e); return nullptr; }
    }
  }
  return e;
}

void lemo_fit_destroy(void* h) {
  FitEngine* e = (FitEngine*)h;
  if (!e) return;
  for (int l = 0; l <= FIT_MAXG; ++l) if (e->exec[l]) (void)hipGraphExecDestroy(e->exec[l]);
  if (e->fs.fork) (void)hipEventDestroy(e->fs.fork);
  if (e->fs.join) (void)hipEventDestroy(e->fs.join);
  if (e->fs.side) { (void)hipStreamSynchronize(e->fs.side); (void)hipStreamDestroy(e->fs.side); }
  delete e;
}

int lemo_fit_forward(void* h, void* stream) {
  FitEngine* e = (FitEngine*)h;
  if (!e) return LEMO_ERR_ARG;
  return fit_forward(e->d, S(stream), true);
}

int lemo_fit_backward(void* h, void* stream) {
  FitEngine* e = (FitEngine*)h;
  if (!e) return LEMO_ERR_ARG;
  return fit_backward(e->d, S(stream));
}

int lemo_fit_step(void* h, int n, int use_graph, void* stream) {
  FitEngine* e = (FitEngine*)h;
  if (!e || n < 0) return LEMO_ERR_ARG;
  hipStream_t s = S(stream);
  if (!use_graph) {
    for (int i = 0; i < n; ++i) CHK(fit_iteration(e->d, s, i == 0, i == n - 1, &e->fs));
    return 0;
  }
  CHK(fit_graphs(e, s, n, false));
  return fit_graphs(e, s, n, true);
}

int lemo_fit_prepare(void* h, int n, void* stream) {
  FitEngine* e = (FitEngine*)h;
  if (!e || n < 0) return LEMO_ERR_ARG;
  return fit_graphs(e, S(stream), n, false);
}

int lemo_fit_census(void* h, int reps, float* ms_out, void* stream) {
  FitEngine* e = (FitEngine*)h;
  hipStream_t s = S(stream);
  if (!e || !ms_out || reps < 1 || !s) return LEMO_ERR_ARG;
  const lemo_fit_desc& d = e->d;
  CHK(fit_forward(d, s, true));
  CHK(fit_backward(d, s));
  hipEvent_t e0, e1;
  CHK((int)hipEventCreate(&e0));
  CHK((int)hipEventCreate(&e1));
  int rc = 0;
  for (int k = 0; k <= LEMO_FIT_NSTAGE && !rc; ++k) {
    const unsigned mask = k == LEMO_FIT_NSTAGE ? ~0u : (1u << k);
    hipGraph_t g = nullptr;
    hipGraphExec_t x = nullptr;
    rc = (int)hipStreamBeginCapture(s, hipStreamCaptureModeThreadLocal);
    for (int r = 0; r < reps && !rc; ++r) {
      if (mask & 15u) rc = fit_forward(d, s, false, true, mask);
      if (!rc && (mask & 112u)) rc = fit_backward(d, s, false, false, mask);
    }
    const int ec = (int)hipStreamEndCapture(s, &g);
    if (!rc) rc = ec;
    if (!rc) rc = (int)hipGraphInstantiate(&x, g, nullptr, nullptr, 0);
    if (g) (void)hipGraphDestroy(g);
    if (!rc) {
      rc = (int)hipGraphLaunch(x, s);
      if (!rc) rc = (int)hipEventRecord(e0, s);
      if (!rc) rc = (int)hipGraphLaunch(x, s);
      if (!rc) rc = (int)hipEventRecord(e1, s);
      if (!rc) rc = (int)hipEventSynchronize(e1);
      float ms = 0.f;
      if (!rc) rc = (int)hipEventElapsedTime(&ms, e0, e1);
      ms_out[k] = ms / (float)reps;
    }
    if (x) (void)hipGraphExecDestroy(x);
  }
  (void)hipEventDestroy(e0);
  (void)hipEventDestroy(e1);
  if (!rc) rc = fit_forward(d, s, true);
  if (!rc) rc = fit_backward(d, s);
  return rc;
}

static int fit_state_io(FitEngine* e, const lemo_fit_state* st, bool load, hipStream_t s) {
  if (!e || !st || !st->transl || !st->rot6d || !st->other || !st->step) return LEMO_ERR_ARG;
  const lemo_fit_desc& d = e->d;
  if (!d.rot6d || !d.other || !d.step_ctr) return LEMO_ERR_STATE;
  StateCopy a{};
  float* eng[9] = {d.transl, d.rot6d, d.other, d.adam_m[0], d.adam_m[1], d.adam_m[2], d.adam_v[0], d.adam_v[1], d.adam_v[2]};
  float* usr[9] = {st->transl, st->rot6d, st->other, st->adam_m[0], st->adam_m[1], st->adam_m[2], st->adam_v[0], st->adam_v[1], st->adam_v[2]};
  const int width[3] = {3, 6, 56};
  for (int i = 0; i < 9; ++i) {
    if (!eng[i] || !usr[i]) return LEMO_ERR_ARG;
    a.src[i] = load ? usr[i] : eng[i];
    a.dst[i] = load ? eng[i] : usr[i];
    a.n[i] = d.B * width[i % 3];
  }
  a.njobs = 9;
  a.step_src = load ? st->step : d.step_ctr;
  a.step_dst = load ? d.step_ctr : st->step;
  a.nonfinite = load ? d.nonfinite : nullptr;
  return state_copy(a, s);
}
int lemo_fit_load_state(void* h, const lemo_fit_state* st, void* stream) { return fit_state_io((FitEngine*)h, st, true, S(stream)); }
int lemo_fit_save_state(void* h, const lemo_fit_state* st, void* stream) { return fit_state_io((FitEngine*)h, st, false, S(stream)); }

}
```

lemo_amd/csrc/loss_device.hpp:

```cpp
#pragma once
#include "kernels.hpp"

namespace lemo {

__device__ __forceinline__ int reflect_idx(int i, int n) { return i < 0 ? -i : (i >= n ? 2 * (n - 1) - i : i); }

__device__ __forceinline__ void canonical_frame(const float* verts, int nrows, const int* row81, const float* Jtr,
                                                int nj, const float* transl, float* canon, const float* cam2world = nullptr) {
  float j1[3], j2[3];
  for (int k = 0; k < 3; ++k) {
    const float tr = transl ? transl[k] : 0.f;
    j1[k] = Jtr[3 * 1 + k] + tr;
    j2[k] = Jtr[3 * 2 + k] + tr;
  }
  if (cam2world) {
    float w1[3], w2[3];
    for (int i = 0; i < 3; ++i) {
      w1[i] = cam2world[3 * i] * j1[0] + cam2world[3 * i + 1] * j1[1] + cam2world[3 * i + 2] * j1[2] + cam2world[9 + i];
      w2[i] = cam2world[3 * i] * j2[0] + cam2world[3 * i + 1] * j2[1] + cam2world[3 * i + 2] * j2[2] + cam2world[9 + i];
    }
    for (int i = 0; i < 3; ++i) { j1[i] = w1[i]; j2[i] = w2[i]; }
  }
  (void)nj;
  float xx = j2[0] - j1[0], xy = j2[1] - j1[1];
  const float nx = sqrtf(xx * xx + xy * xy);
  xx /= nx; xy /= nx;
  float yx = -xy, yy = xx;
  const float ny = sqrtf(yx * yx + yy * yy);
  yx /= ny; yy /= ny;
  canon[0] = xx; canon[1] = yx; canon[2] = 0.f;
  canon[3] = xy; canon[4] = yy; canon[5] = 0.f;
  canon[6] = 0.f; canon[7] = 0.f; canon[8] = 1.f;
  if (cam2world) {
    float m[9];
    for (int k = 0; k < 3; ++k)
      for (int c = 0; c < 3; ++c)
        m[3 * k + c] = cam2world[k] * canon[c] + cam2world[3 + k] * canon[3 + c] + cam2world[6 + k] * canon[6 + c];
    for (int e = 0; e < 9; ++e) canon[e] = m[e];
  }
  const float* m0 = verts + (size_t)row81[0] * 3;
  (void)nrows;
  canon[9] = m0[0]; canon[10] = m0[1]; canon[11] = m0[2];
}



#define LEMO_SMOOTH_ITEMS 4
__device__ __forceinline__ void smooth_loss_body(int blk, const float* __restrict__ z, float* __restrict__ dpre, float* __restrict__ partial,
                                                 int H, int W, int C, float coef2, double* __restrict__ acc) {
  __shared__ float red[4];
  const int Wp = W + 2, HWp = (H + 2) * Wp, P = H * W;
  const int n = P * (C >> 3) * 2;
  float sq = 0.f;
  float4 cv[LEMO_SMOOTH_ITEMS], lv[LEMO_SMOOTH_ITEMS], rv[LEMO_SMOOTH_ITEMS];
  size_t ov[LEMO_SMOOTH_ITEMS];
  bool hasl[LEMO_SMOOTH_ITEMS], hasr[LEMO_SMOOTH_ITEMS], valid[LEMO_SMOOTH_ITEMS];
#pragma unroll
  for (int k = 0; k < LEMO_SMOOTH_ITEMS; ++k) {
    const int idx = (blk * LEMO_SMOOTH_ITEMS + k) * (int)blockDim.x + (int)threadIdx.x;
    valid[k] = idx < n;
    const int ic = valid[k] ? idx : n - 1;
    const int half = ic & 1, rest = ic >> 1;
    const int g = rest / P, p = rest - g * P;
    const int y = p / W, x = p - y * W;
    ov[k] = ((size_t)g * HWp + (y + 1) * Wp + (x + 1)) * 8 + 4 * half;
    hasl[k] = x >= 1; hasr[k] = x <= W - 2;
    cv[k] = ld4(z + ov[k]);
    lv[k] = ld4(z + ov[k] - 8);
    rv[k] = ld4(z + ov[k] + 8);
  }
#pragma unroll
  for (int k = 0; k < LEMO_SMOOTH_ITEMS; ++k) {
    const float4 c = cv[k], l = lv[k], r = rv[k];
    float4 gr = make_float4(0.f, 0.f, 0.f, 0.f);
    if (hasl[k]) { gr.x += c.x - l.x; gr.y += c.y - l.y; gr.z += c.z - l.z; gr.w += c.w - l.w; }
    if (hasr[k]) {
      const float d0 = r.x - c.x, d1 = r.y - c.y, d2 = r.z - c.z, d3 = r.w - c.w;
      if (valid[k]) sq += d0 * d0 + d1 * d1 + d2 * d2 + d3 * d3;
      gr.x -= d0; gr.y -= d1; gr.z -= d2; gr.w -= d3;
    }
    if (valid[k])
      st4(dpre + ov[k], make_float4(coef2 * gr.x * lrelu_grad_from_out(c.x), coef2 * gr.y * lrelu_grad_from_out(c.y),
                                    coef2 * gr.z * lrelu_grad_from_out(c.z), coef2 * gr.w * lrelu_grad_from_out(c.w)));
  }
  const float s = block_sum(sq, red);
  if (threadIdx.x == 0) {
    if (acc) atomicAdd(acc + (blk & 31) * 16, (double)s);
    else partial[blk] = s;
  }
}

__device__ __forceinline__ void vertex_loss_body(int b, FitConst fc, const float* __restrict__ verts, int nrows, const float* __restrict__ target,
                              const float* __restrict__ contact, const float* __restrict__ shape,
                              const float* __restrict__ other, int B, double* __restrict__ accg) {
  __shared__ float red[4][12];
  const int t = threadIdx.x;
  float acc[12];
  for (int i = 0; i < 12; ++i) acc[i] = 0.f;
  for (int w = t; w < fc.n67 * 3; w += 256) {
    const int m = w / 3, c = w % 3;
    acc[0] += fabsf(verts[((size_t)b * nrows + fc.row67[m]) * 3 + c] - target[((size_t)b * fc.n67 + m) * 3 + c]);
  }
  if (b < B - 1) {
    for (int k = 0; k < 4; ++k) {
      if (contact[(size_t)b * 4 + k] != 1.f) continue;
      for (int q = fc.foot_start[k] + t; q < fc.foot_start[k + 1]; q += 256) {
        const float* v0 = verts + ((size_t)b * nrows + fc.foot_row[q]) * 3;
        const float* v1 = v0 + (size_t)nrows * 3;
        const float vx = (v1[0] - v0[0]) * 30.f, vy = (v1[1] - v0[1]) * 30.f, vz = (v1[2] - v0[2]) * 30.f;
        const float sp = sqrtf(vx * vx + vy * vy + vz * vz);
        if (sp - 0.1f > 0.f) { acc[1 + k] += sp; acc[5 + k] += 1.f; }
      }
    }
  }
  if (t < 32) { const float v = other[(size_t)b * 56 + t]; acc[9] = v * v; }
  else if (t >= 64 && t < 74) { const float v = shape[(size_t)b * 10 + (t - 64)]; acc[10] = v * v; }
  else if (t >= 128 && t < 152) { const float v = other[(size_t)b * 56 + 32 + (t - 128)]; acc[11] = v * v; }
#pragma unroll
  for (int i = 0; i < 12; ++i) acc[i] = wave_sum(acc[i]);
  if ((t & 63) == 0) {
#pragma unroll
    for (int i = 0; i < 12; ++i) red[t >> 6][i] = acc[i];
  }
  __syncthreads();
  if (t < 12) {
    const float v = ((red[0][t] + red[1][t]) + red[2][t]) + red[3][t];
    if (v != 0.f) atomicAdd(accg + (b & 31) * 16 + (t < 9 ? t : t + 1), (double)v);
  }
}

__device__ __forceinline__ void finalize_losses(const double* tot, int B, int n67, double smooth_count,
                                                const float* weights, float* losses) {
  const float l_marker = (float)(tot[0] / ((double)B * n67 * 3));
  float l_contact = 0.f;
  for (int k = 0; k < 4; ++k) {
    const double cnt = tot[5 + k];
    const float part = cnt >= 1.0 ? (float)(tot[1 + k] / cnt) : 0.f;
    l_contact = l_contact + part;
    losses[8 + k] = cnt >= 1.0 ? (float)(1.0 / cnt) : 0.f;
  }
  const float l_smooth = (float)(tot[9] / smooth_count);
  const float l_vposer = (float)(tot[10] / ((double)B * 32));
  const float l_shape = (float)(tot[11] / ((double)B * 10));
  const float l_hand = (float)(tot[12] / ((double)B * 24));
  float total = weights[0] * l_marker + weights[1] * l_vposer;
  total = total + weights[2] * l_shape;
  total = total + weights[3] * l_hand;
  total = total + weights[4] * l_contact;
  total = total + weights[5] * l_smooth;
  losses[0] = l_marker; losses[1] = l_vposer; losses[2] = l_shape; losses[3] = l_hand;
  losses[4] = l_contact; losses[5] = l_smooth; losses[6] = total; losses[7] = 0.f;
}


__device__ __forceinline__ double loss_slot_total(const double* __restrict__ acc, int i) {
  double v = 0.0;
  for (int sl = 0; sl < 32; ++sl) v += acc[sl * 16 + i];
  return v;
}


struct DvIdx { int row, m67, fm, m81; };
__device__ __forceinline__ DvIdx dverts_indices(const FitConst& fc, int u) {
  DvIdx ix;
  ix.row = fc.u_row[u]; ix.m67 = fc.u_m67[u]; ix.fm = fc.u_foot_mask[u]; ix.m81 = fc.u_m81[u];
  return ix;
}

struct DvRegs {
  float p[3], pn[3], pm[3], tgv[3], xstd[3], ct[4], ctm[4], cn[9], wm, wc;
  float dx[3][2][4];
  bool on[3][2][4];
  bool fast;
  int m67, fm, m81;
};

__device__ __forceinline__ void dverts_load(const FitConst& fc, const DvertsIn& in, int b, const DvIdx ix, DvRegs& r) {
  const float* __restrict__ verts = in.verts; const float* __restrict__ target = in.target;
  const float* __restrict__ contact = in.contact; const float* __restrict__ dx0 = in.dx0;
  const float* __restrict__ canon = in.canon; const float* __restrict__ weights = in.weights;
  const int nrows = in.nrows, B = in.B;
  const int D = 3 * fc.n81, W = B - 1 + 16, nd = B - 1;
  const int row = ix.row, m67 = ix.m67, fm = ix.fm, m81 = ix.m81;
  const int bn = min(b + 1, B - 1), bp = max(b - 1, 0), bc = max(min(b, B - 2), 0);
  const float* v = verts + ((size_t)b * nrows + row) * 3;
  const float* v1 = verts + ((size_t)bn * nrows + row) * 3;
  const float* vm = verts + ((size_t)bp * nrows + row) * 3;
  const float* tg = target + ((size_t)b * fc.n67 + max(m67, 0)) * 3;
#pragma unroll
  for (int c = 0; c < 3; ++c) { r.p[c] = v[c]; r.pn[c] = v1[c]; r.pm[c] = vm[c]; r.tgv[c] = tg[c]; r.xstd[c] = fc.Xstd[3 * max(m81, 0) + c]; }
#pragma unroll
  for (int k = 0; k < 4; ++k) { r.ct[k] = contact[(size_t)bc * 4 + k]; r.ctm[k] = contact[(size_t)bp * 4 + k]; }
#pragma unroll
  for (int e = 0; e < 9; ++e) r.cn[e] = canon[e];
  r.wm = weights[0] / ((float)in.Bn * fc.n67 * 3); r.wc = weights[4];
  r.fast = D >= 5 && nd >= 18;
  r.m67 = m67; r.fm = fm; r.m81 = m81;
  if (r.fast) {
#pragma unroll
    for (int c = 0; c < 3; ++c) {
      const int d = 3 * max(m81, 0) + c;
      const int yA = d + 1, yB = d == 1 ? 0 : (d == D - 2 ? D + 1 : -1);
#pragma unroll
      for (int side = 0; side < 2; ++side) {
        const int tp = side == 0 ? b - 1 : b;
        const bool tv = tp >= 0 && tp <= nd - 1;
        const int tq = min(max(tp, 0), nd - 1);
        const int xA = tq + 8, xB = (tq >= 1 && tq <= 8) ? 8 - tq : ((tq >= nd - 9 && tq <= nd - 2) ? 2 * (nd - 1) - tq + 8 : -1);
        r.on[c][side][0] = tv;               r.on[c][side][1] = tv && xB >= 0;
        r.on[c][side][2] = tv && yB >= 0;    r.on[c][side][3] = tv && yB >= 0 && xB >= 0;
        const int yb = yB >= 0 ? yB : yA, xb = xB >= 0 ? xB : xA;
        r.dx[c][side][0] = dx0[(size_t)yA * W + xA]; r.dx[c][side][1] = dx0[(size_t)yA * W + xb];
        r.dx[c][side][2] = dx0[(size_t)yb * W + xA]; r.dx[c][side][3] = dx0[(size_t)yb * W + xb];
      }
    }
  }
}

__device__ __forceinline__ void dverts_compute(const FitConst& fc, const DvertsIn& in, const float* losses, int b, const DvRegs& r,
                                               float& gx_out, float& gy_out, float& gz_out) {
  const float* __restrict__ dx0 = in.dx0;
  const int B = in.B, D = 3 * fc.n81, W = B - 1 + 16, nd = B - 1;
  const int m67 = r.m67, fm = r.fm, m81 = r.m81;
  const float wm = r.wm, wc = r.wc;
  const bool fast = r.fast;
  float gx = 0.f, gy = 0.f, gz = 0.f;
  if (m67 >= 0) {
    const float d0 = r.p[0] - r.tgv[0], d1 = r.p[1] - r.tgv[1], d2 = r.p[2] - r.tgv[2];
    gx += wm * (d0 > 0.f ? 1.f : (d0 < 0.f ? -1.f : 0.f));
    gy += wm * (d1 > 0.f ? 1.f : (d1 < 0.f ? -1.f : 0.f));
    gz += wm * (d2 > 0.f ? 1.f : (d2 < 0.f ? -1.f : 0.f));
  }
  if (fm) {
#pragma unroll
    for (int k = 0; k < 4; ++k) {
      if (!((fm >> k) & 1)) continue;
      const float coef = wc * losses[8 + k] * 30.f;
      if (b < B - 1 && r.ct[k] == 1.f) {
        const float vx = (r.pn[0] - r.p[0]) * 30.f, vy = (r.pn[1] - r.p[1]) * 30.f, vz = (r.pn[2] - r.p[2]) * 30.f;
        const float sp = sqrtf(vx * vx + vy * vy + vz * vz);
        if (sp - 0.1f > 0.f) { const float q = coef / sp; gx -= q * vx; gy -= q * vy; gz -= q * vz; }
      }
      if (b >= 1 && r.ctm[k] == 1.f) {
        const float vx = (r.p[0] - r.pm[0]) * 30.f, vy = (r.p[1] - r.pm[1]) * 30.f, vz = (r.p[2] - r.pm[2]) * 30.f;
        const float sp = sqrtf(vx * vx + vy * vy + vz * vz);
        if (sp - 0.1f > 0.f) { const float q = coef / sp; gx += q * vx; gy += q * vy; gz += q * vz; }
      }
    }
  }
  if (m81 >= 0) {
    float dg[3];
#pragma unroll
    for (int c = 0; c < 3; ++c) {
      const int d = 3 * m81 + c;
      float acc = 0.f;
      if (fast) {
#pragma unroll
        for (int side = 0; side < 2; ++side) {
          float sv = 0.f;
#pragma unroll
          for (int q = 0; q < 4; ++q) sv += r.on[c][side][q] ? r.dx[c][side][q] : 0.f;
          acc += side == 0 ? sv : -sv;
        }
      } else {
        int ys[3]; int ny = 0;
        ys[ny++] = d + 1;
        if (d == 1) ys[ny++] = 0;
        if (d == D - 2) ys[ny++] = D + 1;
        for (int side = 0; side < 2; ++side) {
          const int tp = side == 0 ? b - 1 : b;
          if (tp < 0 || tp > nd - 1) continue;
          int xs[3]; int nx = 0;
          xs[nx++] = tp + 8;
          if (tp >= 1 && tp <= 8) xs[nx++] = 8 - tp;
          if (tp >= nd - 9 && tp <= nd - 2) xs[nx++] = 2 * (nd - 1) - tp + 8;
          float sv = 0.f;
          for (int iy = 0; iy < ny; ++iy)
            for (int jx = 0; jx < nx; ++jx) sv += dx0[(size_t)ys[iy] * W + xs[jx]];
          acc += side == 0 ? sv : -sv;
        }
      }
      dg[c] = acc / r.xstd[c];
    }
    gx += r.cn[0] * dg[0] + r.cn[1] * dg[1] + r.cn[2] * dg[2];
    gy += r.cn[3] * dg[0] + r.cn[4] * dg[1] + r.cn[5] * dg[2];
    gz += r.cn[6] * dg[0] + r.cn[7] * dg[1] + r.cn[8] * dg[2];
  }
  gx_out = gx; gy_out = gy; gz_out = gz;
}

__device__ __forceinline__ void dverts_vertex(const FitConst& fc, const DvertsIn& in, const float* losses, int b, const DvIdx ix,
                                              float& gx_out, float& gy_out, float& gz_out) {
  DvRegs r;
  dverts_load(fc, in, b, ix, r);
  dverts_compute(fc, in, losses, b, r, gx_out, gy_out, gz_out);
}

}
```

Measured before the change: 3513.

## Fold loss kernels into encoder head and first backward conv pair

Removes the standalone fit_losses launch. The per-frame vertex/contact/prior losses now run as extra wave-level blocks appended to the enc_head3 grid. The smoothness loss value and its gradient are computed inside the first backward conv-pair kernel while it stages its input. This saves a kernel launch and a full read/write of the smoothness gradient buffer, at the cost of extra neighbour loads, f64 shuffles and atomics inside the conv kernel. It is enabled by default when conv_variant is 9 and the shapes fit.

```diff
diff --git a/include/lemo_hip.h b/include/lemo_hip.h
--- a/include/lemo_hip.h
+++ b/include/lemo_hip.h
@@ -36,6 +36,9 @@
 int lemo_conv3x3_pair_f16(const float* in, const void* wA, float winvA, const float* biasA, const float* auxA, float* mid,
                           const void* wB, float winvB, const float* biasB, const float* auxB, float* out, int H, int W, int epi,
                           unsigned long long* dbg, void* stream);
+int lemo_conv3x3_pair_smooth_f16(const float* z, const void* wA, float winvA, const float* auxA, const void* wB, float winvB,
+                                 const float* auxB, float* out, int H, int W, float coef2, double* sm_acc, unsigned long long* dbg,
+                                 void* stream);
 int lemo_conv3x3_wino_supported(int H, int W, int cin, int cout);
 int lemo_conv3x3_wino_f16(const float* in, const void* wU, float winv, const float* wt, const float* bias, const float* aux, float* out,
                           int H, int W, int epi, unsigned long long* dbg, void* stream);
diff --git a/lemo_amd/_hip.py b/lemo_amd/_hip.py
--- a/lemo_amd/_hip.py
+++ b/lemo_amd/_hip.py
@@ -185,6 +185,7 @@
     'lemo_conv3x3_wino_supported': (C.c_int, [C.c_int] * 4),
     'lemo_conv3x3_wino_f16': (C.c_int, [vp, vp, C.c_float, vp, vp, vp, vp, C.c_int, C.c_int, C.c_int, vp, vp]),
     'lemo_conv3x3_pair_f16': (C.c_int, [vp, vp, C.c_float, vp, vp, vp, vp, C.c_float, vp, vp, vp, C.c_int, C.c_int, C.c_int, vp, vp]),
+    'lemo_conv3x3_pair_smooth_f16': (C.c_int, [vp, vp, C.c_float, vp, vp, C.c_float, vp, vp, C.c_int, C.c_int, C.c_float, vp, vp, vp]),
     'lemo_enc_head': (C.c_int, [vp, vp, C.c_int, vp, C.c_int, vp, C.c_int, vp, vp, vp, C.c_float, vp, vp, vp, vp, vp, vp]),
     'lemo_enc_tail': (C.c_int, [vp, vp, C.c_float, vp, vp, vp, C.c_int, C.c_int, vp]),
     'lemo_enc_tail3': (C.c_int, [vp, vp, C.c_float, vp, vp, C.c_float, vp, vp, vp, C.c_int, C.c_int, vp]),
diff --git a/lemo_amd/csrc/conv_head_kernels.hip b/lemo_amd/csrc/conv_head_kernels.hip
--- a/lemo_amd/csrc/conv_head_kernels.hip
+++ b/lemo_amd/csrc/conv_head_kernels.hip
@@ -1,3 +1,4 @@
+#include <algorithm>
 #include <type_traits>
 #include "conv_f16.hpp"
 #include "loss_device.hpp"
@@ -243,7 +244,10 @@
   HeadArgs h;
   const uint4* w2; float w2inv; const float* b2;
   float* act3;
+  VertexLossRoles vl;
+  int nroles;
 };
+constexpr int H3_CUS = 256, H3_MIN_ROLES = 2, H3_MAX_ROLES = 16;
 
 __global__ void __launch_bounds__(512)
 enc_head3_kernel(Head3Args A3) {
@@ -254,6 +258,12 @@
   __shared__ float wmax[24];
   const HeadArgs& a = A3.h;
   const FitConst& fc = a.fc;
+  if ((int)blockIdx.x >= a.ntiles) {
+    const int wv = __builtin_amdgcn_readfirstlane((int)threadIdx.x >> 6);
+    for (int b = ((int)blockIdx.x - a.ntiles) * 8 + wv; b < a.B; b += A3.nroles * 8)
+      vertex_loss_wave(b, (int)threadIdx.x & 63, fc, a.verts, a.nrows, A3.vl.target, A3.vl.contact, A3.vl.shape, A3.vl.other, a.B, A3.vl.acc);
+    return;
+  }
   const int tid = (int)threadIdx.x, lane = tid & 63, wave = tid >> 6;
   const int j = lane & 31, h = lane >> 5;
   const int D = 3 * fc.n81, H = D + 2, W = a.B - 1 + 16, Wp = W + 2, HWp = (H + 2) * Wp;
@@ -465,8 +475,9 @@
 
 int enc_head3(const FitConst& fc, const float* verts, int nrows, const float* Jtr, int nj, const float* transl, int B, const float* w0,
               const float* b0, const void* w1pack, float w1inv, const float* b1, const void* w2pack, float w2inv, const float* b2,
-              float* x0, float* canon, float* act1, float* act2, float* act3, hipStream_t s) {
+              float* x0, float* canon, float* act1, float* act2, float* act3, hipStream_t s, const VertexLossRoles* roles) {
   if (B < 10 || !w1pack || !w2pack || !(w1inv > 0.f) || !(w2inv > 0.f) || !verts || !x0 || !canon || !act1 || !act2 || !act3) return LEMO_ERR_ARG;
+  if (roles && (!roles->target || !roles->contact || !roles->shape || !roles->other || !roles->acc)) return LEMO_ERR_ARG;
   const int H = 3 * fc.n81 + 2, W = B - 1 + 16;
   Head3Args A{};
   HeadArgs& a = A.h;
@@ -476,7 +487,11 @@
   a.ntx = (W + HD_TW - 1) / HD_TW;
   a.ntiles = a.ntx * ((H + HD_TH - 1) / HD_TH);
   A.w2 = reinterpret_cast<const uint4*>(w2pack); A.w2inv = w2inv; A.b2 = b2; A.act3 = act3;
-  hipLaunchKernelGGL(enc_head3_kernel, dim3(a.ntiles), dim3(512), 0, s, A);
+  if (roles) {
+    A.vl = *roles;
+    A.nroles = std::min(std::max(H3_CUS - a.ntiles, H3_MIN_ROLES), H3_MAX_ROLES);
+  }
+  hipLaunchKernelGGL(enc_head3_kernel, dim3(a.ntiles + (roles ? A.nroles : 0)), dim3(512), 0, s, A);
   return (int)hipGetLastError();
 }
 
diff --git a/lemo_amd/csrc/conv_pair_kernels.hip b/lemo_amd/csrc/conv_pair_kernels.hip
--- a/lemo_amd/csrc/conv_pair_kernels.hip
+++ b/lemo_amd/csrc/conv_pair_kernels.hip
@@ -13,6 +13,8 @@
 constexpr int CP_MID_OFF = 8 * CP_GRP_IN;
 constexpr int CP_WMAX_OFF = CP_MID_OFF + 8 * CP_GRP_MID;
 constexpr int CP_SMEM = CP_WMAX_OFF + 3 * 8 * 4;
+constexpr int CP_SSUM_OFF = CP_SMEM, CP_SMEM_SM = CP_SSUM_OFF + 8 * 8;
+static_assert(CP_SSUM_OFF % 8 == 0, "f64 slots");
 constexpr int CP_NSLOT = 4;
 static_assert(CP_MIDW == 16 && CP_NMID == 6 * 32 && CP_INW == CP_MIDP, "N-tiles = 2 rows x 16 columns on grids of row pitch 18");
 static_assert(4 * 2 * CP_NIN <= CP_NSLOT * 512 && CP_NOUT == 140, "staging slots");
@@ -29,7 +31,22 @@
   float winvA, winvB;
   int H, W, ntx, ntiles;
   unsigned long long* dbg;
+  float coef2;
+  double* sm_acc;
 };
+
+__device__ __forceinline__ float4 pair_smooth_dpre(float4 c, float4 l, float4 r, unsigned fl, float coef2, double& sq) {
+  float4 gr = make_float4(0.f, 0.f, 0.f, 0.f);
+  if (fl & 2u) { gr.x += c.x - l.x; gr.y += c.y - l.y; gr.z += c.z - l.z; gr.w += c.w - l.w; }
+  if (fl & 4u) {
+    const float d0 = r.x - c.x, d1 = r.y - c.y, d2 = r.z - c.z, d3 = r.w - c.w;
+    if (fl & 8u) sq += (double)(d0 * d0 + d1 * d1 + d2 * d2 + d3 * d3);
+    gr.x -= d0; gr.y -= d1; gr.z -= d2; gr.w -= d3;
+  }
+  if (!(fl & 1u)) return make_float4(0.f, 0.f, 0.f, 0.f);
+  return make_float4(coef2 * gr.x * lrelu_grad_from_out(c.x), coef2 * gr.y * lrelu_grad_from_out(c.y),
+                     coef2 * gr.z * lrelu_grad_from_out(c.z), coef2 * gr.w * lrelu_grad_from_out(c.w));
+}
 
 template <int NT> struct PairSplit {
   static constexpr int NQ = NT == 3 ? 6 : 4;
@@ -167,9 +184,10 @@
   }
 }
 
-template <int EPI, bool DBG>
+template <int EPI, bool DBG, bool SM = false>
 __global__ void __launch_bounds__(512)
 conv3x3_pair_kernel(PairArgs a) {
+  static_assert(!SM || EPI == 1, "the smoothness mode stages the first backward pair's input");
   unsigned long long t_start = 0, t_pro = 0, t_l1 = 0, t_mid = 0, t_ex = 0, t_mx = 0;
   if (DBG) t_start = __builtin_amdgcn_s_memtime();
   LEMO_DYN_SMEM(smem_f);
@@ -193,14 +211,21 @@
 
   unsigned offB[CP_NSLOT];
   int dstB[CP_NSLOT];
+  unsigned smfl = 0u;
 #pragma unroll
   for (int k = 0; k < CP_NSLOT; ++k) {
     int c0 = tid + k * 512;
+    const bool surplus = c0 >= 4 * 2 * CP_NIN;
     c0 = c0 < 4 * 2 * CP_NIN ? c0 : 4 * 2 * CP_NIN - 1;
     const int gg = c0 / (2 * CP_NIN), c = c0 - gg * (2 * CP_NIN);
     const int px = c >> 1, half = c & 1;
     const int r = px / CP_INW, col = px - r * CP_INW;
     int gy = y0 - 2 + r, gx = x0 - 2 + col;
+    if (SM) {
+      const bool inimg = (unsigned)gy < (unsigned)H && (unsigned)gx < (unsigned)W;
+      const bool own = inimg && !surplus && r >= 2 && r < 2 + CP_TH && col >= 2 && col < 2 + CP_TW;
+      smfl |= ((inimg ? 1u : 0u) | (inimg && gx >= 1 ? 2u : 0u) | (inimg && gx <= W - 2 ? 4u : 0u) | (own ? 8u : 0u)) << (4 * k);
+    }
     gy = (gy < -1 ? -1 : (gy > H ? H : gy)) + 1;
     gx = (gx < -1 ? -1 : (gx > W ? W : gx)) + 1;
     const int g0 = (gg >> 1) * 4 + (gg & 1);
@@ -208,13 +233,32 @@
     dstB[k] = g0 * CP_GRP_IN + px * 16 + 8 * half;
   }
   float4 stB[CP_NSLOT];
-#pragma unroll
-  for (int k = 0; k < CP_NSLOT; ++k) stB[k] = ld4(a.in + offB[k]);
+  float4 stL[SM ? CP_NSLOT : 1], stR[SM ? CP_NSLOT : 1];
+  double sq = 0.0;
+  auto sm_load = [&](unsigned gofs) {
+#pragma unroll
+    for (int k = 0; k < CP_NSLOT; ++k) {
+      stB[k] = ld4(a.in + gofs + offB[k]);
+      if (SM) {
+        const unsigned d = ((smfl >> (4 * k)) & 1u) ? 8u : 0u;
+        stL[SM ? k : 0] = ld4(a.in + gofs + offB[k] - d);
+        stR[SM ? k : 0] = ld4(a.in + gofs + offB[k] + d);
+      }
+    }
+  };
+  auto sm_dpre = [&]() {
+    if (SM) {
+#pragma unroll
+      for (int k = 0; k < CP_NSLOT; ++k) stB[k] = pair_smooth_dpre(stB[k], stL[SM ? k : 0], stR[SM ? k : 0], (smfl >> (4 * k)) & 15u, a.coef2, sq);
+    }
+  };
+  sm_load(0u);
   if (tid < CP_MIDH * 2 * 16) {
     const int pl = tid / (CP_MIDH * 2), rc = tid - pl * (CP_MIDH * 2);
     *reinterpret_cast<uint4*>(smem + CP_MID_OFF + pl * CP_PL_MID + ((rc >> 1) * CP_MIDP + (rc & 1) * (CP_MIDP - 1)) * 16) = make_uint4(0u, 0u, 0u, 0u);
   }
   float sc[2] = {1.f, 1.f}, sci[2] = {1.f, 1.f};
+  sm_dpre();
   {
     float m = 0.f;
 #pragma unroll
@@ -234,8 +278,7 @@
     *reinterpret_cast<uint2*>(smem + dstB[k]) = s0;
     *reinterpret_cast<uint2*>(smem + dstB[k] + CP_PL_IN) = s1;
   }
-#pragma unroll
-  for (int k = 0; k < CP_NSLOT; ++k) stB[k] = ld4(a.in + 2u * in_gstride + offB[k]);
+  sm_load(2u * in_gstride);
   __syncthreads();
   if (DBG) t_pro = __builtin_amdgcn_s_memtime();
 
@@ -255,6 +298,12 @@
       [&](int cc, int tap) {
         if (cc != 0) return;
         if (tap == 0) {
+          sm_dpre();
+          if (SM) {
+#pragma unroll
+            for (int o = 32; o >= 1; o >>= 1) sq += __shfl_xor(sq, o);
+            if (lane == 0) reinterpret_cast<double*>(smem + CP_SSUM_OFF)[wave] = sq;
+          }
           float m = 0.f;
 #pragma unroll
           for (int k = 0; k < CP_NSLOT; ++k) m = absmax4(stB[k], m);
@@ -267,6 +316,11 @@
 #pragma unroll
           for (int i = 0; i < 8; ++i) mm = fmaxf(mm, wmax[8 + i]);
           f16_scale_after(mm, sc[0], sc[1], sci[1]);
+          if (SM && tid == 0) {
+            const double* ws = reinterpret_cast<const double*>(smem + CP_SSUM_OFF);
+            const double t = ((ws[0] + ws[1]) + (ws[2] + ws[3])) + ((ws[4] + ws[5]) + (ws[6] + ws[7]));
+            atomicAdd(a.sm_acc + (blockIdx.x & 31) * 16, t);
+          }
         }
 #pragma unroll
         for (int k = 0; k < CP_NSLOT; ++k) {
@@ -388,7 +442,8 @@
 
 int conv_pair_init() {
   static LdsOptinOnce once;
-  return lds_optin(once, {{&conv3x3_pair_kernel<0, false>, CP_SMEM}, {&conv3x3_pair_kernel<1, false>, CP_SMEM}, {&conv3x3_pair_kernel<0, true>, CP_SMEM}});
+  return lds_optin(once, {{&conv3x3_pair_kernel<0, false>, CP_SMEM}, {&conv3x3_pair_kernel<1, false>, CP_SMEM}, {&conv3x3_pair_kernel<0, true>, CP_SMEM},
+                          {&conv3x3_pair_kernel<1, false, true>, CP_SMEM_SM}, {&conv3x3_pair_kernel<1, true, true>, CP_SMEM_SM}});
 }
 
 bool conv3x3_pair_supported(int H, int W, int c0, int c1, int c2) {
@@ -416,4 +471,21 @@
   return (int)hipGetLastError();
 }
 
-}
+int conv3x3_pair_smooth_f16(const float* z, const void* wA, float winvA, const float* auxA, const void* wB, float winvB, const float* auxB,
+                            float* out, int H, int W, float coef2, double* sm_acc, hipStream_t s, unsigned long long* dbg) {
+  if (!conv3x3_pair_supported(H, W, 64, 64, 64)) return LEMO_ERR_SHAPE;
+  if (!z || !wA || !wB || !auxA || !auxB || !out || !sm_acc || !(winvA > 0.f) || !(winvB > 0.f)) return LEMO_ERR_ARG;
+  if (int rc = conv_pair_init()) return rc;
+  PairArgs a{};
+  a.in = z; a.wA = reinterpret_cast<const uint4*>(wA); a.wB = reinterpret_cast<const uint4*>(wB);
+  a.auxA = auxA; a.auxB = auxB; a.out = out;
+  a.winvA = winvA; a.winvB = winvB; a.H = H; a.W = W;
+  a.ntx = (W + CP_TW - 1) / CP_TW;
+  a.ntiles = a.ntx * ((H + CP_TH - 1) / CP_TH);
+  a.dbg = dbg; a.coef2 = coef2; a.sm_acc = sm_acc;
+  if (dbg) hipLaunchKernelGGL((conv3x3_pair_kernel<1, true, true>), dim3(a.ntiles), dim3(512), CP_SMEM_SM, s, a);
+  else hipLaunchKernelGGL((conv3x3_pair_kernel<1, false, true>), dim3(a.ntiles), dim3(512), CP_SMEM_SM, s, a);
+  return (int)hipGetLastError();
+}
+
+}
diff --git a/lemo_amd/csrc/enc_chain.hpp b/lemo_amd/csrc/enc_chain.hpp
--- a/lemo_amd/csrc/enc_chain.hpp
+++ b/lemo_amd/csrc/enc_chain.hpp
@@ -60,11 +60,18 @@
 }
 
 template <class D>
-static inline int enc_chain_bwd(const D& d, int H, int W, hipStream_t s, int* cur_out, int l_last = 1) {
+static inline int enc_chain_bwd(const D& d, int H, int W, hipStream_t s, int* cur_out, int l_last = 1, double* sm_acc = nullptr,
+                                float coef2 = 0.f) {
   int cur = 0, l = 9;
   while (l >= l_last) {
-    if (d.conv_variant >= 5 && d.conv_variant != 10 && l - 1 >= l_last && d.enc_wbwd3[l] && d.enc_wbwd3[l - 1] &&
-        conv3x3_pair_supported(H, W, d.enc_ch[l + 1], d.enc_ch[l], d.enc_ch[l - 1])) {
+    const bool pair = d.conv_variant >= 5 && d.conv_variant != 10 && l - 1 >= l_last && d.enc_wbwd3[l] && d.enc_wbwd3[l - 1] &&
+                      conv3x3_pair_supported(H, W, d.enc_ch[l + 1], d.enc_ch[l], d.enc_ch[l - 1]);
+    if (sm_acc && l == 9) {
+      if (!pair) return LEMO_ERR_STATE;
+      ENC_CHK(conv3x3_pair_smooth_f16(d.act[10], d.enc_wbwd3[9], d.enc_wbwd3_inv[9], d.act[9], d.enc_wbwd3[8], d.enc_wbwd3_inv[8], d.act[8],
+                                      d.dact[1 - cur], H, W, coef2, sm_acc, s));
+      l -= 2;
+    } else if (pair) {
       ENC_CHK(conv3x3_pair_f16(d.dact[cur], d.enc_wbwd3[l], d.enc_wbwd3_inv[l], nullptr, d.act[l], nullptr,
                                                                            d.enc_wbwd3[l - 1], d.enc_wbwd3_inv[l - 1], nullptr, d.act[l - 1],
                                                                            d.dact[1 - cur], H, W, 1, s, nullptr));
diff --git a/lemo_amd/csrc/kernels.hpp b/lemo_amd/csrc/kernels.hpp
--- a/lemo_amd/csrc/kernels.hpp
+++ b/lemo_amd/csrc/kernels.hpp
@@ -45,6 +45,8 @@
 int conv3x3_pair_f16(const float* in, const void* wA, float winvA, const float* biasA, const float* auxA, float* mid, const void* wB,
                      float winvB, const float* biasB, const float* auxB, float* out, int H, int W, int epi, hipStream_t s,
                      unsigned long long* dbg = nullptr);
+int conv3x3_pair_smooth_f16(const float* z, const void* wA, float winvA, const float* auxA, const void* wB, float winvB, const float* auxB,
+                            float* out, int H, int W, float coef2, double* sm_acc, hipStream_t s, unsigned long long* dbg = nullptr);
 bool conv3x3_wino_supported(int H, int W, int cin, int cout);
 int conv3x3_wino_f16(const float* in, const void* wU, float winv, const float* wt, const float* bias, const float* aux, float* out,
                      int H, int W, int epi, hipStream_t s, unsigned long long* dbg = nullptr);
@@ -149,9 +151,10 @@
 int enc_head(const FitConst& fc, const float* verts, int nrows, const float* Jtr, int nj, const float* transl, int B, const float* w0,
              const float* b0, const void* w1pack, float w1inv, const float* b1, float* x0, float* canon, float* act1, float* act2,
              hipStream_t s);
+struct VertexLossRoles { const float *target, *contact, *shape, *other; double* acc; };
 int enc_head3(const FitConst& fc, const float* verts, int nrows, const float* Jtr, int nj, const float* transl, int B, const float* w0,
               const float* b0, const void* w1pack, float w1inv, const float* b1, const void* w2pack, float w2inv, const float* b2,
-              float* x0, float* canon, float* act1, float* act2, float* act3, hipStream_t s);
+              float* x0, float* canon, float* act1, float* act2, float* act3, hipStream_t s, const VertexLossRoles* roles = nullptr);
 int enc_tail(const float* din, const void* w1bpack, float w1binv, const float* act1, const float* w0, float* dx0, int H, int W, hipStream_t s);
 int enc_tail3(const float* din, const void* w2bpack, float w2binv, const float* act2, const void* w1bpack, float w1binv, const float* act1,
               const float* w0, float* dx0, int H, int W, hipStream_t s);
diff --git a/lemo_amd/csrc/lemo_hip.hip b/lemo_amd/csrc/lemo_hip.hip
--- a/lemo_amd/csrc/lemo_hip.hip
+++ b/lemo_amd/csrc/lemo_hip.hip
@@ -86,6 +86,11 @@
                           unsigned long long* dbg, void* stream) {
   return conv3x3_pair_f16(in, wA, winvA, biasA, auxA, mid, wB, winvB, biasB, auxB, out, H, W, epi, S(stream), dbg);
 }
+int lemo_conv3x3_pair_smooth_f16(const float* z, const void* wA, float winvA, const float* auxA, const void* wB, float winvB,
+                                 const float* auxB, float* out, int H, int W, float coef2, double* sm_acc, unsigned long long* dbg,
+                                 void* stream) {
+  return conv3x3_pair_smooth_f16(z, wA, winvA, auxA, wB, winvB, auxB, out, H, W, coef2, sm_acc, S(stream), dbg);
+}
 int lemo_enc_head(const lemo_fit_const* fc, const float* verts, int nrows, const float* Jtr, int nj, const float* transl, int B, const float* w0,
                   const float* b0, const void* w1pack, float w1inv, const float* b1, float* x0, float* canon, float* act1, float* act2,
                   void* stream) {
@@ -294,15 +299,16 @@
   hipGraphExec_t exec[FIT_MAXG + 1] = {};
   int head = 5;
   FitSide fs;
+  bool fold = false;
 };
 
-static int fit_iteration(const lemo_fit_desc& d, hipStream_t s, bool first, bool last, FitSide* fs);
+static int fit_iteration(const lemo_fit_desc& d, hipStream_t s, bool first, bool last, FitSide* fs, bool fold);
 
 static int capture_iterations(FitEngine* e, hipStream_t s, int iters, hipGraphExec_t* out) {
   hipGraph_t g = nullptr;
   CHK((int)hipStreamBeginCapture(s, hipStreamCaptureModeThreadLocal));
   int rc = 0;
-  for (int i = 0; i < iters && !rc; ++i) rc = fit_iteration(e->d, s, i == 0, i == iters - 1, &e->fs);
+  for (int i = 0; i < iters && !rc; ++i) rc = fit_iteration(e->d, s, i == 0, i == iters - 1, &e->fs, e->fold);
   const int ec = (int)hipStreamEndCapture(s, &g);
   if (rc) { if (g) (void)hipGraphDestroy(g); return rc; }
   CHK(ec);
@@ -356,7 +362,19 @@
   return fs->side ? (int)hipStreamWaitEvent(s, fs->join, 0) : 0;
 }
 
-static int fit_forward(const lemo_fit_desc& d, hipStream_t s, bool finalize, bool compute_h1 = true, unsigned stages = ~0u, FitSide* fs = nullptr) {
+static bool fit_fold_losses(const lemo_fit_desc& d) {
+  const int H = 3 * d.fit.n81 + 2, W = d.B - 1 + 16;
+  return d.conv_variant == 9 && !d.per_frame && enc_fused_head3(d) && d.enc_wbwd3[9] && d.enc_wbwd3[8] &&
+         conv3x3_pair_supported(H, W, d.enc_ch[10], d.enc_ch[9], d.enc_ch[8]);
+}
+static float fit_smooth_coef2(const lemo_fit_desc& d) {
+  const int H = 3 * d.fit.n81 + 2, W = d.B - 1 + 16;
+  return (float)((double)d.weights_host[5] * 2.0 / ((double)d.enc_ch[10] * H * (W - 1)));
+}
+
+static int fit_forward(const lemo_fit_desc& d, hipStream_t s, bool finalize, bool compute_h1 = true, unsigned stages = ~0u, FitSide* fs = nullptr,
+                       bool fold = false) {
+  if (fold && finalize) return LEMO_ERR_ARG;
   const int B = d.B, nj = d.body.nj;
   const int H = 3 * d.fit.n81 + 2, W = B - 1 + 16;
   if (stages & 1u) {
@@ -388,9 +406,11 @@
     return 0;
   }
   if (stages & 4u) {
-  if (enc_fused_head3(d))
+  if (enc_fused_head3(d)) {
+    const VertexLossRoles vl{d.target, d.contact, d.shape, d.other, d.loss_acc};
     CHK(enc_head3(d.fit, d.verts, d.nrows, d.pose.Jtr, nj, d.transl, B, d.enc_w[0], d.enc_b[0], d.enc_w3[1], d.enc_w3_inv[1], d.enc_b[1], d.enc_w3[2],
-                  d.enc_w3_inv[2], d.enc_b[2], d.x0, d.canon, d.act[1], d.act[2], d.act[3], s));
+                  d.enc_w3_inv[2], d.enc_b[2], d.x0, d.canon, d.act[1], d.act[2], d.act[3], s, fold ? &vl : nullptr));
+  }
   else if (enc_fused_head(d))
     CHK(enc_head(d.fit, d.verts, d.nrows, d.pose.Jtr, nj, d.transl, B, d.enc_w[0], d.enc_b[0], d.enc_w3[1], d.enc_w3_inv[1], d.enc_b[1], d.x0, d.canon,
                  d.act[1], d.act[2], s));
@@ -399,21 +419,22 @@
   CHK(enc_chain_fwd(d, H, W, s, enc_fused_head3(d) ? 3 : (enc_fused_head(d) ? 2 : 1)));
   }
   const double cnt = (double)d.enc_ch[10] * H * (W - 1);
-  const float coef2 = (float)((double)d.weights_host[5] * 2.0 / cnt);
-  if (stages & 8u)
+  const float coef2 = fit_smooth_coef2(d);
+  if ((stages & 8u) && !fold)
   CHK(fit_losses(d.act[10], d.dact[0], H, W, d.enc_ch[10], coef2, d.loss_acc + 9, d.fit, d.verts, d.nrows, d.target, d.contact,
                  d.shape, d.other, B, d.loss_acc, s));
   if (finalize) CHK(loss_finalize(d.loss_acc, B, d.fit.n67, cnt, d.weights, d.losses, s));
   return 0;
 }
 
-static int fit_backward(const lemo_fit_desc& d, hipStream_t s, bool update = false, bool next_h1 = false, unsigned stages = ~0u, FitSide* fs = nullptr) {
+static int fit_backward(const lemo_fit_desc& d, hipStream_t s, bool update = false, bool next_h1 = false, unsigned stages = ~0u, FitSide* fs = nullptr,
+                        bool fold = false) {
   const int B = d.B, nj = d.body.nj;
   const int H = 3 * d.fit.n81 + 2, W = B - 1 + 16;
   const double cnt = d.per_frame ? 1.0 : (double)d.enc_ch[10] * H * (W - 1);
   int cur = 0;
   if (d.per_frame || !(stages & 16u)) goto vertex_stage;
-  CHK(enc_chain_bwd(d, H, W, s, &cur, enc_bwd_l_last(d)));
+  CHK(enc_chain_bwd(d, H, W, s, &cur, enc_bwd_l_last(d), fold ? d.loss_acc + 9 : nullptr, fit_smooth_coef2(d)));
   CHK(enc_bwd_tail(d, cur, H, W, s));
   if (fs && d.verts_side && !d.full_vertices) {
     if (fs->side) {
@@ -446,11 +467,11 @@
   return 0;
 }
 
-static int fit_iteration(const lemo_fit_desc& d, hipStream_t s, bool first, bool last, FitSide* fs) {
+static int fit_iteration(const lemo_fit_desc& d, hipStream_t s, bool first, bool last, FitSide* fs, bool fold) {
   const bool side = d.verts_side && !d.full_vertices && !d.per_frame;
-  CHK(fit_forward(d, s, false, first, ~0u, side ? fs : nullptr));
+  CHK(fit_forward(d, s, false, first, ~0u, side ? fs : nullptr, fold));
   if (side && !fs) return LEMO_ERR_STATE;
-  CHK(fit_backward(d, s, true, !last, ~0u, side ? fs : nullptr));
+  CHK(fit_backward(d, s, true, !last, ~0u, side ? fs : nullptr, fold));
   if (last) CHK(fit_side_join(fs, s));
   return 0;
 }
@@ -464,6 +485,8 @@
     e->d = *d;
     if (d->per_frame) e->head = 0;
     if (const char* h = getenv("LEMO_FIT_HEAD")) e->head = atoi(h);
+    const char* f = getenv("LEMO_FIT_FOLD_LOSSES");
+    e->fold = (!f || atoi(f) != 0) && fit_fold_losses(*d);
     if (d->verts_side && !d->full_vertices) {
       if (!d->transl_side || d->per_frame) { delete e; return nullptr; }
       if (hipStreamCreateWithPriority(&e->fs.side, hipStreamNonBlocking, getenv("LEMO_FIT_SIDE_PRIO") ? atoi(getenv("LEMO_FIT_SIDE_PRIO")) : 0) != hipSuccess ||
@@ -501,7 +524,7 @@
   if (!e || n < 0) return LEMO_ERR_ARG;
   hipStream_t s = S(stream);
   if (!use_graph) {
-    for (int i = 0; i < n; ++i) CHK(fit_iteration(e->d, s, i == 0, i == n - 1, &e->fs));
+    for (int i = 0; i < n; ++i) CHK(fit_iteration(e->d, s, i == 0, i == n - 1, &e->fs, e->fold));
     return 0;
   }
   CHK(fit_graphs(e, s, n, false));
@@ -525,14 +548,16 @@
   CHK((int)hipEventCreate(&e0));
   CHK((int)hipEventCreate(&e1));
   int rc = 0;
+  const bool fold = e->fold;
   for (int k = 0; k <= LEMO_FIT_NSTAGE && !rc; ++k) {
     const unsigned mask = k == LEMO_FIT_NSTAGE ? ~0u : (1u << k);
+    if (fold && k == 3) { ms_out[k] = 0.f; continue; }
     hipGraph_t g = nullptr;
     hipGraphExec_t x = nullptr;
     rc = (int)hipStreamBeginCapture(s, hipStreamCaptureModeThreadLocal);
     for (int r = 0; r < reps && !rc; ++r) {
-      if (mask & 15u) rc = fit_forward(d, s, false, true, mask);
-      if (!rc && (mask & 112u)) rc = fit_backward(d, s, false, false, mask);
+      if (mask & 15u) rc = fit_forward(d, s, false, true, mask, nullptr, fold);
+      if (!rc && (mask & 112u)) rc = fit_backward(d, s, false, false, mask, nullptr, fold);
     }
     const int ec = (int)hipStreamEndCapture(s, &g);
     if (!rc) rc = ec;
diff --git a/lemo_amd/csrc/loss_device.hpp b/lemo_amd/csrc/loss_device.hpp
--- a/lemo_amd/csrc/loss_device.hpp
+++ b/lemo_amd/csrc/loss_device.hpp
@@ -127,6 +127,61 @@
     const float v = ((red[0][t] + red[1][t]) + red[2][t]) + red[3][t];
     if (v != 0.f) atomicAdd(accg + (b & 31) * 16 + (t < 9 ? t : t + 1), (double)v);
   }
+}
+
+__device__ __forceinline__ void vertex_loss_wave(int b, int lane, const FitConst& fc, const float* __restrict__ verts, int nrows,
+                                                 const float* __restrict__ target, const float* __restrict__ contact,
+                                                 const float* __restrict__ shape, const float* __restrict__ other, int B,
+                                                 double* __restrict__ accg) {
+  float acc[12];
+#pragma unroll
+  for (int i = 0; i < 12; ++i) acc[i] = 0.f;
+  const int nm = fc.n67 * 3;
+  for (int w0 = lane; w0 < nm; w0 += 256) {
+    float d[4];
+#pragma unroll
+    for (int u = 0; u < 4; ++u) {
+      const int w = w0 + 64 * u, wc = w < nm ? w : w0;
+      const int m = wc / 3, c = wc - 3 * m;
+      const float e = fabsf(verts[((size_t)b * nrows + fc.row67[m]) * 3 + c] - target[((size_t)b * fc.n67 + m) * 3 + c]);
+      d[u] = w < nm ? e : 0.f;
+    }
+    acc[0] += d[0]; acc[0] += d[1]; acc[0] += d[2]; acc[0] += d[3];
+  }
+  if (b < B - 1) {
+    bool on[4];
+#pragma unroll
+    for (int k = 0; k < 4; ++k) on[k] = contact[(size_t)b * 4 + k] == 1.f;
+    const int q0 = fc.foot_start[0], q1 = fc.foot_start[4], s1 = fc.foot_start[1], s2 = fc.foot_start[2], s3 = fc.foot_start[3];
+    for (int qb = q0 + lane; qb < q1; qb += 128) {
+      float sp[2];
+      int kq[2];
+#pragma unroll
+      for (int u = 0; u < 2; ++u) {
+        const int q = qb + 64 * u, qc = q < q1 ? q : qb;
+        const float* v0 = verts + ((size_t)b * nrows + fc.foot_row[qc]) * 3;
+        const float* v1 = v0 + (size_t)nrows * 3;
+        const float vx = (v1[0] - v0[0]) * 30.f, vy = (v1[1] - v0[1]) * 30.f, vz = (v1[2] - v0[2]) * 30.f;
+        sp[u] = sqrtf(vx * vx + vy * vy + vz * vz);
+        kq[u] = q < q1 ? (qc >= s1) + (qc >= s2) + (qc >= s3) : -1;
+      }
+#pragma unroll
+      for (int u = 0; u < 2; ++u)
+#pragma unroll
+        for (int k = 0; k < 4; ++k)
+          if (kq[u] == k && on[k] && sp[u] - 0.1f > 0.f) { acc[1 + k] += sp[u]; acc[5 + k] += 1.f; }
+    }
+  }
+  if (lane < 32) { const float v = other[(size_t)b * 56 + lane]; acc[9] = v * v; }
+  if (lane < 10) { const float v = shape[(size_t)b * 10 + lane]; acc[10] = v * v; }
+  if (lane < 24) { const float v = other[(size_t)b * 56 + 32 + lane]; acc[11] = v * v; }
+  float mine = 0.f;
+#pragma unroll
+  for (int i = 0; i < 12; ++i) {
+    const float s = wave_sum(acc[i]);
+    mine = lane == i ? s : mine;
+  }
+  if (lane < 12 && mine != 0.f) atomicAdd(accg + (b & 31) * 16 + (lane < 9 ? lane : lane + 1), (double)mine);
 }
 
 __device__ __forceinline__ void finalize_losses(const double* tot, int B, int n67, double smooth_count,
```

Measured after the change: 3592, median of 6. 1.02x the previous value.
